# microsoft/GenerativeImage2Text

Hardware: AMD Instinct MI355X
Metric: captions/sec whole-node (GIT_BASE 224px bs=64/GPU greedy len=20) (higher is better)
Workload: dtype f16; 1 GPU; GIT_BASE 224px bs=64/GPU greedy max_len=20 frames=1; global_batch=64, parallelism=dp1, decode_steps_per_caption=19, seq_len_returned=20, hip_graph=True, contexts_in_flight=4, layernorm_folded=True, library=libgitmi_f16.so, encoder_chains=2, schedule=mixed

## Files before the change

generativeimage2text_amd/csrc/abi_ops.hip:

```cpp
#include "../../include/gitmi.h"
#include "abi_common.h"
#include "gitmi_common.h"
#include "launchers.h"

#include <hip/hip_runtime.h>

using namespace gitmi;

#ifdef GITMI_EXPERIMENT
#include "../../include/gitmi_experiment.h"
#define GITMI_EXP_EXPORT extern "C"
#else
#define GITMI_EXP_EXPORT [[maybe_unused]] static
#endif

static inline int round_up(int x, int m) { return (x + m - 1) / m * m; }

extern "C" int gitmi_operand_dtype(void);
static const char* dtype_name(int dtype) {
    return dtype == GITMI_DTYPE_F32 ? "fp32" : dtype == GITMI_DTYPE_BF16 ? "bf16" : dtype == GITMI_DTYPE_F16 ? "fp16" : "unknown";
}
static int check_dtype(const char* op, const char* arg, int dtype) {
    if (dtype == GITMI_DTYPE_F32 || dtype == gitmi_operand_dtype()) return 0;
    return fail("%s: %s is %s (%d), but this library's 16-bit operands are %s (libgitmi%s.so)", op, arg, dtype_name(dtype), dtype,
// ... 164 lines not shown
                                                  const float* stats, int strips, float eps, int M, int V, int K, int cols_per_wg,
                                                  int mtop, const int* ids, int ld_ids, int cur_len, const int* plen, int beams,
                                                  int suppress_kind, float rep_penalty, float* part_val, int* part_idx,
                                                  float* part_lse, float* logits_out, int max_wgs, void* stream) {
    if (!A || !W || !bias || !part_val || !part_idx || !part_lse) return fail("debug_vocab_topm_rules: null argument");
    if (cols_per_wg != 128) return fail("debug_vocab_topm_rules: cols_per_wg must be 128");
    VocabArgs v = vocab_op_args(A, W, bias, colsum, stats, strips, eps, M, V, K, cols_per_wg, part_val, part_idx, part_lse, logits_out, max_wgs);
    if (ids) {
        if (!plen) return fail("debug_vocab_topm_rules: ids without plen");
        if (beams < 1 || M % beams) return fail("debug_vocab_topm_rules: M=%d is not a multiple of beams=%d", M, beams);
        if (cur_len < 1 || cur_len > ld_ids) return fail("debug_vocab_topm_rules: cur_len=%d outside [1, ld_ids=%d]", cur_len, ld_ids);
        if (rep_penalty != 0.f && rep_penalty != 1.f && cur_len > HIST_SLOTS / 2)
            return fail("debug_vocab_topm_rules: the repetition penalty supports histories up to %d tokens (cur_len=%d)", HIST_SLOTS / 2, cur_len);
        v.ids = ids; v.ld_ids = ld_ids; v.cur_len = cur_len; v.plen = plen; v.beams = beams; v.suppress_kind = suppress_kind;
        v.rep_penalty = rep_penalty;
    }
    HIPCK(launch_vocab_topm(v, mtop, (hipStream_t)stream));
    return 0;
}

extern "C" int gitmi_op_sample_rows(const float* logits, int R, int V, float temperature, int top_k, float top_p, int ndraw,
                                    uint64_t seed, int step, float* draw_logprob, int* draw_token, float* filtered_out,
                                    void* stream) {
    float2* lse = nullptr;
    HIPCK(hipMalloc((void**)&lse, (size_t)R * sizeof(float2)));
    hipError_t err = launch_sample_rows(logits, V, V, R, temperature, top_k, top_p, ndraw, seed, step, draw_logprob, draw_token,
                                        lse, filtered_out, nullptr, 0, 0, 0.f, ndraw, (hipStream_t)stream);
    if (err == hipSuccess) err = hipStreamSynchronize((hipStream_t)stream);
    hipFree(lse);
    HIPCK(err);
    return 0;
}

GITMI_EXP_EXPORT int gitmi_debug_set_gemm_impl(int impl) {
    if (!set_gemm_impl(impl)) return fail("debug_set_gemm_impl: unknown selector %d (low byte: -1, 0 or 9)", impl);
    return 0;
}

GITMI_EXP_EXPORT int gitmi_debug_gemm_form(const void* A, int lda, const void* W, const float* bias, const void* res, int ldr, void* C,
                                           int ldc, int M, int N, int K, int act, int in_dtype, int out_dtype, int shared,
                                           const float* ln_part, const float* colsum, float ln_eps, float* part_out,
                                           const float* res_part, const float* res_gamma, const float* res_beta, float res_eps,
                                           void* stream) {
    if (!A || !W || !C) return fail("debug_gemm_form: null argument (A, W, C)");
    if (M < 0 || N < 1 || K < 1) return fail("debug_gemm_form: M=%d N=%d K=%d", M, N, K);
    if (lda < K) return fail("debug_gemm_form: lda=%d < K=%d", lda, K);
    if (ldc < N) return fail("debug_gemm_form: ldc=%d < N=%d", ldc, N);
    if (res && ldr < N) return fail("debug_gemm_form: ldr=%d < N=%d", ldr, N);
    if (act < GITMI_ACT_NONE || act > GITMI_ACT_GELU_ERF) return fail("debug_gemm_form: act=%d", act);
    RCK(check_dtype("debug_gemm_form", "in_dtype", in_dtype));
    const bool in_f32 = in_dtype == GITMI_DTYPE_F32;
    if ((in_f32 && K % 16) || (!in_f32 && K % 64)) return fail("debug_gemm_form: K must be a multiple of %d (K=%d)", in_f32 ? 16 : 64, K);
    GemmArgs g{};
    g.A = A; g.W = W; g.bias = bias; g.res = (const float*)res; g.C = C;
    g.M = M; g.N = N; g.K = K; g.lda = lda; g.ldc = ldc; g.ldr = res ? ldr : 0; g.act = act;
    g.shared = shared ? 1 : 0;
    if (out_dtype == GITMI_DTYPE_F16_STREAM) {
        if (in_f32) return fail("debug_gemm_form: fp16 stream rows need 16-bit operands");
        g.out_f16 = 1;
    } else {
        RCK(check_dtype("debug_gemm_form", "out_dtype", out_dtype));
    }
    const bool out_f32 = out_dtype == GITMI_DTYPE_F32;
    const bool consumer = ln_part != nullptr, producer = part_out != nullptr || res_part != nullptr;
    if (colsum && !consumer) return fail("debug_gemm_form: colsum without ln_part");
    if ((res_gamma || res_beta) && !res_part) return fail("debug_gemm_form: res_gamma / res_beta without res_part");
    if (consumer || producer) {
#ifndef GITMI_OPS_F16
        return fail("debug_gemm_form: the folded-LayerNorm forms are built into the fp16-operand library only");
#endif
        if (consumer && producer) return fail("debug_gemm_form: consumer (ln_part) and producer (part_out / res_part) arguments in one launch");
        if (consumer) {
            if (!colsum) return fail("debug_gemm_form: ln_part without colsum");
            if (res || in_f32 || out_f32 || g.out_f16) return fail("debug_gemm_form: the consumer writes operand-type rows and takes no residual");
            if (K > 1024) return fail("debug_gemm_form: row partials cover K <= 1024 (K=%d)", K);
            g.ln_part = (const float2*)ln_part; g.ln_nparts = (K + 255) / 256; g.ln_colsum = colsum; g.ln_inv_d = 1.0f / (float)K; g.ln_eps = ln_eps;
        } else {
            if (!g.out_f16 || act != GITMI_ACT_NONE) return fail("debug_gemm_form: the producer writes fp16 stream rows and has no activation");
            if (N > 1024) return fail("debug_gemm_form: row partials cover N <= 1024 (N=%d)", N);
            g.part_out = (float2*)part_out;
            if (res_part) {
                if (!res || !res_gamma || !res_beta) return fail("debug_gemm_form: res_part without res / res_gamma / res_beta");
                g.res_part = (const float2*)res_part; g.res_nparts = (N + 255) / 256; g.res_gamma = res_gamma; g.res_beta = res_beta;
                g.res_inv_d = 1.0f / (float)N; g.res_eps = res_eps;
            }
        }
        if (!gemm_uses_p8(g, false, false))
            return fail("debug_gemm_form: the folded forms exist in gemm_p8_kernel only (more than 512 rows, N %% 256 == 0, K >= 128, 16-byte aligned rows)");
    }
    HIPCK(launch_gemm(g, in_f32, out_f32, (hipStream_t)stream));
    return 0;
}

extern "C" int gitmi_op_attn_decode(const void* qkv, const void* img_k, const void* img_v, void* txt_k, void* txt_v,
                                    const int* kv_src, void* out, int B, int H, int N_img, int T_max, int pos, int beams,
                                    int dtype, int dbg, void* stream) {
    RCK(check_dtype("op_attn_decode", "dtype", dtype));
    AttnDecodeArgs a{};
    a.qkv = qkv; a.img_k = img_k; a.img_v = img_v; a.txt_k = txt_k; a.txt_v = txt_v; a.out = out;
    a.kv_src = kv_src; a.ld_src = T_max; a.d = H * 64; a.N_img = N_img; a.T_max = T_max; a.pos = pos; a.beams = beams;
    a.scale = 0.125f; a.dbg = dbg & 0xffff; a.waves_per_pair = (dbg >> 16) & 3; a.stream_wgs = dbg >> 18;
    if (dtype == GITMI_DTYPE_F32) {
        HIPCK(launch_attn_decode(a, B, H, (hipStream_t)stream));
        return 0;
    }
    a.N_pad = round_up(N_img, 32);
    HIPCK(launch_attn_decode_mfma(a, B, H, (hipStream_t)stream));
    return 0;
}
extern "C" int gitmi_op_kv_repack(const void* qkv_rows, void* kf, void* vt, int B, int N, int H, void* stream) {
    HIPCK(launch_kv_repack_frag(qkv_rows, kf, vt, B, N, round_up(N, 32), H, H * 64, (hipStream_t)stream));
    return 0;
}

GITMI_EXP_EXPORT int gitmi_debug_attention_ragged(const void* qkv, void* out, const int* ntok, int B, int N, int H, int dtype, int impl,
                                                  void* stream) {
    if (!ntok) return fail("debug_attention_ragged: ntok is required");
    const size_t esz = dtype == GITMI_DTYPE_F32 ? 4 : 2;
    const int D = H * 64;
    AttnFullArgs a{};
    a.q = qkv;
    a.k = (const char*)qkv + (size_t)D * esz;
    a.v = (const char*)qkv + (size_t)2 * D * esz;
    a.out = out;
    a.ldq = a.ldk = a.ldv = 3 * D;
    a.ldo = D;
    a.N = N; a.H = H; a.scale = 0.125f; a.ntok = ntok;
    HIPCK(launch_attn_full(a, B, dtype == GITMI_DTYPE_F32, impl, (hipStream_t)stream));
    return 0;
}
GITMI_EXP_EXPORT int gitmi_debug_attn_decode_form(const void* qkv, const void* img_k, const void* img_v, void* txt_k, void* txt_v,
                                                  const int* kv_src, void* out, const int* ntok, const int* img_of, int n_images,
                                                  int B, int H, int N_img, int T_max, int pos, int beams, int dtype, int out_frag,
                                                  int pairs_per_wg, int waves_per_pair, int stream_wgs, void* stream) {
    RCK(check_dtype("debug_attn_decode_form", "dtype", dtype));
    if (!qkv || !img_k || !img_v || !txt_k || !txt_v || !kv_src || !out) return fail("debug_attn_decode_form: null argument");
    if (beams < 1 || beams > 8) return fail("debug_attn_decode_form: beams=%d outside [1, 8]", beams);
    if (n_images < 1) return fail("debug_attn_decode_form: n_images=%d", n_images);
    if (B < 1 || H < 1 || N_img < 1 || pos < 0 || pos >= T_max)
        return fail("debug_attn_decode_form: B=%d H=%d N_img=%d pos=%d T_max=%d", B, H, N_img, pos, T_max);
    if (out_frag && dtype == GITMI_DTYPE_F32) return fail("debug_attn_decode_form: out_frag needs 16-bit rows");
    if (ntok && stream_wgs > 0) return fail("debug_attn_decode_form: the streaming kernel does not serve ragged batches (ntok)");
    AttnDecodeArgs a{};
    a.qkv = qkv; a.img_k = img_k; a.img_v = img_v; a.txt_k = txt_k; a.txt_v = txt_v; a.out = out;
    a.kv_src = kv_src; a.ld_src = T_max; a.d = H * 64; a.N_img = N_img; a.T_max = T_max; a.pos = pos; a.beams = beams;
    a.scale = 0.125f; a.ntok = ntok; a.img_of = img_of; a.out_frag = out_frag;
    a.pairs_per_wg = pairs_per_wg; a.waves_per_pair = waves_per_pair; a.stream_wgs = stream_wgs;
    if (dtype == GITMI_DTYPE_F32) {
        HIPCK(launch_attn_decode(a, B, H, (hipStream_t)stream));
        return 0;
    }
    a.N_pad = round_up(N_img, 32);
    HIPCK(launch_attn_decode_mfma(a, B, H, (hipStream_t)stream));
    return 0;
}
GITMI_EXP_EXPORT int gitmi_debug_attn_decode_ragged(const void* qkv, const void* img_k, const void* img_v, void* txt_k, void* txt_v,
                                                    const int* kv_src, void* out, const int* ntok, int B, int H, int N_img, int T_max,
                                                    int pos, int beams, int dtype, void* stream) {
    if (!ntok) return fail("debug_attn_decode_ragged: ntok is required");
    return gitmi_debug_attn_decode_form(qkv, img_k, img_v, txt_k, txt_v, kv_src, out, ntok, nullptr, B, B, H, N_img, T_max, pos, beams,
                                        dtype, 0, 0, 0, 0, stream);
}

extern "C" int gitmi_preprocess_image(const uint8_t* rgb_hwc, int H, int W, int crop, uint8_t* tmp, size_t tmp_bytes,
                                      float* out_chw, void* stream) {
    if (!rgb_hwc || !out_chw || H < 1 || W < 1 || crop < 1) return fail("preprocess: bad argument");
    const int nw = W <= H ? crop : (int)((double)crop * W / H);
    if (nw != W && (!tmp || tmp_bytes < (size_t)H * nw * 3)) return fail("preprocess: workspace must hold H * %d * 3 bytes", nw);
    HIPCK(launch_preprocess(rgb_hwc, H, W, crop, tmp, out_chw, (hipStream_t)stream));
    return 0;
}

extern "C" int gitmi_preprocess_batch(const uint8_t* rgb, size_t rgb_bytes, const int64_t* desc_host, int n, int crop, uint8_t* tmp,
                                      size_t tmp_bytes, float* out, void* stream) {
    if (!rgb || !desc_host || !out || n < 1 || crop < 1 || crop > 4096) return fail("preprocess_batch: bad argument");
    for (int i = 0; i < n; ++i) {
        const int64_t off = desc_host[3 * i], H = desc_host[3 * i + 1], W = desc_host[3 * i + 2];
        if (H < 1 || W < 1 || H > 65535 || W > 65535 || off < 0 || (uint64_t)off + (uint64_t)H * W * 3 > rgb_bytes ||
            (uint64_t)off + (uint64_t)H * W * 3 > 0xffffffffull)
            return fail("preprocess_batch: image %d (offset %lld, %lld x %lld) does not fit the staging buffer of %zu bytes", i,
                        (long long)off, (long long)H, (long long)W, rgb_bytes);
        const double r = W <= H ? (double)H / W : (double)W / H;
        if (r * crop > 65535.0) return fail("preprocess_batch: image %d: aspect ratio too extreme", i);
    }
    const size_t need = preprocess_batch_workspace((const long long*)desc_host, n, crop);
    if (need > 0 && (!tmp || tmp_bytes < need)) return fail("preprocess_batch: workspace must hold %zu bytes", need);
    if (need > 0xffffffffull) return fail("preprocess_batch: batch too large for one call");
    HIPCK(launch_preprocess_batch(rgb, (const long long*)desc_host, n, crop, tmp, out, (hipStream_t)stream));
    return 0;
}

extern "C" int gitmi_preprocess_image_to(const uint8_t* rgb_hwc, int H, int W, int out_h, int out_w, uint8_t* tmp,
                                         size_t tmp_bytes, float* out_chw, void* stream) {
    if (!rgb_hwc || !out_chw || H < 1 || W < 1 || out_h < 1 || out_w < 1) return fail("preprocess: bad argument");
    if (out_w != W && (!tmp || tmp_bytes < (size_t)H * out_w * 3))
        return fail("preprocess: workspace must hold H * %d * 3 bytes", out_w);
    HIPCK(launch_resize_crop_norm(rgb_hwc, H, W, out_h, out_w, 0, 0, out_h, out_w, tmp, out_chw, (hipStream_t)stream));
    return 0;
}

GITMI_EXP_EXPORT int gitmi_debug_score_attn(const void* qkv, const void* img_kv, const int* image_of, void* out, int Q, int H,
                                            int N_img, int Lp, int dtype, void* stream) {
    if (!qkv || !img_kv || !image_of || !out) return fail("debug_score_attn: null argument");
    if (dtype != GITMI_DTYPE_F32 && dtype != gitmi_operand_dtype()) return fail("debug_score_attn: dtype %d not served by this build", dtype);
    HIPCK(launch_score_attn(qkv, img_kv, image_of, out, Q, H, H * 64, N_img, Lp, 0.125f, dtype == GITMI_DTYPE_F32,
                            (hipStream_t)stream));
    return 0;
}
GITMI_EXP_EXPORT int gitmi_debug_score_attn_map(const void* qkv, const void* img_kv, const int* image_of, const int* ntok, float* out,
                                                int Q, int H, int N_img, int Lp, int dtype, void* stream) {
    if (!qkv || !img_kv || !image_of || !out || Q < 1 || H < 1 || N_img < 1 || Lp < 1) return fail("debug_score_attn_map: bad argument");
    if (dtype != GITMI_DTYPE_F32 && dtype != gitmi_operand_dtype()) return fail("debug_score_attn_map: dtype %d not served by this build", dtype);
    hipStream_t s = (hipStream_t)stream;
    const bool f32 = dtype == GITMI_DTYPE_F32;
    const int d = H * 64, Kc = N_img + Lp;
    void* ctx = nullptr; float2* stats = nullptr;
    auto body = [&]() -> int {
        HIPCK(hipMalloc(&ctx, (size_t)Q * Lp * d * (f32 ? 4 : 2)));
        HIPCK(hipMalloc(&stats, (size_t)Q * H * Lp * sizeof(float2)));
        HIPCK(launch_score_attn(qkv, img_kv, image_of, ctx, Q, H, d, N_img, Lp, 0.125f, f32, s, ntok, stats));
        HIPCK(launch_score_attn_map(qkv, img_kv, image_of, ntok, stats, nullptr, out, (size_t)Lp * Kc, (size_t)Kc, Lp, Q, H, N_img, Lp,
                                    0.125f, f32, nullptr, s));
        HIPCK(hipStreamSynchronize(s));
        return 0;
    };
    const int rc = body();
    hipFree(ctx); hipFree(stats);
    return rc;
}
GITMI_EXP_EXPORT int gitmi_debug_score_head(const void* A, const void* W, const float* bias, const int* tgt, int M, int V, int K,
                                            int dtype, float* out, void* stream) {
    if (!A || !W || !bias || !tgt || !out || M < 1 || V < 2 || K < 32 || K % 32) return fail("debug_score_head: bad argument");
    if (dtype != GITMI_DTYPE_F32 && dtype != gitmi_operand_dtype()) return fail("debug_score_head: dtype %d not served by this build", dtype);
    hipStream_t s = (hipStream_t)stream;
    const bool f32 = dtype == GITMI_DTYPE_F32;
    const int ntiles = f32 ? 1 : score_head_tiles(V);
    const int ldl = round_up(V, 8);
    float4* part = nullptr; float* zt = nullptr; float2* o2 = nullptr; int* bad = nullptr; float* logits = nullptr;
    int rc = 0;
    auto body = [&]() -> int {
        HIPCK(hipMalloc(&part, (size_t)M * ntiles * sizeof(float4)));
        HIPCK(hipMalloc(&zt, (size_t)M * sizeof(float)));
        HIPCK(hipMalloc(&o2, (size_t)(M + 1) * sizeof(float2)));
        HIPCK(hipMalloc(&bad, (size_t)M * sizeof(int)));
        if (f32) {
            HIPCK(hipMalloc(&logits, (size_t)M * ldl * sizeof(float)));
            GemmArgs g{};
            g.A = A; g.W = W; g.bias = bias; g.C = logits; g.M = M; g.N = V; g.K = K; g.lda = K; g.ldc = ldl;
            HIPCK(launch_gemm(g, true, true, s));
            HIPCK(launch_score_rowstats(logits, ldl, V, tgt, 0, M, part, zt, s));
        } else {
            HIPCK(launch_score_head(A, K, W, bias, tgt, M, V, K, part, zt, s));
        }
        HIPCK(hipMemsetAsync(o2, 0, (size_t)(M + 1) * sizeof(float2), s));
        HIPCK(launch_score_combine(part, ntiles, zt, tgt, M, 1, 1, V, o2, bad, s));
        HIPCK(hipMemcpyAsync(out, o2 + 1, (size_t)M * sizeof(float2), hipMemcpyDefault, s));
        HIPCK(hipStreamSynchronize(s));
        return 0;
    };
    rc = body();
    hipFree(part); hipFree(zt); hipFree(o2); hipFree(bad); hipFree(logits);
    return rc;
}

#ifdef GITMI_EXPERIMENT
GITMI_EXP_EXPORT int gitmi_debug_im2col(const float* img, void* out, int out_dtype, int B, int H, int W, int p, int K, int Kpad,
                                        void* stream) {
    if (!img || !out) return fail("debug_im2col: null argument");
    RCK(check_dtype("debug_im2col", "out_dtype", out_dtype));
    if (B < 1 || p < 1 || H < p || W < p || K != 3 * p * p || Kpad < K) return fail("debug_im2col: bad shape");
    HIPCK(launch_im2col(img, out, out_dtype == GITMI_DTYPE_F32, B, H, W, p, K, Kpad, (hipStream_t)stream));
    return 0;
}
GITMI_EXP_EXPORT int gitmi_debug_pos_resize(const float* pos, float* out, int g, int gh, int gw, int D, void* stream) {
    if (!pos || !out || g < 1 || gh < 1 || gw < 1 || D < 1) return fail("debug_pos_resize: bad argument");
    HIPCK(launch_pos_bicubic(pos, out, g, gh, gw, D, (hipStream_t)stream));
    return 0;
}
GITMI_EXP_EXPORT int gitmi_debug_vit_assemble(const float* patch_out, const float* cls, const float* pos, const float* gamma,
                                              const float* beta, float eps, void* X, int x_f16, int B, int N, int D, float* part,
                                              void* stream) {
    if (!patch_out || !cls || !pos || !gamma || !beta || !X || B < 1 || N < 1 || D < 1) return fail("debug_vit_assemble: bad argument");
    HIPCK(launch_vit_assemble_ln(patch_out, cls, pos, gamma, beta, eps, X, x_f16 != 0, B, N, D, (float2*)part, (D + 255) / 256,
                                 (hipStream_t)stream));
    return 0;
}
GITMI_EXP_EXPORT int gitmi_debug_ragged_front(int stage, const float* src, float* slots, int* meta, int* ntok, void* patches,
                                              int patches_dtype, const float* patch_out, const float* cls, const float* pos, int g,
                                              const float* gamma, const float* beta, float eps, void* X, int x_f16, float* part,
                                              int B, int p, long long max_pixels, int Nmax, int K, int Kpad, int D, void* stream) {
    hipStream_t s = (hipStream_t)stream;
    if (B < 1 || p < 1 || max_pixels < 1 || Nmax < 2 || !meta) return fail("debug_ragged_front: bad argument");
    const size_t slot = (size_t)3 * (size_t)max_pixels;
    if (stage == 0) {
        if (!src || !slots || !ntok) return fail("debug_ragged_front: staging takes src, slots, meta and ntok");
        HIPCK(launch_ragged_stage(src, slots, slot, (int4*)meta, ntok, B, p, (size_t)max_pixels, Nmax, s));
    } else if (stage == 1) {
        if (!slots || !patches || K != 3 * p * p || Kpad < K) return fail("debug_ragged_front: im2col takes slots, meta and patches");
        RCK(check_dtype("debug_ragged_front", "patches_dtype", patches_dtype));
        HIPCK(launch_im2col_ragged(slots, slot, (const int4*)meta, patches, patches_dtype == GITMI_DTYPE_F32, B, Nmax, p, K, Kpad, s));
    } else if (stage == 2) {
        if (!patch_out || !cls || !pos || !gamma || !beta || !X || g < 1 || D < 1) return fail("debug_ragged_front: assembly argument missing");
        HIPCK(launch_vit_assemble_ragged(patch_out, cls, pos, g, (const int4*)meta, gamma, beta, eps, X, x_f16 != 0, B, Nmax, p, D,
                                         (float2*)part, s));
    } else {
        return fail("debug_ragged_front: stage %d (0 staging, 1 im2col, 2 assembly)", stage);
// ... 51 lines not shown
```

generativeimage2text_amd/csrc/engine.hip:

```cpp
#include "../../include/gitmi.h"
#include "engine_state.h"

#include <algorithm>
#include <cmath>
#include <cstdarg>
#include <cstdio>
#include <cstring>

using namespace gitmi;

#ifdef GITMI_EXPERIMENT
#include "../../include/gitmi_experiment.h"
#define GITMI_EXP_EXPORT extern "C"
#else
#define GITMI_EXP_EXPORT [[maybe_unused]] static
#endif

static thread_local char g_err[1024] = "";
int gitmi::fail(const char* fmt, ...) {
    va_list ap;
    va_start(ap, fmt);
    vsnprintf(g_err, sizeof(g_err), fmt, ap);
    va_end(ap);
    return 1;
// ... 276 lines not shown
    return 0;
}

static Stream vit_stream(gitmi_engine* e, int M) {
    const int D = e->cfg.vit_width;
    const VitLayerW& L = e->w.vit[0];
    Stream st;
    st.x = e->v_x; st.M = M; st.D = D; st.tag = TAG_GEMM_VIT; st.t = e->v_h;
    st.fold = e->pol.ln_fold && on_p8(e->v_x, D, L.qkv_f.w, e->v_qkv, 3 * D, M, 3 * D, D, false) &&
              on_p8(e->v_x, D, L.ffn1_f.w, e->v_u, 4 * D, M, 4 * D, D, false) && on_p8(e->v_ctx, D, L.wo, e->v_x, D, M, D, D, true) &&
              on_p8(e->v_u, 4 * D, L.w2, e->v_x, D, M, D, 4 * D, true);
    if (st.fold) st.parts[0] = st.parts[1] = e->v_part;
    return st;
}
static Stream prefill_stream(gitmi_engine* e, int M) {
    const int d = e->cfg.dec_hidden, ffn = e->cfg.dec_ffn, D = e->cfg.vit_width;
    const DecLayerW& L = e->w.dec[0];
    Stream st;
    st.x = e->p_y; st.M = M; st.D = d; st.tag = TAG_GEMM_OTHER; st.t = e->p_ht; st.xn = e->p_hf;
    st.fold = e->pol.ln_fold && on_p8(e->feats, D, e->w.vp_w, e->p_y, d, M, d, D, true) &&
              on_p8(e->p_y, d, L.qkv_pf.w, e->img_kv[0], 3 * d, M, 3 * d, d, false) &&
              on_p8(e->p_y, d, L.qkv_pf.w, e->img_kv[0], 3 * d, M, 2 * d, d, false) &&
              (e->cfg.dec_layers < 2 || (on_p8(e->p_y, d, L.ffn1_pf.w, e->p_u, ffn, M, ffn, d, false) &&
                                         on_p8(e->p_ctx, d, L.wo, e->p_y, d, M, d, d, true) && on_p8(e->p_u, ffn, L.w2, e->p_y, d, M, d, ffn, true)));
    if (st.fold) { st.parts[0] = e->p_part[0]; st.parts[1] = e->p_part[1]; }
    return st;
}

static int encode_frames_impl(gitmi_engine* e, const float* const* frames, int F, int B, float* feats_out,
                              hipStream_t s, int stride = 0) {
    const gitmi_config& c = e->cfg;
    const int D = c.vit_width, N = e->N;
    const int F_eff = c.num_frames > 0 ? std::min(F, c.num_frames) : F;
    const int Nimg = stride > 0 ? stride : F_eff * N;
    drop_resident(e);
    SpanGuard phase(e, s, TAG_VIT, 0);
    const int BI = F_eff * B;
    const int M = BI * N;
    const int g2 = N - 1;
    const size_t slot = (size_t)3 * e->max_pixels;
    if (e->ragged)
        HIPCK(launch_im2col_ragged(e->frame_stage[0], slot, e->rg_meta, e->patches, e->pol.f32, B, N, c.patch, e->Kp, e->Kp_pad, s));
    else
    for (int fr = 0; fr < F_eff; ++fr)
        HIPCK(launch_im2col(frames[fr], (char*)e->patches + (size_t)fr * B * g2 * e->Kp_pad * e->pol.esz, e->pol.f32, B,
                            e->H, e->W, c.patch, e->Kp, e->Kp_pad, s));
    RCK(gemm(e, s, e->patches, e->Kp_pad, e->w.conv_w, nullptr, nullptr, 0, e->patch_out, D, true, BI * g2, D, e->Kp_pad, 0,
             TAG_GEMM_VIT));
    Stream x = vit_stream(e, M);
    float2* part = stream_part_out(x);
    if (e->ragged)
        HIPCK(launch_vit_assemble_ragged(e->patch_out, e->w.cls, e->w.pos, e->g_nat, e->rg_meta, e->w.lnpre_g, e->w.lnpre_b, 1e-5f, e->v_x,
                                         e->pol.stream_f16, BI, N, c.patch, D, part, s));
    else
    HIPCK(launch_vit_assemble_ln(e->patch_out, e->w.cls, e->pos_cur, e->w.lnpre_g, e->w.lnpre_b, 1e-5f, e->v_x, e->pol.stream_f16, BI, N, D,
                                 part, D / 256, s));
    stream_written(x, part, e->w.vit[0].ln1g, e->w.vit[0].ln1b, 1e-5f);
    for (int l = 0; l < c.vit_layers; ++l) {
        const VitLayerW& L = e->w.vit[l];
        const VitLayerW* Ln = l + 1 < c.vit_layers ? &e->w.vit[l + 1] : nullptr;
        RCK(ln_gemm(e, s, x, L.qkv_f, L.wqkv, L.bqkv, e->v_qkv, 3 * D, 0, 3 * D, 0));
        RCK(attn_full_packed(e, e->v_qkv, e->v_ctx, D, c.vit_heads, N, BI, e->ragged ? e->rg_ntok : nullptr, s));
        RCK(gemm_to_stream(e, s, x, e->v_ctx, D, L.wo, L.bo, D, true, L.ln2g, L.ln2b, 1e-5f));
        RCK(ln_gemm(e, s, x, L.ffn1_f, L.w1, L.b1, e->v_u, 4 * D, 0, 4 * D, 1));
        RCK(gemm_to_stream(e, s, x, e->v_u, 4 * D, L.w2, L.b2, 4 * D, true, Ln ? Ln->ln1g : nullptr, Ln ? Ln->ln1b : nullptr, 1e-5f));
    }
    for (int fr = 0; fr < F_eff; ++fr) {
        const float* te = (c.num_frames > 0 && e->pol.use_temb) ? e->w.temb[fr] : nullptr;
        if (e->pol.stream_f16) {
            const char* xs = (const char*)e->v_x + (size_t)fr * B * N * D * 2;
            HIPCK(launch_layernorm_s16(xs, D, e->w.lnpost_g, e->w.lnpost_b, 1e-5f, te, e->feats, D, false, nullptr, 0, B * N, D, N,
                                       Nimg, fr * N, s));
            if (feats_out)
                HIPCK(launch_layernorm_s16(xs, D, e->w.lnpost_g, e->w.lnpost_b, 1e-5f, te, feats_out, D, true, nullptr, 0, B * N, D,
                                           N, Nimg, fr * N, s));
        } else {
            HIPCK(launch_layernorm(e->v_x + (size_t)fr * B * N * D, D, e->w.lnpost_g, e->w.lnpost_b, 1e-5f, te, e->feats, D, e->pol.f32,
                                   feats_out, D, B * N, D, N, Nimg, fr * N, s));
        }
    }
    if (e->ragged) {
        HIPCK(launch_zero_pad_rows(e->feats, e->pol.f32, D, e->rg_ntok, B, N, s));
        if (feats_out) HIPCK(launch_zero_pad_rows(feats_out, true, D, e->rg_ntok, B, N, s));
    }

    set_resident(e, B, F_eff, stride);
    return 0;
}

static int kv_repack(gitmi_engine* e, int l, int B, int Nimg, hipStream_t s) {
    const gitmi_config& c = e->cfg;
    void* kh = e->img_kh[l];
    void* vh = e->img_vh[l];
    if (e->pol.f32) HIPCK(launch_kv_repack(e->img_kv[l], kh, vh, B, Nimg, c.dec_heads, c.dec_hidden, s));
    else HIPCK(launch_kv_repack_frag(e->img_kv[l], kh, vh, B, Nimg, round_up(Nimg, 32), c.dec_heads, c.dec_hidden, s));
    return 0;
}

static int prefill_impl(gitmi_engine* e, hipStream_t s) {
    const gitmi_config& c = e->cfg;
    const int d = c.dec_hidden, ffn = c.dec_ffn, D = c.vit_width;
    const int B = e->cur_B, Nimg = e->cur_Nimg, M = B * Nimg;
    e->have_prefill = false;
    SpanGuard phase(e, s, TAG_PREFILL, 0);
    Stream y = prefill_stream(e, M);
    RCK(gemm_to_stream(e, s, y, e->feats, D, e->w.vp_w, e->w.vp_b, D, false, e->w.vp_lng, e->w.vp_lnb, 1e-5f));
    for (int l = 0; l < c.dec_layers; ++l) {
        const DecLayerW& L = e->w.dec[l];
        const bool last = l + 1 == c.dec_layers;
        const int col0 = last ? d : 0;
        RCK(ln_gemm(e, s, y, L.qkv_pf, L.wqkv, L.bqkv, e->img_kv[l], 3 * d, col0, 3 * d - col0, 0));
        RCK(kv_repack(e, l, B, Nimg, s));
        if (last) break;
        RCK(attn_full_packed(e, e->img_kv[l], e->p_ctx, d, c.dec_heads, Nimg, B, key_counts(e), s));
        RCK(gemm_to_stream(e, s, y, e->p_ctx, d, L.wo, L.bo, d, true, L.lnag, L.lnab, 1e-12f));
        RCK(ln_gemm(e, s, y, L.ffn1_pf, L.w1, L.b1, e->p_u, ffn, 0, ffn, 2));
        RCK(gemm_to_stream(e, s, y, e->p_u, ffn, L.w2, L.b2, ffn, true, L.lnog, L.lnob, 1e-12f));
    }
    set_prefilled(e);
    return 0;
}

#ifdef GITMI_EXPERIMENT
#define GITMI_SKIPPED(e, bit) (((e)->pol.decode_skip & (bit)) != 0)
#else
#define GITMI_SKIPPED(e, bit) false
#endif
static int dgemm(gitmi_engine* e, hipStream_t s, const DGemmArgs& g_in) {
    DGemmArgs g = g_in;
    g.dbg = e->pol.dgemm_dbg;
    g.no_row_walk = e->pol.dgemm_no_row_walk >= 0 ? e->pol.dgemm_no_row_walk : e->pol.shared_device ? 0 : 1;
    g.strips_per_wg = e->pol.dgemm_strips >= 0 ? e->pol.dgemm_strips : e->pol.shared_device ? 2 : 1;
    g.rows_per_wg = e->pol.dgemm_rows > 0 ? e->pol.dgemm_rows : g.M > 64 ? 64 : e->pol.shared_device ? 32 : 16;
    SpanGuard sp(e, s, TAG_GEMM_OTHER, gemm_flops(g.M, g.N, g.K));
    HIPCK(launch_dgemm(g, s));
    return 0;
}

static DGemmArgs dgemm_ln(const void* A, const Folded& f, const DLn* ln, void* C, int c_frag, int act, int M, int N, int K) {
    return dgemm_ln(A, f.w, f.bias, f.colsum, ln, C, c_frag, act, M, N, K);
}

static int decode_layers_impl(gitmi_engine* e, const int* kv_src, int ld_ids, int pos, int R, int beams, hipStream_t s) {
    const gitmi_config& c = e->cfg;
    const int d = c.dec_hidden, ffn = c.dec_ffn;
    const int B = R / beams;
    const bool chain = e->pol.skinny && !e->pol.f32;
    for (int l = 0; l < c.dec_layers; ++l) {
        const DecLayerW& L = e->w.dec[l];
        const DecLayerW* Lp = l > 0 ? &e->w.dec[l - 1] : nullptr;
        const DLn ln_prev{e->stats_o, d / 16, 1.0f / (float)d, 1e-12f, Lp ? Lp->lnog : nullptr, Lp ? Lp->lnob : nullptr};
        const DLn ln_a{e->stats_a, d / 16, 1.0f / (float)d, 1e-12f, L.lnag, L.lnab};
        const DLn* ln_o = Lp ? &ln_prev : nullptr;
        if (chain) {
            if (!GITMI_SKIPPED(e, 2)) RCK(dgemm(e, s, dgemm_ln(l == 0 ? e->d_ht : e->xo_b, L.qkv_f, ln_o, e->d_qkv, 0, 0, R, 3 * d, d)));
        } else {
            RCK(gemm(e, s, e->d_ht, d, L.wqkv, L.bqkv, nullptr, 0, e->d_qkv, 3 * d, e->pol.f32, R, 3 * d, d, 0, TAG_GEMM_OTHER));
        }
        AttnDecodeArgs a{};
        a.qkv = e->d_qkv; a.img_k = e->img_kh[l]; a.img_v = e->img_vh[l]; a.txt_k = e->txt_k[l]; a.txt_v = e->txt_v[l]; a.out = e->d_ctx;
        a.kv_src = kv_src; a.ld_src = ld_ids; a.d = d; a.N_img = e->cur_Nimg; a.T_max = c.max_text_len;
        a.img_of = e->img_identity ? nullptr : e->img_of_dev;
        a.pos = pos; a.beams = beams; a.scale = 0.125f;
        a.out_frag = chain ? 1 : 0;
        a.N_pad = round_up(e->cur_Nimg, 32);
        a.dbg = e->pol.attn_dbg;
        a.waves_per_pair = e->pol.attn_nh;
        a.pairs_per_wg = e->pol.attn_pw > 0 ? e->pol.attn_pw : e->pol.shared_device ? 8 : 4;
        const bool stream_ok = !e->pol.shared_device && a.N_pad <= 8 * 32 && B * c.dec_heads >= 384 && e->pol.attn_nh != 2;
        a.stream_wgs = e->pol.attn_stream >= 0 ? e->pol.attn_stream : stream_ok ? 192 : 0;
        if (e->keyed) { a.ntok = e->rg_ntok; a.stream_wgs = 0; }
        if (e->pol.f32) HIPCK(launch_attn_decode(a, B, c.dec_heads, s));
        else if (!GITMI_SKIPPED(e, 1)) HIPCK(launch_attn_decode_mfma(a, B, c.dec_heads, s));
        if (chain) {
            if (!GITMI_SKIPPED(e, 4))
                RCK(dgemm(e, s, dgemm_to_stream(e->d_ctx, L.wo_p, L.bo, l == 0 ? e->d_hf : e->xo_f, ln_o, e->xa_f, e->xa_b, e->stats_a, R, d, d)));
            if (!GITMI_SKIPPED(e, 2)) RCK(dgemm(e, s, dgemm_ln(e->xa_b, L.ffn1_f, &ln_a, e->d_u, 1, 2, R, ffn, d)));
            if (!GITMI_SKIPPED(e, 4))
                RCK(dgemm(e, s, dgemm_to_stream(e->d_u, L.w2_p, L.b2, e->xa_f, &ln_a, e->xo_f, e->xo_b, e->stats_o, R, d, ffn)));
        } else {
            RCK(dec_layer_tail(e, s, L, e->d_ctx, e->d_hf, e->d_ht, e->d_y, e->d_u, R));
        }
    }
    return 0;
}

static int sample_candidates(gitmi_engine* e, const float* logits, int ldl, int R, int step, hipStream_t s, StepCands* cands);
static int trie_candidates(gitmi_engine* e, const float* logits, int ldl, int cur_len, hipStream_t s, StepCands* cands);
static float rep_penalty_of(const gitmi_engine* e) {
    const double rp = e->sample.repetition_penalty;
    return (e->ss.kind == GITMI_SEARCH_GENERATOR && rp > 0 && rp != 1.0) ? (float)rp : 0.f;
}

static int decode_head_impl(gitmi_engine* e, const int* ids, int ld_ids, int cur_len, int R, int beams, int suppress_kind,
                            int M, float* logits_out, int ldl, hipStream_t s, StepCands* cands) {
    const gitmi_config& c = e->cfg;
    const int d = c.dec_hidden;
    const bool chain = e->pol.skinny && !e->pol.f32;
    cands->part_val = e->part_val; cands->part_idx = e->part_idx; cands->part_lse = e->part_lse;
    const bool sampling = ids != nullptr && e->ss.sampled;
    const bool trie = ids != nullptr && e->trie_search;
    if ((sampling || trie) && !logits_out) { logits_out = e->logits; ldl = e->ldl; }
    if (chain) {
        VocabArgs v{};
        v.A = (const unsigned short*)e->xo_b; v.lda = d; v.W = (const unsigned short*)e->w.out_f.w; v.bias = e->w.out_f.bias; v.colsum = e->w.out_f.colsum;
        v.stats_in = e->stats_o; v.strips_in = d / 16; v.inv_d = 1.0f / (float)d; v.eps_in = 1e-12f;
        v.M = R; v.N = c.vocab; v.K = d; v.cols_per_wg = e->vocab_cols;
        v.max_wgs = e->pol.vocab_wgs >= 0 ? e->pol.vocab_wgs : (e->pol.shared_device && R <= 64) ? 60 : 0;
        v.ids = ids; v.ld_ids = ld_ids; v.cur_len = cur_len; v.plen = e->plen_dev; v.beams = beams; v.suppress_kind = suppress_kind;
        v.rep_penalty = ids ? rep_penalty_of(e) : 0.f;
        v.part_val = e->part_val; v.part_idx = e->part_idx; v.part_lse = e->part_lse;
        v.logits_out = logits_out; v.ld_logits = ldl;
        {
            SpanGuard sp(e, s, TAG_GEMM_OTHER, gemm_flops(R, c.vocab, d));
            if (!GITMI_SKIPPED(e, 8)) HIPCK(launch_vocab_topm(v, M, s));
        }
        cands->nparts = e->vocab_nparts; cands->slots = vocab_mtop_slots(M);
        if (sampling) RCK(sample_candidates(e, logits_out, ldl, R, cur_len, s, cands));
        if (trie) RCK(trie_candidates(e, logits_out, ldl, cur_len, s, cands));
    } else {
        RCK(gemm(e, s, e->d_ht, d, e->w.out_w, e->w.out_b, nullptr, 0, e->logits, e->ldl, true, R, c.vocab, d, 0, TAG_GEMM_OTHER));
        cands->nparts = 1; cands->slots = row_topm_slots(M);
        if (sampling) RCK(sample_candidates(e, e->logits, e->ldl, R, cur_len, s, cands));
        else if (trie) RCK(trie_candidates(e, e->logits, e->ldl, cur_len, s, cands));
        else if (ids)
            HIPCK(launch_row_topm(e->logits, e->ldl, c.vocab, ids, ld_ids, cur_len, e->plen_dev, beams, suppress_kind,
                                  rep_penalty_of(e), M, R,
                                  e->part_val, e->part_idx, e->part_lse, s));
        if (logits_out && logits_out != e->logits) HIPCK(launch_copy_f32(e->logits, e->ldl, logits_out, ldl, R, c.vocab, s));
    }
    return 0;
}

static int check_ready(gitmi_engine* e) {
    if (!e) return fail("null engine");
    if (!e->finalized) return fail("weights not finalized (call gitmi_finalize_weights)");
    HIPCK(hipSetDevice(e->device));
    return 0;
}

static int ragged_prepare(gitmi_engine* e, const float* const* frames, int F, int B, hipStream_t s) {
    if (!e->ragged) return 0;
    if (F != 1 || !frames[0]) return fail("ragged input (gitmi_set_image_shape(e, 0, 0)): F must be 1, frames[0] the descriptor buffer");
    drop_resident(e);
    HIPCK(launch_ragged_stage(frames[0], e->frame_stage[0], (size_t)3 * e->max_pixels, e->rg_meta, e->rg_ntok, B, e->cfg.patch,
                              e->max_pixels, e->Nmax, s));
    return 0;
}

static int check_frames(const gitmi_engine* e, const char* who, const float* const* frames, int F, int B) {
    if (!frames || F < 1 || F > e->cfg.max_frames) return fail("%s: F=%d outside [1,%d]", who, F, e->cfg.max_frames);
    if (B < 1 || B > e->cfg.max_batch) return fail("%s: B=%d outside [1,%d]", who, B, e->cfg.max_batch);
    return 0;
}

static int check_resident(const gitmi_engine* e, const char* who, int B) {
    if (!e->have_feats)
        return fail("%s: frames == NULL is a follow-up call, but the engine holds no resident images (encode some with a call "
                    "that takes frames; a change of the image shape or mode, of the temporal embedding or of the LayerNorm "
                    "folding, and a failed call, drop them)", who);
    if (B != e->cur_B) return fail("%s: follow-up call with B=%d, but %d images are resident (B must equal that count)", who, B, e->cur_B);
    return 0;
}

extern "C" int gitmi_encode_frames(gitmi_engine* e, const float* const* frames, int F, int B, float* feats_out,
                                   void* stream) {
    RCK(check_ready(e));
    RCK(check_frames(e, "encode_frames", frames, F, B));
    RCK(ragged_prepare(e, frames, F, B, (hipStream_t)stream));
    return encode_frames_impl(e, frames, F, B, feats_out, (hipStream_t)stream);
}

static EmbedArgs embed_args(gitmi_engine* e, bool on) {
    EmbedArgs em{};
    if (!on) return em;
    em.words = e->w.words_f; em.positions = e->w.positions_f; em.gamma = e->w.emb_lng; em.beta = e->w.emb_lnb; em.eps = 1e-8f;
    em.h_f = e->d_hf; em.h_t = e->d_ht; em.D = e->cfg.dec_hidden; em.vocab = e->cfg.vocab;
    em.frag = (e->pol.skinny && !e->pol.f32) ? 1 : 0;
    return em;
}
static int embed_position(gitmi_engine* e, const int* ids, int ld_ids, int pos, int R, hipStream_t s) {
    const EmbedArgs em = embed_args(e, true);
    HIPCK(launch_embed_ln(ids, ld_ids, pos, em.words, em.positions, em.gamma, em.beta, em.eps, em.h_f, em.h_t, e->pol.f32, R, em.D,
                          em.vocab, em.frag != 0, s));
    return 0;
}

extern "C" int gitmi_prefill(gitmi_engine* e, void* stream) {
    RCK(check_ready(e));
    if (!e->have_feats) return fail("prefill: no encoded frames");
    return prefill_impl(e, (hipStream_t)stream);
}

extern "C" int gitmi_step_logits(gitmi_engine* e, const int64_t* tokens, int R, int t, float* logits_out, void* stream) {
    RCK(check_ready(e));
    if (!e->have_feats) return fail("step_logits: no encoded frames");
    hipStream_t s = (hipStream_t)stream;
    if (!e->have_prefill) RCK(prefill_impl(e, s));
    const int B = e->cur_B;
    if (R < B || R % B) return fail("step_logits: R=%d is not a multiple of the encoded batch %d", R, B);
    const int beams = R / B;
    if (beams > e->cfg.max_beams) return fail("step_logits: %d beams exceed max_beams", beams);
    if (t < 1 || t > e->cfg.max_text_len) return fail("step_logits: t=%d outside [1,%d]", t, e->cfg.max_text_len);
    const gitmi_config& c = e->cfg;
    const int T = c.max_text_len;
    e->img_identity = true;
    HIPCK(launch_load_ids((const long long*)tokens, R, t, e->ss.ids[0], e->ss.kv_src[0], T, s));
    StepCands cands{};
    for (int pos = 0; pos < t; ++pos) {
        SpanGuard step(e, s, TAG_STEP, 0);
        RCK(embed_position(e, e->ss.ids[0], T, pos, R, s));
        RCK(decode_layers_impl(e, e->ss.kv_src[0], T, pos, R, beams, s));
        if (pos == t - 1) RCK(decode_head_impl(e, nullptr, T, t, R, beams, 0, 1, logits_out, c.vocab, s, &cands));
    }
    return 0;
}

static int search_begin_impl(gitmi_engine* e, const Request& rq, int V, hipStream_t s) {
    const gitmi_config& c = e->cfg;
    const gitmi_search* sp = rq.sp;
    const int B = rq.Q, minP = rq.minP, maxP = rq.maxP;
    if (!sp) return fail("search: null config");
    if (sp->kind != GITMI_SEARCH_AUTOREGRESSIVE && sp->kind != GITMI_SEARCH_GENERATOR && sp->kind != GITMI_SEARCH_TRIE)
        return fail("search: bad kind");
    if (sp->kind == GITMI_SEARCH_TRIE) {
// ... 784 lines not shown
```

generativeimage2text_amd/csrc/kernels_attn_decode.hip:

```cpp
#include "gitmi_common.h"
#include "launchers.h"
#include <algorithm>
#include <type_traits>

#pragma clang fp contract(off)

namespace gitmi {

static constexpr int HD = 64;

__global__ __launch_bounds__(256) void kv_repack_frag_kernel(const bf16_t* __restrict__ qkv, bf16_t* __restrict__ kf,
                                                             bf16_t* __restrict__ vt, int N, int Np, int H, int d) {
    __shared__ bf16_t vs[32][HD + 8];
    const int s = blockIdx.x, h = blockIdx.y, b = blockIdx.z, tid = threadIdx.x;
    const int nsteps = Np >> 5;
    bf16_t* kdst = kf + ((size_t)b * H + h) * Np * HD;
    bf16_t* vdst = vt + ((size_t)b * H + h) * Np * HD;
    const int key = tid >> 3, ch = tid & 7;
    const int n = s * 32 + key;
    u32x4_t kv = {0u, 0u, 0u, 0u}, vv = kv;
    if (n < N) {
        const bf16_t* src = qkv + ((size_t)b * N + n) * 3 * d + d + h * HD + ch * 8;
        kv = *reinterpret_cast<const u32x4_t*>(src);
        vv = *reinterpret_cast<const u32x4_t*>(src + d);
    }
    *reinterpret_cast<u32x4_t*>(kdst + frag_tile(n >> 4, ch >> 2, 2, (ch & 3) * 16 + (n & 15))) = kv;
    *reinterpret_cast<u32x4_t*>(&vs[key][ch * 8]) = vv;
    __syncthreads();
    const int dt = tid >> 6, lane = tid & 63, lg = lane >> 4, dim = dt * 16 + (lane & 15);
    bf16_t o[8];
#pragma unroll
    for (int e = 0; e < 8; ++e) o[e] = vs[(e >> 2) * 16 + lg * 4 + (e & 3)][dim];
    u32x4_t ov;
#pragma unroll
    for (int e = 0; e < 4; ++e) ov[e] = (uint32_t)o[2 * e] | ((uint32_t)o[2 * e + 1] << 16);
    *reinterpret_cast<u32x4_t*>(vdst + (((size_t)s * 4 + dt) * 64 + lane) * 8) = ov;
}

__device__ __forceinline__ void unpack8(const u32x4_t& r, float (&v)[8]) {
#pragma unroll
    for (int i = 0; i < 4; ++i) {
        unpack2op(r[i], v[2 * i], v[2 * i + 1]);
    }
}
__device__ __forceinline__ void ld8bf(const bf16_t* p, float (&v)[8]) { unpack8(*reinterpret_cast<const u32x4_t*>(p), v); }

constexpr int ACS = 4;

struct Pair {
    int h, row0;
    bool on;
};

template <int KB>
__device__ __forceinline__ void load_text_kv(const AttnDecodeArgs& a, const Pair& p, int j, int s, int sub, u32x4_t& kr, u32x4_t& vr) {
    if (s == a.pos) {
        const bf16_t* src = reinterpret_cast<const bf16_t*>(a.qkv) + (size_t)(p.row0 + j) * (3 * a.d) + a.d + p.h * HD + sub * 8;
        kr = *reinterpret_cast<const u32x4_t*>(src);
        vr = *reinterpret_cast<const u32x4_t*>(src + a.d);
    } else {
        const int srow = KB == 1 ? p.row0 : a.kv_src[(size_t)(p.row0 + j) * a.ld_src + s];
        const size_t off = ((size_t)srow * a.T_max + s) * a.d + p.h * HD + sub * 8;
        kr = *reinterpret_cast<const u32x4_t*>(reinterpret_cast<const bf16_t*>(a.txt_k) + off);
        vr = *reinterpret_cast<const u32x4_t*>(reinterpret_cast<const bf16_t*>(a.txt_v) + off);
    }
}

template <int KB, int TI>
struct TextItems {
    int j[TI];
    u32x4_t kr[TI], vr[TI];
    __device__ __forceinline__ void load(const AttnDecodeArgs& a, const Pair& p, int grp, int ngrp, int sub) {
        const int nt = a.pos + 1;
#pragma unroll
        for (int u = 0; u < TI; ++u) {
            const int it = grp + ngrp * u;
            j[u] = (p.on && it < a.beams * nt) ? it / nt : -1;
            const int s = it < a.beams * nt ? it % nt : 0;
            kr[u] = u32x4_t{0u, 0u, 0u, 0u};
            vr[u] = kr[u];
            if (j[u] >= 0) load_text_kv<KB>(a, p, j[u], s, sub, kr[u], vr[u]);
        }
    }
};

__device__ __forceinline__ void append_text_cache(const AttnDecodeArgs& a, const Pair& p, int t, int sub) {
    if (p.on && t < a.beams * 8) {
        const int j = t >> 3;
        const bf16_t* src = reinterpret_cast<const bf16_t*>(a.qkv) + (size_t)(p.row0 + j) * (3 * a.d) + a.d + p.h * HD + sub * 8;
        const size_t dst = ((size_t)(p.row0 + j) * a.T_max + a.pos) * a.d + p.h * HD + sub * 8;
        *reinterpret_cast<u32x4_t*>(reinterpret_cast<bf16_t*>(a.txt_k) + dst) = *reinterpret_cast<const u32x4_t*>(src);
        *reinterpret_cast<u32x4_t*>(reinterpret_cast<bf16_t*>(a.txt_v) + dst) = *reinterpret_cast<const u32x4_t*>(src + a.d);
    }
}

__device__ __forceinline__ void load_q_frag(const AttnDecodeArgs& a, const Pair& p, int l15, int lg, bf16x8_t (&qf)[2]) {
#pragma unroll
    for (int ds = 0; ds < 2; ++ds) {
        float qv[8] = {0.f, 0.f, 0.f, 0.f, 0.f, 0.f, 0.f, 0.f};
        if (p.on && l15 < a.beams)
            ld8bf(reinterpret_cast<const bf16_t*>(a.qkv) + (size_t)(p.row0 + l15) * (3 * a.d) + p.h * HD + ds * 32 + lg * 8, qv);
        u32x4_t t;
#pragma unroll
        for (int e = 0; e < 4; ++e) t[e] = pack2bf(qv[2 * e] * a.scale, qv[2 * e + 1] * a.scale);
        qf[ds] = __builtin_bit_cast(bf16x8_t, t);
    }
}

struct ImagePartial {
    float m, l;
    f32x4_t o[4];
    __device__ __forceinline__ void init() {
        m = -INFINITY;
        l = 0.f;
#pragma unroll
        for (int dt = 0; dt < 4; ++dt) o[dt] = f32x4_t{0.f, 0.f, 0.f, 0.f};
    }
    __device__ __forceinline__ static void mask_max(f32x4_t (&sc)[2], int s, int nimg_steps, int n_img, int lg, float& cm) {
#pragma unroll
        for (int t = 0; t < 2; ++t)
#pragma unroll
            for (int r = 0; r < 4; ++r) {
                if (s * 32 + t * 16 + lg * 4 + r >= n_img || s >= nimg_steps) sc[t][r] = -INFINITY;
                cm = fmaxf(cm, sc[t][r]);
            }
    }
    __device__ __forceinline__ float new_max(float cm, bool rescale) {
        cm = fmaxf(cm, __shfl_xor(cm, 16, 64));
        cm = fmaxf(cm, __shfl_xor(cm, 32, 64));
        const float mn = fmaxf(m, cm);
        if (rescale) {
            const float al = fast_exp(m - mn);
            l *= al;
#pragma unroll
            for (int dt = 0; dt < 4; ++dt) { o[dt][0] *= al; o[dt][1] *= al; o[dt][2] *= al; o[dt][3] *= al; }
        }
        m = mn;
        return mn;
    }
    __device__ __forceinline__ bf16x8_t p_frag(const f32x4_t (&sc)[2], float mn) {
        float p[8];
#pragma unroll
        for (int t = 0; t < 2; ++t)
#pragma unroll
            for (int r = 0; r < 4; ++r) {
                p[t * 4 + r] = fast_exp(sc[t][r] - mn);
                l += p[t * 4 + r];
            }
        u32x4_t pp;
#pragma unroll
        for (int e = 0; e < 4; ++e) pp[e] = pack2bf(p[2 * e], p[2 * e + 1]);
        return __builtin_bit_cast(bf16x8_t, pp);
    }
    __device__ __forceinline__ void finish() {
        l += __shfl_xor(l, 16, 64);
        l += __shfl_xor(l, 32, 64);
    }
    template <int KB>
    __device__ __forceinline__ void publish(float (&slot)[KB][HD + 2], int k, int l15, int lg) const {
        if (l15 < k) {
#pragma unroll
            for (int dt = 0; dt < 4; ++dt)
#pragma unroll
                for (int r = 0; r < 4; ++r) slot[l15][dt * 16 + lg * 4 + r] = o[dt][r];
            if (lg == 0) { slot[l15][HD] = m; slot[l15][HD + 1] = l; }
        }
    }
};

template <int KB>
struct TextPartial {
    float q[KB][8], m[KB], l[KB], o[KB][8];
    __device__ __forceinline__ void init(const AttnDecodeArgs& a, const Pair& p, int sub) {
#pragma unroll
        for (int j = 0; j < KB; ++j) {
            m[j] = -INFINITY;
            l[j] = 0.f;
#pragma unroll
            for (int e = 0; e < 8; ++e) { q[j][e] = 0.f; o[j][e] = 0.f; }
            if (p.on && j < a.beams) {
                ld8bf(reinterpret_cast<const bf16_t*>(a.qkv) + (size_t)(p.row0 + j) * (3 * a.d) + p.h * HD + sub * 8, q[j]);
#pragma unroll
                for (int e = 0; e < 8; ++e) q[j][e] *= a.scale;
            }
        }
    }
    __device__ __forceinline__ void item(int jj, const u32x4_t& kr, const u32x4_t& vr) {
        float kv[8], vv[8];
        unpack8(kr, kv);
        unpack8(vr, vv);
#pragma unroll
        for (int j = 0; j < KB; ++j) {
            if (j == jj) {
                float sv = 0.f;
#pragma unroll
                for (int e = 0; e < 8; ++e) sv = fmaf(q[j][e], kv[e], sv);
                sv += __shfl_xor(sv, 1, 64);
                sv += __shfl_xor(sv, 2, 64);
                sv += __shfl_xor(sv, 4, 64);
                const float mn = fmaxf(m[j], sv);
                const float al = fast_exp(m[j] - mn);
                const float pe = fast_exp(sv - mn);
                l[j] = fmaf(l[j], al, pe);
#pragma unroll
                for (int e = 0; e < 8; ++e) o[j][e] = fmaf(o[j][e], al, pe * vv[e]);
                m[j] = mn;
            }
        }
    }
    template <int TI>
    __device__ __forceinline__ void items(const TextItems<KB, TI>& ti, bool enabled) {
#pragma unroll
        for (int u = 0; u < TI; ++u) {
            if (ti.j[u] >= 0 && enabled) item(ti.j[u], ti.kr[u], ti.vr[u]);
        }
    }
    template <int TI>
    __device__ __forceinline__ void tail(const AttnDecodeArgs& a, const Pair& p, int grp, int ngrp, int sub) {
        if (!p.on) return;
        const int nt = a.pos + 1;
        for (int it = grp + ngrp * TI; it < a.beams * nt; it += ngrp) {
            u32x4_t kr, vr;
            load_text_kv<KB>(a, p, it / nt, it % nt, sub, kr, vr);
            item(it / nt, kr, vr);
        }
    }
    __device__ __forceinline__ void merge_groups() {
#pragma unroll
        for (int j = 0; j < KB; ++j) {
#pragma unroll
            for (int off = 8; off < 64; off <<= 1) {
                const float m2 = __shfl_xor(m[j], off, 64);
                const float l2 = __shfl_xor(l[j], off, 64);
                const float mn = fmaxf(m[j], m2);
                const float a1 = m[j] == -INFINITY ? 0.f : fast_exp(m[j] - mn);
                const float a2 = m2 == -INFINITY ? 0.f : fast_exp(m2 - mn);
                l[j] = fmaf(l[j], a1, l2 * a2);
#pragma unroll
                for (int e = 0; e < 8; ++e) {
                    const float o2 = __shfl_xor(o[j][e], off, 64);
                    o[j][e] = fmaf(o[j][e], a1, o2 * a2);
                }
                m[j] = mn;
            }
        }
    }
    __device__ __forceinline__ void fold_into(float (&slot)[KB][HD + 2], int k, int lane, int sub) const {
#pragma unroll
        for (int j = 0; j < KB; ++j) {
            if (lane < 8 && j < k) {
                const float mi = slot[j][HD], li = slot[j][HD + 1];
                const float mn = fmaxf(mi, m[j]);
                const float a1 = mi == -INFINITY ? 0.f : fast_exp(mi - mn);
                const float a2 = m[j] == -INFINITY ? 0.f : fast_exp(m[j] - mn);
#pragma unroll
                for (int e = 0; e < 8; ++e) slot[j][sub * 8 + e] = fmaf(slot[j][sub * 8 + e], a1, o[j][e] * a2);
                if (sub == 0) { slot[j][HD] = mn; slot[j][HD + 1] = fmaf(li, a1, l[j] * a2); }
            }
        }
    }
};

__device__ __forceinline__ void store_out(const AttnDecodeArgs& a, int row, int col, float r) {
    bf16_t* O = reinterpret_cast<bf16_t*>(a.out);
    if (a.out_frag) O[frag_offset(row, col, a.d >> 5)] = f2bf(r);
    else O[(size_t)row * a.d + col] = f2bf(r);
}
template <int KB>
__device__ __forceinline__ void write_rows(const AttnDecodeArgs& a, const Pair& p, const float (&s0)[KB][HD + 2], int t, int nthr) {
    if (!p.on) return;
    for (int i = t; i < a.beams * HD; i += nthr) {
        const int j = i / HD, dd = i % HD;
        const float r1 = s0[j][dd] / s0[j][HD + 1];
        store_out(a, p.row0 + j, p.h * HD + dd, r1);
    }
}
template <int KB>
__device__ __forceinline__ void write_rows(const AttnDecodeArgs& a, const Pair& p, const float (&s0)[KB][HD + 2],
                                           const float (&s1)[KB][HD + 2], int t, int nthr) {
    if (!p.on) return;
    for (int i = t; i < a.beams * HD; i += nthr) {
        const int j = i / HD, dd = i % HD;
        const float m0 = s0[j][HD], m1 = s1[j][HD];
        const float mm = fmaxf(m0, m1);
        const float a0 = m0 == -INFINITY ? 0.f : fast_exp(m0 - mm);
        const float a1 = m1 == -INFINITY ? 0.f : fast_exp(m1 - mm);
        const float num = fmaf(a0, s0[j][dd], a1 * s1[j][dd]);
        const float den = fmaf(a0, s0[j][HD + 1], a1 * s1[j][HD + 1]);
        const float r = num / den;
        store_out(a, p.row0 + j, p.h * HD + dd, r);
    }
}

template <int KB, int TI = 3, int PW = 1, int NH = 2, bool RAGGED = false>
__global__ __launch_bounds__(64 * NH * PW) void attn_decode_mfma_kernel(AttnDecodeArgs a) {
    __shared__ float part[PW][NH][KB][HD + 2];
    constexpr int PT = 64 * NH;

    const int tid = threadIdx.x, lane = tid & 63, wave = tid >> 6;
    const int l15 = lane & 15, lg = lane >> 4;
    const int hp = wave / NH, half = wave % NH;
    const int H = a.d / HD;
    const int k = a.beams;
    const int Np = a.N_pad, nsteps = Np >> 5;
    const int pair = NH == 2 ? (int)(blockIdx.y * H + blockIdx.x) : (int)blockIdx.x * PW + hp;
    Pair p;
    p.on = PW == 1 || pair < a.n_pairs;
    p.h = p.on ? pair % H : 0;
    const int b = p.on ? pair / H : 0;
    p.row0 = b * k;
    const int bi = a.img_of ? a.img_of[b] : b;
    const bf16_t* Kf = reinterpret_cast<const bf16_t*>(a.img_k) + ((size_t)bi * H + p.h) * Np * HD;
    const bf16_t* Vt = reinterpret_cast<const bf16_t*>(a.img_v) + ((size_t)bi * H + p.h) * Np * HD;
    const int n_img = RAGGED ? a.ntok[bi] : a.N_img;
    const int nimg_steps = (!p.on || (a.dbg & 1)) ? 0 : RAGGED ? (n_img + 31) >> 5 : nsteps;

    bf16x8_t kq[ACS][2][2], vq[ACS][4];
    auto load_chunk = [&](int s0) {
#pragma unroll
        for (int c = 0; c < ACS; ++c) {
            const int s = s0 + NH * c;
            const bool on = s < nimg_steps && !(a.dbg & 8);
            const bf16_t* kp = Kf + frag_tile(2 * s, 0, 2, lane);
            const bf16_t* vp = Vt + ((size_t)s * 4 * 64 + lane) * 8;
#pragma unroll
            for (int t = 0; t < 2; ++t)
#pragma unroll
                for (int ds = 0; ds < 2; ++ds) {
                    const bf16x8_t* q = reinterpret_cast<const bf16x8_t*>(kp + (t * 2 + ds) * 512);
                    kq[c][t][ds] = !on ? bf16x8_t{0, 0, 0, 0, 0, 0, 0, 0} : (a.dbg & 16) ? *q : __builtin_nontemporal_load(q);
                }
#pragma unroll
            for (int dt = 0; dt < 4; ++dt) {
                const bf16x8_t* q = reinterpret_cast<const bf16x8_t*>(vp + dt * 512);
                vq[c][dt] = !on ? bf16x8_t{0, 0, 0, 0, 0, 0, 0, 0} : (a.dbg & 16) ? *q : __builtin_nontemporal_load(q);
            }
        }
    };
    load_chunk(half);

    const int t = tid % PT, grp = t >> 3, sub = tid & 7;
    TextItems<KB, TI> ti;
    ti.load(a, p, grp, 8 * NH, sub);
    append_text_cache(a, p, t, sub);
    bf16x8_t qf[2];
    load_q_frag(a, p, l15, lg, qf);

    ImagePartial ip;
    ip.init();
    for (int s0 = half; s0 < nimg_steps; s0 += NH * ACS) {
        if (s0 != half) load_chunk(s0);
        f32x4_t sc[ACS][2];
        float cm = -INFINITY;
#pragma unroll
        for (int c = 0; c < ACS; ++c) {
#pragma unroll
            for (int u = 0; u < 2; ++u) {
                sc[c][u] = mfma16(kq[c][u][0], qf[0], f32x4_t{0.f, 0.f, 0.f, 0.f});
                sc[c][u] = mfma16(kq[c][u][1], qf[1], sc[c][u]);
            }
            ip.mask_max(sc[c], s0 + NH * c, nimg_steps, RAGGED ? n_img : a.N_img, lg, cm);
        }
        const float mn = ip.new_max(cm, s0 != half);
#pragma unroll
        for (int c = 0; c < ACS; ++c) {
            const bf16x8_t pf = ip.p_frag(sc[c], mn);
            if (a.dbg & 4) {
#pragma unroll
                for (int dt = 0; dt < 4; ++dt) asm volatile("" ::"v"(vq[c][dt]));
                asm volatile("" ::"v"(pf));
                continue;
            }
#pragma unroll
            for (int dt = 0; dt < 4; ++dt) ip.o[dt] = mfma16(vq[c][dt], pf, ip.o[dt]);
        }
    }
    ip.finish();
    TextPartial<KB> tp;
    tp.init(a, p, sub);
    tp.items(ti, !(a.dbg & 2));
    tp.template tail<TI>(a, p, grp, 8 * NH, sub);
    tp.merge_groups();
    ip.publish(part[hp][half], k, l15, lg);
    if constexpr (NH > 1) __syncthreads(); else __builtin_amdgcn_wave_barrier();
    tp.fold_into(part[hp][half], k, lane, sub);
    if constexpr (NH > 1) __syncthreads(); else __builtin_amdgcn_wave_barrier();
    if constexpr (NH == 1) write_rows(a, p, part[hp][0], t, PT);
    else write_rows(a, p, part[hp][0], part[hp][NH - 1], t, PT);
}

typedef __attribute__((address_space(3))) void attn_lds_void_t;

template <int N> __device__ __forceinline__ void attn_wait_vm() { asm volatile("s_waitcnt vmcnt(%0)" ::"n"(N) : "memory"); }
__device__ __forceinline__ void attn_wait_slots_ahead(int ahead) {
    switch (ahead) {
        case 0: attn_wait_vm<0>(); break;
        case 1: attn_wait_vm<4>(); break;
        case 2: attn_wait_vm<8>(); break;
        case 3: attn_wait_vm<12>(); break;
        case 4: attn_wait_vm<16>(); break;
        case 5: attn_wait_vm<20>(); break;
        case 6: attn_wait_vm<24>(); break;
        case 7: attn_wait_vm<28>(); break;
        case 8: attn_wait_vm<32>(); break;
        case 9: attn_wait_vm<36>(); break;
        case 10: attn_wait_vm<40>(); break;
        default: attn_wait_vm<44>(); break;
    }
}

constexpr int AS_WAVES = 4;
constexpr int AS_SLOT = 4096;

template <int KB, int TI, int RING>
__global__ __launch_bounds__(64 * AS_WAVES) void attn_decode_stream_kernel(AttnDecodeArgs a) {
    static_assert(RING >= 2 && RING <= 12, "ring depth");
    __shared__ __attribute__((aligned(16))) unsigned char ring_mem[AS_WAVES][RING * AS_SLOT];
    __shared__ float part[AS_WAVES][KB][HD + 2];

    const int tid = threadIdx.x, lane = tid & 63;
    const int wave = __builtin_amdgcn_readfirstlane(tid >> 6);
    const int l15 = lane & 15, lg = lane >> 4;
    const int H = a.d / HD;
    const int k = a.beams;
    const int Np = a.N_pad, nsteps = Np >> 5;
    unsigned char* ring = ring_mem[wave];

    const int W = (int)gridDim.x * AS_WAVES, w0 = (int)blockIdx.x * AS_WAVES + wave;
    const int npw = w0 < a.n_pairs ? (a.n_pairs - 1 - w0) / W + 1 : 0;
    const int slots_per_pair = 2 * nsteps;
    const int total_slots = npw * slots_per_pair;

    int issued = 0;
    int p_ord = 0, p_s0 = 0, p_v = 0, p_c = 0;
    const bf16_t* p_K = nullptr; const bf16_t* p_V = nullptr;
    auto producer_pair = [&]() {
        const int pair = w0 + p_ord * W;
        const int h = pair % H, b = pair / H;
        const int bi = a.img_of ? a.img_of[b] : b;
        p_K = reinterpret_cast<const bf16_t*>(a.img_k) + ((size_t)bi * H + h) * Np * HD;
        p_V = reinterpret_cast<const bf16_t*>(a.img_v) + ((size_t)bi * H + h) * Np * HD;
    };
    if (npw > 0) producer_pair();
    auto issue_slot = [&]() {
        if (issued >= total_slots) return;
        const bf16_t* src = (p_v ? p_V : p_K) + (size_t)(p_s0 + p_c) * (AS_SLOT / 2) + lane * 8;
        unsigned char* dst = ring + (issued % RING) * AS_SLOT;
#pragma unroll
        for (int f = 0; f < 4; ++f)
            __builtin_amdgcn_global_load_lds((const void*)(src + f * 512), (attn_lds_void_t*)(dst + f * 1024), 16, 0, 2);
        ++issued;
        const int nsc = min(ACS, nsteps - p_s0);
        if (++p_c == nsc) {
            p_c = 0;
            if (p_v == 0) p_v = 1;
            else {
                p_v = 0; p_s0 += ACS;
                if (p_s0 >= nsteps) { p_s0 = 0; ++p_ord; if (p_ord < npw) producer_pair(); }
            }
        }
    };
    for (int i = 0; i < RING; ++i) issue_slot();

    int consumed = 0;
    auto slot_ready = [&]() -> const unsigned char* {
        const int ahead = issued - consumed - 1;
        if (ahead == RING - 1) attn_wait_vm<4 * (RING - 1)>();
        else attn_wait_slots_ahead(ahead);
        return ring + (consumed % RING) * AS_SLOT;
    };
    auto slot_done = [&]() {
        asm volatile("s_waitcnt lgkmcnt(0)" ::: "memory");
        ++consumed;
        issue_slot();
    };


    for (int ord = 0; ord < npw; ++ord) {
        const int pair = w0 + ord * W;
        const Pair p{pair % H, (pair / H) * k, true};

        const int grp = lane >> 3, sub = lane & 7;
        TextItems<KB, TI> ti;
        ti.load(a, p, grp, 8, sub);
        append_text_cache(a, p, lane, sub);
        bf16x8_t qf[2];
        load_q_frag(a, p, l15, lg, qf);

        ImagePartial ip;
        ip.init();
        for (int s0 = 0; s0 < nsteps; s0 += ACS) {
            f32x4_t sc[ACS][2];
            float cm = -INFINITY;
#pragma unroll
            for (int c = 0; c < ACS; ++c) {
                if (s0 + c < nsteps) {
                    const unsigned char* sl = slot_ready();
                    bf16x8_t kq[2][2];
#pragma unroll
                    for (int t = 0; t < 2; ++t)
#pragma unroll
                        for (int ds = 0; ds < 2; ++ds)
                            kq[t][ds] = *reinterpret_cast<const bf16x8_t*>(sl + (t * 2 + ds) * 1024 + lane * 16);
                    __builtin_amdgcn_sched_barrier(0);
#pragma unroll
                    for (int t = 0; t < 2; ++t) {
                        sc[c][t] = mfma16(kq[t][0], qf[0], f32x4_t{0.f, 0.f, 0.f, 0.f});
                        sc[c][t] = mfma16(kq[t][1], qf[1], sc[c][t]);
                    }
                    slot_done();
                } else {
                    sc[c][0] = f32x4_t{0.f, 0.f, 0.f, 0.f};
                    sc[c][1] = sc[c][0];
                }
                ip.mask_max(sc[c], s0 + c, nsteps, a.N_img, lg, cm);
            }
            const float mn = ip.new_max(cm, s0 != 0);
#pragma unroll
            for (int c = 0; c < ACS; ++c) {
                const bf16x8_t pf = ip.p_frag(sc[c], mn);
                if (s0 + c < nsteps) {
                    const unsigned char* sl = slot_ready();
                    bf16x8_t vq[4];
#pragma unroll
                    for (int dt = 0; dt < 4; ++dt) vq[dt] = *reinterpret_cast<const bf16x8_t*>(sl + dt * 1024 + lane * 16);
                    __builtin_amdgcn_sched_barrier(0);
#pragma unroll
                    for (int dt = 0; dt < 4; ++dt) ip.o[dt] = mfma16(vq[dt], pf, ip.o[dt]);
                    slot_done();
                } else {
#pragma unroll
                    for (int dt = 0; dt < 4; ++dt) ip.o[dt] = mfma16(bf16x8_t{0, 0, 0, 0, 0, 0, 0, 0}, pf, ip.o[dt]);
                }
            }
        }
        ip.finish();
        TextPartial<KB> tp;
        tp.init(a, p, sub);
        tp.items(ti, true);
        tp.template tail<TI>(a, p, grp, 8, sub);
        tp.merge_groups();
        ip.publish(part[wave], k, l15, lg);
        __builtin_amdgcn_wave_barrier();
        tp.fold_into(part[wave], k, lane, sub);
        __builtin_amdgcn_wave_barrier();
        write_rows(a, p, part[wave], lane, 64);
        __builtin_amdgcn_wave_barrier();
    }
}

hipError_t launch_kv_repack_frag(const void* qkv, void* kf, void* vt, int B, int N, int N_pad, int H, int d, hipStream_t s) {
    if (B <= 0 || N <= 0) return hipSuccess;
    if (N_pad % 32 || N_pad < N) return hipErrorInvalidValue;
    hipLaunchKernelGGL(kv_repack_frag_kernel, dim3(N_pad / 32, H, B), dim3(256), 0, s, (const bf16_t*)qkv, (bf16_t*)kf,
                       (bf16_t*)vt, N, N_pad, H, d);
    return hipGetLastError();
}

template <typename F>
static void with_beam_rows(int beams, F&& f) {
    if (beams <= 1) f(std::integral_constant<int, 1>{});
    else if (beams <= 2) f(std::integral_constant<int, 2>{});
    else if (beams <= 4) f(std::integral_constant<int, 4>{});
    else f(std::integral_constant<int, 8>{});
}

hipError_t launch_attn_decode_mfma(const AttnDecodeArgs& a, int B, int H, hipStream_t s) {
    if (B <= 0) return hipSuccess;
    if (a.beams > 8 || a.N_pad % 32 || a.N_pad < a.N_img || a.N_img < 1) return hipErrorInvalidValue;
    if (a.ntok && a.stream_wgs > 0) return hipErrorInvalidValue;
    AttnDecodeArgs p = a;
    p.n_pairs = B * H;
    if (a.stream_wgs > 0) {
        const int nwg = std::max(1, std::min(a.stream_wgs, (p.n_pairs + AS_WAVES - 1) / AS_WAVES));
        with_beam_rows(a.beams, [&](auto kb) {
            constexpr int KB = decltype(kb)::value;
            hipLaunchKernelGGL((attn_decode_stream_kernel<KB, 3, KB == 8 ? 8 : 9>), dim3(nwg), dim3(64 * AS_WAVES), 0, s, p);
        });
        return hipGetLastError();
    }
    const bool one_wave = a.waves_per_pair == 1 || (a.waves_per_pair != 2 && a.N_pad <= 8 * 32);
    if (a.ntok || !one_wave) {
        with_beam_rows(a.beams, [&](auto kb) {
            constexpr int KB = decltype(kb)::value;
            if (a.ntok) hipLaunchKernelGGL((attn_decode_mfma_kernel<KB, 3, 1, 2, true>), dim3(H, B), dim3(128), 0, s, p);
            else hipLaunchKernelGGL((attn_decode_mfma_kernel<KB>), dim3(H, B), dim3(128), 0, s, p);
        });
        return hipGetLastError();
    }
    int pw = a.pairs_per_wg >= 8 ? 8 : a.pairs_per_wg >= 4 || a.pairs_per_wg <= 0 ? 4 : a.pairs_per_wg >= 2 ? 2 : 1;
    while (pw > 1 && p.n_pairs / pw < 96) pw >>= 1;
    if (a.beams > 4 && pw == 8) pw = 4;
    with_beam_rows(a.beams, [&](auto kb) {
        constexpr int KB = decltype(kb)::value;
        auto packed = [&](auto pwc) {
            constexpr int PW = decltype(pwc)::value;
            hipLaunchKernelGGL((attn_decode_mfma_kernel<KB, 3, PW, 1>), dim3((p.n_pairs + PW - 1) / PW), dim3(64 * PW), 0, s, p);
        };
        if (pw == 8) { if constexpr (KB < 8) packed(std::integral_constant<int, 8>{}); }
        else if (pw == 4) packed(std::integral_constant<int, 4>{});
        else if (pw == 2) packed(std::integral_constant<int, 2>{});
        else packed(std::integral_constant<int, 1>{});
    });
    return hipGetLastError();
}

}
```

generativeimage2text_amd/csrc/kernels_dgemm.hip:

```cpp
#include "gitmi_common.h"
#include "launchers.h"
#include <type_traits>
#include <utility>

namespace gitmi {

constexpr int STRIP_SLOTS = 16;

struct RowStatLoads {
    float2 v[STRIP_SLOTS];
};
__device__ __forceinline__ void stats_issue(RowStatLoads& L, const float2* __restrict__ stats, int strips, int M,
                                            int row, int lg) {
#pragma unroll
    for (int u = 0; u < STRIP_SLOTS; ++u) {
        const int sidx = lg + 4 * u;
        L.v[u] = sidx < strips ? stats[(size_t)sidx * M + row] : float2{0.f, 0.f};
    }
}
__device__ __forceinline__ void stats_issue_nb(RowStatLoads& L, const float2* __restrict__ stats, int strips, int M,
                                               int row, int lg) {
#pragma unroll
    for (int u = 0; u < STRIP_SLOTS; ++u) {
        const int sidx = lg + 4 * u;
        const float2 v = stats[(size_t)min(sidx, strips - 1) * M + row];
        L.v[u] = sidx < strips ? v : float2{0.f, 0.f};
    }
}
__device__ __forceinline__ void stats_finish(const RowStatLoads& L, float inv_d, float eps, float& mean, float& rstd) {
    float s = 0.f, q = 0.f;
#pragma unroll
    for (int u = 0; u < STRIP_SLOTS; ++u) { s += L.v[u].x; q += L.v[u].y; }
    s += __shfl_xor(s, 16, 64); q += __shfl_xor(q, 16, 64);
    s += __shfl_xor(s, 32, 64); q += __shfl_xor(q, 32, 64);
    mean = s * inv_d;
    const float var = fmaxf(q * inv_d - mean * mean, 0.f);
    rstd = rsqrtf(var + eps);
}


struct KSlice { int kb, ke; };
__device__ __forceinline__ KSlice k_slice(int ksteps, int nw, int wave) {
    const int per = (ksteps + nw - 1) / nw;
    const int kb = wave * per;
    return KSlice{kb, min(kb + per, ksteps)};
}

__device__ __forceinline__ float4 load_cols4(const float* p, int n, int N) {
    float4 r;
    r.x = p[n < N ? n : N - 1];
    r.y = p[n + 1 < N ? n + 1 : N - 1];
    r.z = p[n + 2 < N ? n + 2 : N - 1];
    r.w = p[n + 3 < N ? n + 3 : N - 1];
    return r;
}

constexpr int DW_KS = 6;
struct WSlice { bf16x8_t f[DW_KS]; };
__device__ __forceinline__ WSlice load_w_slice(const bf16_t* W, int strip, KSlice ks, int ksteps, int lane) {
    WSlice w;
    const bf16_t* wp = W + frag_tile(strip, 0, ksteps, lane);
#pragma unroll
    for (int u = 0; u < DW_KS; ++u)
        w.f[u] = ks.kb + u < ks.ke ? __builtin_nontemporal_load(reinterpret_cast<const bf16x8_t*>(wp + (size_t)(ks.kb + u) * 512))
                                   : bf16x8_t{0, 0, 0, 0, 0, 0, 0, 0};
    return w;
}
__device__ __forceinline__ void load_x_slice(bf16x8_t (&xf)[DW_KS][4], const bf16_t* X, int rt0, KSlice ks, int ksteps, int lane) {
#pragma unroll
    for (int u = 0; u < DW_KS; ++u)
#pragma unroll
        for (int i = 0; i < 4; ++i)
            xf[u][i] = ks.kb + u < ks.ke ? *reinterpret_cast<const bf16x8_t*>(X + frag_tile(rt0 + i, ks.kb + u, ksteps, lane))
                                         : bf16x8_t{0, 0, 0, 0, 0, 0, 0, 0};
}
__device__ __forceinline__ void mfma_slice(f32x4_t (&acc)[4], const WSlice& w, const bf16x8_t (&xf)[DW_KS][4], KSlice ks) {
#pragma unroll
    for (int u = 0; u < DW_KS; ++u) {
        if (ks.kb + u < ks.ke) {
#pragma unroll
            for (int i = 0; i < 4; ++i) acc[i] = mfma16(w.f[u], xf[u][i], acc[i]);
        }
    }
}

template <int NW, int MT>
__device__ __forceinline__ f32x4_t sum_waves(f32x4_t (*red)[MT][64], int tile, int lane) {
    f32x4_t tot = {0.f, 0.f, 0.f, 0.f};
#pragma unroll
    for (int w = 0; w < NW; ++w) {
        const f32x4_t t = red[w][tile][lane];
        tot[0] += t[0]; tot[1] += t[1]; tot[2] += t[2]; tot[3] += t[3];
    }
    return tot;
}

#define DGEMM_CONSUMER_FINISH(v, tot, bias4, cs4, have_stats, mean, rstd, act)              \
    float v[4] = {(tot)[0], (tot)[1], (tot)[2], (tot)[3]};                                  \
    {                                                                                       \
        const float biasv[4] = {(bias4).x, (bias4).y, (bias4).z, (bias4).w};                \
        if (have_stats) {                                                                   \
            const float cs[4] = {(cs4).x, (cs4).y, (cs4).z, (cs4).w};                       \
            _Pragma("unroll") for (int r = 0; r < 4; ++r) v[r] = (rstd) * (v[r] - (mean) * cs[r]) + biasv[r]; \
        } else {                                                                            \
            _Pragma("unroll") for (int r = 0; r < 4; ++r) v[r] += biasv[r];                 \
        }                                                                                   \
        if ((act) != GITMI_ACT_NONE) {                                                      \
            _Pragma("unroll") for (int r = 0; r < 4; ++r) v[r] = apply_act(v[r], (act));    \
        }                                                                                   \
    }
__device__ __forceinline__ void consumer_store(const DGemmArgs& g, const float (&v)[4], int fm_raw, int fm, int fn) {
    if (fm_raw >= g.M || fn >= g.N) return;
    if (g.c_frag) {
        uint2 t;
        t.x = pack2bf(v[0], v[1]);
        t.y = pack2bf(v[2], v[3]);
        *reinterpret_cast<uint2*>(reinterpret_cast<bf16_t*>(g.C) + frag_offset(fm, fn, g.N >> 5)) = t;
        return;
    }
    bf16_t* cp = reinterpret_cast<bf16_t*>(g.C) + (size_t)fm * g.ldc + fn;
    if (fn + 3 < g.N && (g.ldc & 3) == 0) {
        uint2 t;
        t.x = pack2bf(v[0], v[1]);
        t.y = pack2bf(v[2], v[3]);
        *reinterpret_cast<uint2*>(cp) = t;
    } else {
        for (int r = 0; r < 4; ++r)
            if (fn + r < g.N) cp[r] = f2bf(v[r]);
    }
}

enum { DEPI_BF16 = 0, DEPI_RES = 1 };

template <int MT, int NW, int EPI>
__global__ __launch_bounds__(64 * NW) void dgemm_kernel(DGemmArgs g) {
    static_assert(NW >= MT, "wave i finishes row tile i: a workgroup needs at least MT waves");
    __shared__ __attribute__((aligned(16))) f32x4_t red[NW][MT][64];

    const int tid = threadIdx.x, lane = tid & 63, wave = tid >> 6;
    const int l15 = lane & 15, lg = lane >> 4;
    const int n0 = blockIdx.x * 16, m0 = blockIdx.y * (16 * MT);

    const bf16_t* __restrict__ X = g.A;
    const bf16_t* __restrict__ W = g.W;

    const bool finisher = wave < MT;
    const int fi = wave;
    const int fm_raw = m0 + fi * 16 + l15;
    const int fm = fm_raw < g.M ? fm_raw : g.M - 1;
    const int fn = n0 + lg * 4;

    RowStatLoads sl;
    bool have_stats = false;
    float4 ep_a = {0.f, 0.f, 0.f, 0.f}, ep_b = ep_a, ep_c = ep_a, ep_d = ep_a;
    if (finisher && !(g.dbg & 8)) {
        ep_a = load_cols4(g.bias, fn, g.N);
        if constexpr (EPI == DEPI_BF16) {
            if (g.stats_in) {
                stats_issue(sl, g.stats_in, g.strips_in, g.M, fm, lg);
                have_stats = true;
                ep_b = load_cols4(g.colsum, fn, g.N);
            }
        } else {
            ep_b = *reinterpret_cast<const float4*>(g.res_x + (size_t)fm * g.N + fn);
            if (g.res_stats) {
                stats_issue(sl, g.res_stats, g.res_strips, g.M, fm, lg);
                have_stats = true;
                ep_c = *reinterpret_cast<const float4*>(g.res_gamma + fn);
                ep_d = *reinterpret_cast<const float4*>(g.res_beta + fn);
            }
        }
    }

    const int ksteps = g.K >> 5;
    const KSlice ks = k_slice(ksteps, NW, wave);

    const bf16_t* wp = W + frag_tile(blockIdx.x, 0, ksteps, lane);
    const bf16_t* xp[MT];
#pragma unroll
    for (int i = 0; i < MT; ++i) xp[i] = X + frag_tile(blockIdx.y * MT + i, 0, ksteps, lane);
    f32x4_t acc[MT];
#pragma unroll
    for (int i = 0; i < MT; ++i) acc[i] = f32x4_t{0.f, 0.f, 0.f, 0.f};

    auto chunk = [&](auto UC, int k0) {
        constexpr int U = decltype(UC)::value;
        bf16x8_t wf[U], xf[U][MT];
#pragma unroll
        for (int u = 0; u < U; ++u) {
            if (g.dbg & 16) wf[u] = *reinterpret_cast<const bf16x8_t*>(wp + (size_t)(k0 + u) * 512);
            else if (!(g.dbg & 2)) wf[u] = __builtin_nontemporal_load(reinterpret_cast<const bf16x8_t*>(wp + (size_t)(k0 + u) * 512));
            else wf[u] = bf16x8_t{1, 1, 1, 1, 1, 1, 1, 1};
#pragma unroll
            for (int i = 0; i < MT; ++i) {
                if (!(g.dbg & 1)) xf[u][i] = *reinterpret_cast<const bf16x8_t*>(xp[i] + (size_t)(k0 + u) * 512);
                else xf[u][i] = bf16x8_t{1, 1, 1, 1, 1, 1, 1, 1};
            }
        }
        if (g.dbg & 4) {
#pragma unroll
            for (int u = 0; u < U; ++u) {
                asm volatile("" ::"v"(wf[u]));
#pragma unroll
                for (int i = 0; i < MT; ++i) asm volatile("" ::"v"(xf[u][i]));
            }
            return;
        }
#pragma unroll
        for (int u = 0; u < U; ++u)
#pragma unroll
            for (int i = 0; i < MT; ++i)
                acc[i] = mfma16(wf[u], xf[u][i], acc[i]);
    };
    constexpr int UBIG = MT >= 4 ? 6 : 12;
    int k = ks.kb;
    for (; k + UBIG <= ks.ke; k += UBIG) chunk(std::integral_constant<int, UBIG>{}, k);
    for (; k + 2 <= ks.ke; k += 2) chunk(std::integral_constant<int, 2>{}, k);
    for (; k < ks.ke; ++k) chunk(std::integral_constant<int, 1>{}, k);

#pragma unroll
    for (int i = 0; i < MT; ++i) red[wave][i][lane] = acc[i];
    __syncthreads();
    if (!finisher) return;
    const f32x4_t tot = sum_waves<NW>(red, fi, lane);

    if constexpr (EPI == DEPI_BF16) {
        float mean = 0.f, rstd = 1.f;
        if (have_stats) stats_finish(sl, g.inv_d, g.eps_in, mean, rstd);
        DGEMM_CONSUMER_FINISH(v, tot, ep_a, ep_b, have_stats, mean, rstd, g.act);
        consumer_store(g, v, fm_raw, fm, fn);
    } else {
        float v[4] = {tot[0], tot[1], tot[2], tot[3]};
        const float biasv[4] = {ep_a.x, ep_a.y, ep_a.z, ep_a.w};
        float res[4] = {ep_b.x, ep_b.y, ep_b.z, ep_b.w};
        if (have_stats) {
            float mean, rstd;
            stats_finish(sl, g.res_inv_d, g.res_eps, mean, rstd);
            const float gm[4] = {ep_c.x, ep_c.y, ep_c.z, ep_c.w}, bt[4] = {ep_d.x, ep_d.y, ep_d.z, ep_d.w};
#pragma unroll
            for (int r = 0; r < 4; ++r) res[r] = (res[r] - mean) * rstd * gm[r] + bt[r];
        }
        float s = 0.f, q = 0.f;
#pragma unroll
        for (int r = 0; r < 4; ++r) {
            v[r] += biasv[r] + res[r];
            s += v[r];
            q += v[r] * v[r];
        }
        s += __shfl_xor(s, 16, 64); q += __shfl_xor(q, 16, 64);
        s += __shfl_xor(s, 32, 64); q += __shfl_xor(q, 32, 64);
        if (fm_raw >= g.M) return;
        *reinterpret_cast<f32x4_t*>(g.x_out + (size_t)fm * g.N + fn) = f32x4_t{v[0], v[1], v[2], v[3]};
        uint2 t;
        t.x = pack2bf(v[0], v[1]);
        t.y = pack2bf(v[2], v[3]);
        *reinterpret_cast<uint2*>(g.xb_out + frag_offset(fm, fn, (g.N + 31) >> 5)) = t;
        if (lg == 0) g.stats_out[(size_t)blockIdx.x * g.M + fm] = float2{s, q};
    }
}

__global__ __launch_bounds__(256) void dgemm_wide_rows_kernel(DGemmArgs g) {
    __shared__ __attribute__((aligned(16))) f32x4_t red[2][4][4][64];

// ... 448 lines not shown
```

generativeimage2text_amd/csrc/launchers.h:

```cpp
#pragma once
#include <hip/hip_runtime.h>
#include <stddef.h>

namespace gitmi {

struct GemmArgs {
    const void* A; const void* W; const float* bias; const float* res; void* C;
    int M, N, K;
    int lda, ldc, ldr;
    int act;
    int tiles_n, nwg;
    int ng;
    int dbg;
    int out_f16;
    int shared;
    const float2* ln_part; int ln_nparts; const float* ln_colsum; float ln_inv_d, ln_eps;
    float2* part_out;
    const float2* res_part; int res_nparts; const float* res_gamma; const float* res_beta; float res_inv_d, res_eps;
};
bool gemm_uses_p8(const GemmArgs& g, bool in_f32, bool out_f32);
hipError_t launch_gemm(const GemmArgs& g, bool in_f32, bool out_f32, hipStream_t s);
hipError_t launch_gemm_p8(GemmArgs g, bool out_f32, hipStream_t s);
bool gemm_p8_supports(const GemmArgs& g);
int gemm_p8_cost(const GemmArgs& g, int bm);
bool set_gemm_impl(int impl);

struct DGemmArgs {
    const unsigned short* A; const unsigned short* W;
    const float* bias;
    const float* colsum;
    const float2* stats_in;
    int strips_in; float inv_d, eps_in;
    void* C;
    int c_frag;
    const float* res_x;
    const float2* res_stats; int res_strips; const float* res_gamma; const float* res_beta; float res_inv_d, res_eps;
    float* x_out; unsigned short* xb_out; float2* stats_out;
    int M, N, K, lda, ldc, act;
    int dbg;
    int rows_per_wg;
    int strips_per_wg;
    int no_row_walk;
};
hipError_t launch_dgemm(const DGemmArgs& g, hipStream_t s);
struct DLn { const float2* stats; int strips; float inv_d, eps; const float* gamma; const float* beta; };
inline DGemmArgs dgemm_ln(const void* A, const void* W, const float* bias, const float* colsum, const DLn* ln, void* C, int c_frag,
                          int act, int M, int N, int K) {
    DGemmArgs g{};
    g.A = (const unsigned short*)A; g.lda = K; g.W = (const unsigned short*)W; g.bias = bias;
    if (ln) { g.colsum = colsum; g.stats_in = ln->stats; g.strips_in = ln->strips; g.inv_d = ln->inv_d; g.eps_in = ln->eps; }
    g.C = C; g.ldc = N; g.c_frag = c_frag; g.act = act; g.M = M; g.N = N; g.K = K;
    return g;
}
inline DGemmArgs dgemm_to_stream(const void* A, const void* W, const float* bias, const float* res_x, const DLn* res_ln, float* x_out,
                                 void* xb_out, float2* stats_out, int M, int N, int K) {
    DGemmArgs g{};
    g.A = (const unsigned short*)A; g.lda = K; g.W = (const unsigned short*)W; g.bias = bias; g.res_x = res_x;
    if (res_ln) {
        g.res_stats = res_ln->stats; g.res_strips = res_ln->strips; g.res_gamma = res_ln->gamma; g.res_beta = res_ln->beta;
        g.res_inv_d = res_ln->inv_d; g.res_eps = res_ln->eps;
    }
    g.x_out = x_out; g.xb_out = (unsigned short*)xb_out; g.stats_out = stats_out; g.M = M; g.N = N; g.K = K;
    return g;
}

struct VocabArgs {
    const unsigned short* A; int lda; const unsigned short* W; const float* bias; const float* colsum;
    const float2* stats_in; int strips_in; float inv_d, eps_in;
    int M, N, K, cols_per_wg;
    const int* ids; int ld_ids, cur_len; const int* plen; int beams, suppress_kind;
    float rep_penalty;
    float* part_val; int* part_idx; float2* part_lse;
    float* logits_out; int ld_logits;
    int max_wgs;
    int nblk;
};
hipError_t launch_vocab_topm(const VocabArgs& g, int mtop, hipStream_t s);
int vocab_parts(int V, int cols_per_wg);
int vocab_mtop_slots(int mtop);

hipError_t launch_layernorm(const float* x, int ldx, const float* gamma, const float* beta, float eps,
                            const float* add_after, void* y_t, int ld_t, bool t_is_f32, float* y_f, int ld_f,
                            int rows, int D, int map_n_in, int map_n_out, int map_off, hipStream_t s);
hipError_t launch_im2col(const float* img, void* out, bool out_f32, int B, int H, int W, int p, int K, int Kpad,
                         hipStream_t s);
hipError_t launch_pos_bicubic(const float* pos, float* out, int g, int gh, int gw, int D, hipStream_t s);
hipError_t launch_ragged_stage(const float* src, float* dst, size_t slot, int4* meta, int* ntok, int B, int p, size_t max_pixels,
                               int Nmax, hipStream_t s);
hipError_t launch_im2col_ragged(const float* stage, size_t slot, const int4* meta, void* out, bool out_f32, int B, int Nmax,
                                int p, int K, int Kpad, hipStream_t s);
hipError_t launch_vit_assemble_ragged(const float* patch_out, const float* cls, const float* pos, int g, const int4* meta,
                                      const float* gamma, const float* beta, float eps, void* X, bool x_f16, int B, int Nmax,
                                      int p, int D, float2* part, hipStream_t s);
hipError_t launch_zero_pad_rows(void* x, bool is_f32, int ld, const int* ntok, int B, int Nmax, hipStream_t s);
hipError_t launch_ragged_report(const int4* meta, const int* image_of, int Q, int nout_per, float* logprob, int* info,
                                int* bad, hipStream_t s);
hipError_t launch_vit_assemble_ln(const float* patch_out, const float* cls, const float* pos, const float* gamma,
                                  const float* beta, float eps, void* X, bool x_f16, int B, int N, int D, float2* part,
                                  int nparts, hipStream_t s);
hipError_t launch_layernorm_s16(const void* x, int ldx, const float* gamma, const float* beta, float eps,
                                const float* add_after, void* y_t, int ld_t, bool t_is_f32, void* y_s, int ld_s,
                                int rows, int D, int map_n_in, int map_n_out, int map_off, hipStream_t s);
hipError_t launch_embed_ln(const int* ids, int ld_ids, int pos, const float* words, const float* positions,
                           const float* gamma, const float* beta, float eps, float* h_f, void* h_t, bool t_is_f32,
                           int R, int D, int vocab, bool frag, hipStream_t s);
hipError_t launch_context_embed(const long long* tokens, int ld, const int4* seg, int Q, const int* cnt, const float* words,
                                const float* positions, const float* gamma, const float* beta, float eps, void* feats, bool t_is_f32,
                                float* feats_f, int* ntok, int B, int n_img, int stride, int D, int vocab, int max_pos, hipStream_t s);
hipError_t launch_frag_pack(const void* src_bf16, void* dst_bf16, int rows, int rows_out, int K, hipStream_t s);
hipError_t launch_convert_pad(const float* src, void* dst, bool dst_f32, size_t rows, int K, int Kpad,
                              hipStream_t s);
hipError_t launch_convert(const void* src, bool src_f32, void* dst, bool dst_f32, size_t n, hipStream_t s);
hipError_t launch_chain_input(const float* x, void* xb_frag, float2* stats, int R, int d, hipStream_t s);
hipError_t launch_copy_f32(const float* src, int lds, float* dst, int ldd, int rows, int cols, hipStream_t s);
hipError_t launch_fill_i32(int* dst, int value, int n, hipStream_t s);

struct AttnFullArgs {
    const void* q; const void* k; const void* v; void* out;
    int ldq, ldk, ldv, ldo;
    int N, H;
    float scale;
    const int* ntok;
};
hipError_t launch_attn_full(const AttnFullArgs& a, int B, bool is_f32, int impl, hipStream_t s);

struct AttnDecodeArgs {
    const void* qkv; const void* img_k; const void* img_v; void* txt_k; void* txt_v; void* out;
    const int* kv_src;
    const int* img_of;
    int ld_src;
    int d;
    int N_img, T_max, pos, beams;
    int N_pad;
    int out_frag;
    float scale;
    int dbg;
    int pairs_per_wg;
    int stream_wgs;
    int waves_per_pair;
    int n_pairs;
    const int* ntok;
};
hipError_t launch_kv_repack(const void* qkv, void* kh, void* vh, int B, int N, int H, int d, hipStream_t s);
hipError_t launch_attn_decode(const AttnDecodeArgs& a, int B, int H, hipStream_t s);
hipError_t launch_kv_repack_frag(const void* qkv, void* kf, void* vt, int B, int N, int N_pad, int H, int d, hipStream_t s);
hipError_t launch_attn_decode_mfma(const AttnDecodeArgs& a, int B, int H, hipStream_t s);

constexpr int SS_NHMAX = 8;
struct SearchState {
    int B, k, pn, T, V, eos, kind;
    int prefixed;
    int sampled;
    double length_penalty;
    double* len_norm;
    const long long* start;
    int ld_start;
    const int* plen;
    int* ids[2];
    int* kv_src[2];
    float* score[2];
    int* done;
    int nh;
    int* hyp_n;
    int* hyp_cnt;
    double* hyp_worst;
    double* hyp_score;
    int* hyp_len;
    int* hyp_seq;
    int* hyp_tok;
    int* stop;
    int* early;
    int* info;
};
struct StepCands {
    const float* part_val; const int* part_idx; const float2* part_lse;
    int nparts, slots;
};
struct EmbedArgs {
    const float* words; const float* positions; const float* gamma; const float* beta; float eps;
    float* h_f; void* h_t; int D, vocab;
    int frag;
};
int row_topm_slots(int M);
hipError_t launch_sample_rows(const float* logits, int ldl, int V, int R, float temperature, int top_k, float top_p,
                              int ndraw, unsigned long long seed, int step, float* part_val, int* part_idx,
                              float2* part_lse, float* filtered_out, const int* ids, int ld_ids, int cur_len,
                              float rep_penalty, int stride, hipStream_t s);
struct TrieArgs {
    const int* child_off; const int* child_tok; const int* child_node;
    int* cursor;
};
hipError_t launch_trie_select(const float* logits, int ldl, int V, const int* ids, int ld_ids, int cur_len, const int* plen,
                              int eos, const TrieArgs& tr, int B, float* part_val, int* part_idx, float2* part_lse,
                              hipStream_t s);
hipError_t launch_row_topm(const float* logits, int ldl, int V, const int* ids, int ld_ids, int cur_len,
                           const int* plen, int beams, int suppress_kind, float rep_penalty, int M, int R,
                           float* part_val, int* part_idx, float2* part_lse, hipStream_t s);
hipError_t launch_search_step(const SearchState& st, int src, int cur_len, const StepCands& in, const EmbedArgs& em,
                              bool t_is_f32, hipStream_t s);
hipError_t launch_search_init(const SearchState& st, hipStream_t s);
hipError_t launch_search_finish(const SearchState& st, int cur, int cur_len, long long* tokens_out,
                                float* logprob_out, int* info_out, int* sent_out, hipStream_t s);
hipError_t launch_search_rows(const SearchState& st, int cur, int cur_len, long long* out, hipStream_t s);
hipError_t launch_fill_start(long long* start, int ld, const long long* prefix, int ldp, int shared, int sos, int B, int P,
                             hipStream_t s);
hipError_t launch_load_ids(const long long* tokens, int R, int t, int* ids, int* kv_src, int ld, hipStream_t s);

hipError_t launch_score_embed_ln(const long long* tokens, int ld, int Q, int Lp, const float* words, const float* positions,
                                 const float* gamma, const float* beta, float eps, float* h_f, void* h_t, bool t_is_f32,
                                 int D, int vocab, int max_pos, hipStream_t s);
hipError_t launch_score_attn(const void* qkv, const void* img_kv, const int* image_of, void* out, int Q, int H, int d,
                             int N_img, int Lp, float scale, bool is_f32, hipStream_t s, const int* ntok = nullptr,
                             float2* stats = nullptr);
hipError_t launch_score_attn_map(const void* qkv, const void* img_kv, const int* image_of, const int* ntok, const float2* stats,
                                 const int* lens, float* out, size_t out_sq, size_t out_sj, int Tc, int Q, int H, int N_img,
                                 int Lp, float scale, bool is_f32, int* bad, hipStream_t s);
int score_head_tiles(int V);
hipError_t launch_score_head(const void* A, int lda, const void* W, const float* bias, const int* tgt, int M, int V, int K,
                             float4* part, float* zt, hipStream_t s);
hipError_t launch_score_rowstats(const float* logits, int ldl, int V, const int* tgt, int row_off, int rows, float4* part,
                                 float* zt, hipStream_t s);
hipError_t launch_score_targets(const long long* tokens, int ld, int Lp, const int* lens, int V, int M, int* tgt,
                                hipStream_t s);
hipError_t launch_score_combine(const float4* part, int ntiles, const float* zt, const int* tgt, int M, int Lp, int ld, int V,
                                float2* out, int* bad, hipStream_t s);
hipError_t launch_score_info(const int* bad, int Q, int ld, int* info, hipStream_t s, int i1 = 0, int i2 = 0);

hipError_t launch_preprocess(const unsigned char* rgb, int H, int W, int crop, unsigned char* tmp, float* out, hipStream_t s);
hipError_t launch_preprocess_batch(const unsigned char* rgb, const long long* desc, int n, int crop, unsigned char* tmp, float* out,
                                   hipStream_t s);
size_t preprocess_batch_workspace(const long long* desc, int n, int crop);
hipError_t launch_resize_crop_norm(const uint8_t* rgb, int H, int W, int nh, int nw, int top, int left, int ch, int cw,
                                   uint8_t* tmp, float* out, hipStream_t s);

}
```

generativeimage2text_amd/engine.py:

```python
from __future__ import annotations

import ctypes as C
import os
from typing import Dict, List, Mapping, Optional, Sequence, Tuple

import torch

_HERE = os.path.dirname(os.path.abspath(__file__))
LIB_PATH = os.path.join(_HERE, "libgitmi.so")
LIB_PATH_F16 = os.path.join(_HERE, "libgitmi_f16.so")
LIB_PATH_EXP = os.path.join(_HERE, "libgitmi_exp.so")
LIB_PATH_F16_EXP = os.path.join(_HERE, "libgitmi_f16_exp.so")

PREC_BF16, PREC_F32 = 0, 1
DTYPE_F32, DTYPE_BF16, DTYPE_F16 = 0, 1, 2
DTYPE_F16_STREAM = 3
SEARCH_AUTOREGRESSIVE, SEARCH_GENERATOR, SEARCH_TRIE = 0, 1, 2
SEARCH_SCORE = 3
SEARCH_ATTEND = 4
SEARCH_CONTEXT = 5
ACT_NONE, ACT_QUICKGELU, ACT_GELU_ERF = 0, 1, 2

EXPORTED_SYMBOLS = [
    "gitmi_abi_version", "gitmi_last_error", "gitmi_create", "gitmi_destroy", "gitmi_load_tensor",
    "gitmi_finalize_weights", "gitmi_encode_frames", "gitmi_prefill", "gitmi_step_logits",
    "gitmi_generate", "gitmi_search_begin", "gitmi_search_rows", "gitmi_search_advance",
    "gitmi_search_finish", "gitmi_profile_enable", "gitmi_profile_read", "gitmi_set_graph",
    "gitmi_op_gemm", "gitmi_op_layernorm", "gitmi_op_attention", "gitmi_op_dgemm", "gitmi_op_dgemm_res",
    "gitmi_op_vocab_topm", "gitmi_clone", "gitmi_op_attn_decode", "gitmi_preprocess_image",
    "gitmi_set_image_shape", "gitmi_preprocess_image_to", "gitmi_generate_prefixed", "gitmi_set_temporal_embedding", "gitmi_op_kv_repack", "gitmi_set_encode_after", "gitmi_op_sample_rows",
    "gitmi_search_done_count", "gitmi_set_trie", "gitmi_operand_dtype", "gitmi_set_shared_device", "gitmi_preprocess_batch",
    "gitmi_set_ln_fold", "gitmi_op_gemm_ln",
]
EXPERIMENT_SYMBOLS = [
    "gitmi_debug_import_stage", "gitmi_debug_head_from", "gitmi_debug_set_gemm_impl", "gitmi_debug_set_dgemm",
    "gitmi_debug_score_attn", "gitmi_debug_score_head", "gitmi_debug_attention_ragged", "gitmi_debug_attn_decode_ragged",
    "gitmi_debug_vocab_topm_rules", "gitmi_debug_search_begin_prefixed", "gitmi_debug_search_advance_lists", "gitmi_debug_read_hidden",
    "gitmi_debug_im2col", "gitmi_debug_pos_resize", "gitmi_debug_vit_assemble", "gitmi_debug_ragged_front", "gitmi_debug_zero_pad_rows",
    "gitmi_debug_layernorm_map", "gitmi_debug_score_attn_map", "gitmi_debug_attn_decode_form", "gitmi_debug_dgemm_form",
    "gitmi_debug_gemm_form", "gitmi_debug_context_embed",
]


class GitmiConfig(C.Structure):
    _fields_ = [(n, C.c_int32) for n in (
        "image_size", "patch", "vit_width", "vit_layers", "vit_heads", "dec_hidden", "dec_layers",
        "dec_heads", "dec_ffn", "vocab", "max_pos", "num_frames", "sos", "eos", "precision",
        "max_batch", "max_beams", "max_frames", "max_text_len", "max_image_pixels", "max_image_tokens")]


class GitmiSearch(C.Structure):
    _fields_ = [("kind", C.c_int32), ("beam_size", C.c_int32), ("per_node_beam_size", C.c_int32),
                ("max_steps", C.c_int32), ("length_penalty", C.c_double),
                ("do_sample", C.c_int32), ("top_k", C.c_int32), ("top_p", C.c_double), ("temperature", C.c_double),
                ("seed", C.c_uint64), ("repetition_penalty", C.c_double),
                ("num_keep_best", C.c_int32), ("reserved_", C.c_int32)]


class GitmiProfile(C.Structure):
    _fields_ = [("vit_ms", C.c_float), ("prefill_ms", C.c_float), ("decode_ms", C.c_float),
                ("total_ms", C.c_float), ("gemm_ms", C.c_float), ("gemm_launches", C.c_int32),
                ("gemm_flops", C.c_double), ("vit_gemm_ms", C.c_float), ("vit_gemm_launches", C.c_int32),
                ("vit_gemm_flops", C.c_double), ("decode_step_ms", C.c_float), ("decode_steps", C.c_int32),
                ("decode_step_bytes", C.c_double)]

    def as_dict(self) -> Dict[str, float]:
        return {n: getattr(self, n) for n, _ in self._fields_}


class GitmiError(RuntimeError):
    pass


_libs: Dict[str, C.CDLL] = {}
_experiment = False
_MEASUREMENT_LIBS = ("exp", "f16_exp")
_gemm_impl = -1


def use_experiment_build(on: bool = True) -> None:
    global _experiment
    _experiment = bool(on)


def load_library(operands: str = "bf16") -> C.CDLL:
    if operands == "bf16" and _experiment:
        operands = "exp"
    if operands in _libs:
        return _libs[operands]
    path = {"bf16": LIB_PATH, "f16": LIB_PATH_F16, "exp": LIB_PATH_EXP, "f16_exp": LIB_PATH_F16_EXP}[operands]
    if not os.path.exists(path):
        raise GitmiError(
            f"{path} not found: build it with `python -c 'import __graft_entry__ as g; g.build()'` "
            f"or `make -C generativeimage2text_amd/csrc`.  There is no CPU fallback.")
    lib = C.CDLL(path)
    vp, i32, i64p, fp = C.c_void_p, C.c_int, C.POINTER(C.c_int64), C.c_void_p
    lib.gitmi_abi_version.restype = C.c_int
    lib.gitmi_last_error.restype = C.c_char_p
    lib.gitmi_create.argtypes = [C.POINTER(GitmiConfig), i32, C.POINTER(vp)]
    lib.gitmi_destroy.argtypes = [vp]
    lib.gitmi_destroy.restype = None
    lib.gitmi_load_tensor.argtypes = [vp, C.c_char_p, vp, i64p, i32, i32]
    lib.gitmi_finalize_weights.argtypes = [vp]
    lib.gitmi_encode_frames.argtypes = [vp, C.POINTER(vp), i32, i32, vp, vp]
    lib.gitmi_prefill.argtypes = [vp, vp]
    lib.gitmi_step_logits.argtypes = [vp, vp, i32, i32, vp, vp]
    lib.gitmi_generate.argtypes = [vp, C.POINTER(vp), i32, i32, vp, i32, C.POINTER(GitmiSearch), vp, vp, vp, vp]
    lib.gitmi_search_begin.argtypes = [vp, C.POINTER(GitmiSearch), i32, vp, i32, i32, vp]
    lib.gitmi_search_rows.argtypes = [vp, vp, C.POINTER(C.c_int), C.POINTER(C.c_int), vp]
    lib.gitmi_search_advance.argtypes = [vp, vp, vp]
    lib.gitmi_search_finish.argtypes = [vp, vp, vp, vp, vp]
    lib.gitmi_search_done_count.argtypes = [vp, C.POINTER(C.c_int), vp]
    lib.gitmi_set_trie.argtypes = [vp, i32, vp, vp, vp]
    lib.gitmi_profile_enable.argtypes = [vp, i32]
    lib.gitmi_profile_read.argtypes = [vp, C.POINTER(GitmiProfile)]
    lib.gitmi_set_graph.argtypes = [vp, i32]
    lib.gitmi_set_temporal_embedding.argtypes = [vp, i32]
    lib.gitmi_set_encode_after.argtypes = [vp, vp]
    lib.gitmi_set_shared_device.argtypes = [vp, i32]
    lib.gitmi_set_ln_fold.argtypes = [vp, i32]
    lib.gitmi_op_gemm.argtypes = [vp, vp, vp, vp, vp, i32, i32, i32, i32, i32, i32, i32, i32, vp]
    lib.gitmi_op_gemm_ln.argtypes = [vp, vp, vp, vp, vp, C.c_float, vp, vp, vp, vp, C.c_float, vp, vp, i32, i32, i32, i32, vp]
    lib.gitmi_op_layernorm.argtypes = [vp, vp, vp, C.c_float, vp, vp, i32, i32, i32, vp]
    lib.gitmi_op_attention.argtypes = [vp, vp, i32, i32, i32, i32, i32, vp]
    lib.gitmi_op_dgemm.argtypes = [vp, vp, vp, vp, vp, i32, C.c_float, vp, i32, i32, i32, i32, i32, i32, vp]
    lib.gitmi_op_dgemm_res.argtypes = [vp, vp, vp, vp, vp, i32, vp, vp, C.c_float, vp, vp, vp, i32, i32, i32, vp]
    lib.gitmi_op_vocab_topm.argtypes = [vp, vp, vp, vp, vp, i32, C.c_float, i32, i32, i32, i32, i32, vp, vp, vp, vp, vp, i32, vp]
    lib.gitmi_generate_prefixed.argtypes = [vp, C.POINTER(vp), i32, i32, vp, i32, C.POINTER(C.c_int32), C.POINTER(C.c_int32),
                                            i32, C.POINTER(GitmiSearch), vp, vp, vp, vp, vp]
    lib.gitmi_clone.argtypes = [vp, C.POINTER(vp)]
    lib.gitmi_preprocess_image.argtypes = [vp, i32, i32, i32, vp, C.c_size_t, vp, vp]
    lib.gitmi_preprocess_image_to.argtypes = [vp, i32, i32, i32, i32, vp, C.c_size_t, vp, vp]
    lib.gitmi_preprocess_batch.argtypes = [vp, C.c_size_t, i64p, i32, i32, vp, C.c_size_t, vp, vp]
    lib.gitmi_set_image_shape.argtypes = [vp, i32, i32, vp]
    lib.gitmi_op_attn_decode.argtypes = [vp, vp, vp, vp, vp, vp, vp, i32, i32, i32, i32, i32, i32, i32, i32, vp]
    lib.gitmi_op_kv_repack.argtypes = [vp, vp, vp, i32, i32, i32, vp]
    lib.gitmi_op_sample_rows.argtypes = [vp, i32, i32, C.c_float, i32, C.c_float, i32, C.c_uint64, i32, vp, vp, vp, vp]
    if operands in _MEASUREMENT_LIBS:
        lib.gitmi_debug_import_stage.argtypes = [vp, vp, i32, vp]
        lib.gitmi_debug_head_from.argtypes = [vp, vp, i32, vp, vp]
        lib.gitmi_debug_set_gemm_impl.argtypes = [i32]
        lib.gitmi_debug_set_dgemm.argtypes = [i32]
        lib.gitmi_debug_dgemm_form.argtypes = [vp, i32, vp, vp, vp, vp, i32, C.c_float, vp, i32, i32, vp, vp, i32, vp, vp, C.c_float,
                                               vp, vp, vp, i32, i32, i32, i32, i32, i32, vp]
        lib.gitmi_debug_gemm_form.argtypes = [vp, i32, vp, vp, vp, i32, vp, i32, i32, i32, i32, i32, i32, i32, i32, vp, vp, C.c_float,
                                              vp, vp, vp, vp, C.c_float, vp]
        lib.gitmi_debug_score_attn.argtypes = [vp, vp, vp, vp, i32, i32, i32, i32, i32, vp]
        lib.gitmi_debug_score_head.argtypes = [vp, vp, vp, vp, i32, i32, i32, i32, vp, vp]
        lib.gitmi_debug_score_attn_map.argtypes = [vp, vp, vp, vp, vp, i32, i32, i32, i32, i32, vp]
        lib.gitmi_debug_attention_ragged.argtypes = [vp, vp, vp, i32, i32, i32, i32, i32, vp]
        lib.gitmi_debug_attn_decode_ragged.argtypes = [vp, vp, vp, vp, vp, vp, vp, vp, i32, i32, i32, i32, i32, i32, i32, vp]
        lib.gitmi_debug_attn_decode_form.argtypes = [vp, vp, vp, vp, vp, vp, vp, vp, vp, i32, i32, i32, i32, i32, i32, i32, i32, i32,
                                                     i32, i32, i32, vp]
        lib.gitmi_debug_vocab_topm_rules.argtypes = [vp, vp, vp, vp, vp, i32, C.c_float, i32, i32, i32, i32, i32, vp, i32, i32, vp, i32,
                                                     i32, C.c_float, vp, vp, vp, vp, i32, vp]
        lib.gitmi_debug_search_begin_prefixed.argtypes = [vp, C.POINTER(GitmiSearch), i32, vp, i32, vp, i32, vp]
        lib.gitmi_debug_search_advance_lists.argtypes = [vp, vp, vp, vp, i32, i32, i32, vp]
        lib.gitmi_debug_read_hidden.argtypes = [vp, i32, vp, vp, C.POINTER(C.c_int), C.POINTER(C.c_int), vp]
        lib.gitmi_debug_im2col.argtypes = [vp, vp, i32, i32, i32, i32, i32, i32, i32, vp]
        lib.gitmi_debug_pos_resize.argtypes = [vp, vp, i32, i32, i32, i32, vp]
        lib.gitmi_debug_vit_assemble.argtypes = [vp, vp, vp, vp, vp, C.c_float, vp, i32, i32, i32, i32, vp, vp]
        lib.gitmi_debug_ragged_front.argtypes = [i32, vp, vp, vp, vp, vp, i32, vp, vp, vp, i32, vp, vp, C.c_float, vp, i32, vp, i32, i32,
                                                 C.c_longlong, i32, i32, i32, i32, vp]
        lib.gitmi_debug_zero_pad_rows.argtypes = [vp, i32, i32, vp, i32, i32, vp]
        lib.gitmi_debug_layernorm_map.argtypes = [vp, i32, vp, vp, C.c_float, vp, vp, i32, vp, i32, i32, i32, i32, i32, vp]
        lib.gitmi_debug_context_embed.argtypes = [vp, i32, vp, vp, i32, vp, i32, vp, i32, vp, vp, C.c_float, vp, i32, vp, vp, i32, i32,
                                                  i32, i32, vp]
    for name in EXPORTED_SYMBOLS + (EXPERIMENT_SYMBOLS if operands in _MEASUREMENT_LIBS else []):
        if name not in ("gitmi_last_error", "gitmi_destroy"):
            getattr(lib, name).restype = C.c_int
    if lib.gitmi_abi_version() != 10:
        raise GitmiError("libgitmi.so ABI version mismatch")
    lib.gitmi_operand_dtype.restype = C.c_int
    if lib.gitmi_operand_dtype() != {"bf16": DTYPE_BF16, "f16": DTYPE_F16, "exp": DTYPE_BF16, "f16_exp": DTYPE_F16}[operands]:
        raise GitmiError(f"{path} was not built for {operands} operands")
    if operands in _MEASUREMENT_LIBS and _gemm_impl != -1:
        _ck(lib.gitmi_debug_set_gemm_impl(_gemm_impl), lib)
    _libs[operands] = lib
    return lib


def _experiment_only(lib, name: str):
    try:
        return getattr(lib, name)
    except AttributeError:
        raise GitmiError(f"{name} is exported by the measurement build only (libgitmi_exp.so, libgitmi_f16_exp.so): call "
                         f"generativeimage2text_amd.engine.use_experiment_build() before creating the engine") from None


def _ck(rc: int, lib=None) -> None:
    if rc != 0:
        libs = [lib] if lib is not None else list(_libs.values())
        msgs = [m for m in ((l.gitmi_last_error() or b"").decode("utf-8", "replace") for l in libs) if m]
        raise GitmiError(" | ".join(msgs) or "gitmi call failed")


def _stream() -> int:
    return int(torch.cuda.current_stream().cuda_stream)


def _ptr(t: Optional[torch.Tensor]) -> Optional[int]:
    return None if t is None else int(t.data_ptr())


def _torch_dtype_code(t: torch.Tensor) -> int:
    return {torch.float32: DTYPE_F32, torch.bfloat16: DTYPE_BF16, torch.float16: DTYPE_F16}[t.dtype]


_OPERAND_LIBS = {torch.bfloat16: "bf16", torch.float16: "f16"}


def _op_library(*dtypes: torch.dtype, fp32_ok: bool = False) -> C.CDLL:
    dts = set(dtypes) - {torch.float32}
    if not dts and fp32_ok:
        return load_library()
    if len(dts) != 1 or next(iter(dts)) not in _OPERAND_LIBS:
        raise GitmiError(f"operands must all be bf16 or all fp16, got {sorted(str(d) for d in dts) or ['float32']}")
    return load_library(_OPERAND_LIBS[dts.pop()])


def _exp_library(*dtypes: torch.dtype, operands: Optional[str] = None) -> C.CDLL:
    if operands is None:
        dts = set(dtypes) - {torch.float32}
        if len(dts) > 1 or not dts <= set(_OPERAND_LIBS):
            raise GitmiError(f"operands must all be bf16 or all fp16, got {sorted(str(d) for d in dts)}")
        operands = _OPERAND_LIBS[dts.pop()] if dts else "bf16"
    if operands not in ("bf16", "f16"):
        raise GitmiError(f"operands={operands!r}: bf16 or f16")
    return load_library("f16_exp" if operands == "f16" and _experiment else operands)


RAGGED_DESC_BYTES = 256


def id_table(rows: Sequence[Sequence[int]]) -> torch.Tensor:
    table = torch.zeros(len(rows), max(len(r) for r in rows), dtype=torch.int64)
    for q, r in enumerate(rows):
        table[q, :len(r)] = torch.as_tensor(list(r), dtype=torch.int64)
    return table


def _sentence_tables(lens: Sequence[int], image_of: Optional[Sequence[int]]):
    Q = len(lens)
    return (C.c_int32 * Q)(*lens), None if image_of is None else (C.c_int32 * Q)(*[int(i) for i in image_of])


class Geometry(tuple):

    def __new__(cls, Nk: int, F: int, grids, image_rows: Optional[int] = None, context: Optional[Sequence[int]] = None):
        self = super().__new__(cls, (int(Nk), int(F), list(grids)))
        self.image_rows = int(Nk if image_rows is None else image_rows)
        self.context = [0] * len(self[2]) if context is None else [int(v) for v in context]
        return self

    @property
    def stride(self) -> int:
        return self[0]


def context_segments(context, B: int, vocab: int, max_pos: int):
    segments, image_of = [], []
    for i, seg in enumerate(context or []):
        tokens = torch.as_tensor(seg["tokens"]).detach().to("cpu", torch.int64)
        length = torch.as_tensor(seg["length"]).detach().to("cpu", torch.int64).reshape(-1)
        if tokens.dim() != 2 or int(tokens.shape[0]) != B or int(length.numel()) != B:
            raise ValueError(f"context[{i}]: 'tokens' must be [B, Lc] and 'length' [B] for the {B} images of the batch, got "
                             f"{tuple(tokens.shape)} and {tuple(length.shape)}")
        Lc = int(tokens.shape[1])
        for b in range(B):
            n = int(length[b])
            if n < 0 or n > Lc:
                raise ValueError(f"context[{i}]: length {n} of image {b} outside [0, {Lc}]")
            if n > max_pos:
                raise ValueError(f"context[{i}]: a segment of {n} tokens exceeds the {max_pos} positions of the textual embedding")
            if n == 0:
                continue
            ids = tokens[b, :n].tolist()
            if min(ids) < 0 or max(ids) >= vocab:
                raise ValueError(f"context[{i}]: token ids of image {b} outside [0, {vocab})")
            segments.append(ids)
            image_of.append(b)
    return segments, image_of


def context_capacity(image_size: int, patch: int, max_image_tokens: int, max_frames: int, max_context: int) -> int:
    if max_context <= 0:
        return int(max_image_tokens)
    n_nat = (int(image_size) // int(patch)) ** 2 + 1
    return max(n_nat, int(max_image_tokens)) + -(-int(max_context) // max(1, int(max_frames)))


class RaggedImages:

    def __init__(self, buffer: torch.Tensor, shapes: Sequence[Tuple[int, int]]):
        self.buffer, self.shapes = buffer, [tuple(int(v) for v in hw) for hw in shapes]

    def __len__(self) -> int:
        return len(self.shapes)


def pack_ragged(images: Sequence[torch.Tensor], patch: int, max_pixels: int, max_tokens: int, max_batch: int,
                device=None) -> RaggedImages:
    images = list(images)
    B = len(images)
    if not 1 <= B <= max_batch:
        raise ValueError(f"{B} images: a ragged call takes 1 .. max_batch={max_batch}")
# ... 654 lines not shown
                  res_x=None, res_stats=None, res_gamma=None, res_beta=None, res_eps: float = 1e-12, x=None, xb=None,
                  stats_out=None, packed: bool = False, rows_per_wg: int = 0, strips_per_wg: int = 0, no_row_walk: int = 0):
    lib = _exp_library(A.dtype, W.dtype)
    own = A.dtype
    if own == torch.float32:
        raise GitmiError(f"operands must be bf16 or fp16, got {A.dtype} / {W.dtype}")
    if packed:
        if M is None:
            raise ValueError("packed operands: M is required")
        Af, Wf = A, W
    else:
        M = int(A.shape[0]) if M is None else int(M)
        Af, Wf = to_frag(A, 64), to_frag(W)
    M, N, K = int(M), int(bias.numel()), int(A.shape[1])
    Mp = (M + 15) // 16 * 16
    producer = res_x is not None
    if producer:
        x = torch.empty(M, N, device=A.device, dtype=torch.float32) if x is None else x
        xb = torch.empty(Mp, (N + 31) // 32 * 32, device=A.device, dtype=own) if xb is None else xb
        stats_out = torch.empty(N // 16, M, 2, device=A.device, dtype=torch.float32) if stats_out is None else stats_out
    elif out is None:
        out = torch.empty(Mp if frag_out else M, N, device=A.device, dtype=own)
    _ck(_experiment_only(lib, "gitmi_debug_dgemm_form")(
        Af.data_ptr(), int(Af.shape[0]), Wf.data_ptr(), _ptr(bias), _ptr(colsum), _ptr(stats),
        0 if stats is None else int(stats.shape[0]), eps, _ptr(out), int(bool(frag_out)), int(act), _ptr(res_x), _ptr(res_stats),
        0 if res_stats is None else int(res_stats.shape[0]), _ptr(res_gamma), _ptr(res_beta), res_eps, _ptr(x), _ptr(xb),
        _ptr(stats_out), M, N, K, int(rows_per_wg), int(strips_per_wg), int(no_row_walk), _stream()), lib)
    return (x, xb, stats_out) if producer else out


def _vocab_head_call(A, W, bias, mtop, cols_per_wg, colsum, stats, want_logits, packed, rows, V, measurement=False):
    lib = _exp_library(A.dtype, W.dtype) if measurement else _op_library(A.dtype, W.dtype)
    K = A.shape[1]
    V = int(bias.numel()) if V is None else int(V)
    if packed:
        Af, Wf, M, bp, cp = A, W, int(rows), bias, colsum
    else:
        M = A.shape[0]
        Vp = (V + cols_per_wg - 1) // cols_per_wg * cols_per_wg
        Af, Wf, bp, cp = to_frag(A, 64), to_frag(W, cols_per_wg), _pad_vec(bias, Vp), _pad_vec(colsum, Vp)
    nparts = (V + cols_per_wg - 1) // cols_per_wg
    slots = 1 if mtop <= 1 else 2 if mtop <= 2 else 4 if mtop <= 4 else 8 if mtop <= 8 else 16
    pv = torch.empty(M, nparts, slots, device=A.device, dtype=torch.float32)
    pi = torch.empty(M, nparts, slots, device=A.device, dtype=torch.int32)
    pl = torch.empty(M, nparts, 2, device=A.device, dtype=torch.float32)
    lg = torch.empty(M, V, device=A.device, dtype=torch.float32) if want_logits else None
    strips = 0 if stats is None else int(stats.shape[0])
    keep = (Af, Wf, bp, cp)
    return lib, M, (Af.data_ptr(), Wf.data_ptr(), bp.data_ptr(), _ptr(cp), _ptr(stats), strips), (M, V, K, cols_per_wg, mtop), \
        (pv.data_ptr(), pi.data_ptr(), pl.data_ptr(), _ptr(lg)), (pv, pi, pl, lg), keep


def op_vocab_topm(A: torch.Tensor, W: torch.Tensor, bias: torch.Tensor, mtop: int, cols_per_wg: int = 128,
                  colsum: Optional[torch.Tensor] = None, stats: Optional[torch.Tensor] = None, eps: float = 1e-12,
                  suppress_tok: Optional[torch.Tensor] = None, want_logits: bool = False, packed: bool = False,
                  rows: Optional[int] = None, V: Optional[int] = None, max_wgs: int = 0):
    lib, _, ops, shape, outs, result, keep = _vocab_head_call(A, W, bias, mtop, cols_per_wg, colsum, stats, want_logits, packed, rows, V)
    _ck(lib.gitmi_op_vocab_topm(*ops, eps, *shape, _ptr(suppress_tok), *outs, int(max_wgs), _stream()), lib)
    return result


def op_vocab_topm_rules(A: torch.Tensor, W: torch.Tensor, bias: torch.Tensor, mtop: int, ids: Optional[torch.Tensor],
                        cur_len: int, plen: Optional[torch.Tensor], beams: int = 1, suppress_kind: int = 0,
                        rep_penalty: float = 0.0, cols_per_wg: int = 128, colsum: Optional[torch.Tensor] = None,
                        stats: Optional[torch.Tensor] = None, eps: float = 1e-12, want_logits: bool = False, packed: bool = False,
                        rows: Optional[int] = None, V: Optional[int] = None, max_wgs: int = 0):
    lib, M, ops, shape, outs, result, keep = _vocab_head_call(A, W, bias, mtop, cols_per_wg, colsum, stats, want_logits, packed, rows, V,
                                                              measurement=True)
    if ids is not None:
        ids = ids.to(device=A.device, dtype=torch.int32).contiguous()
        plen = plen.to(device=A.device, dtype=torch.int32).contiguous()
        if ids.dim() != 2 or ids.shape[0] != M or plen.numel() * beams != M:
            raise ValueError(f"ids {tuple(ids.shape)} / plen {tuple(plen.shape)} do not describe {M} rows of {beams} beams")
    _ck(_experiment_only(lib, "gitmi_debug_vocab_topm_rules")(
        *ops, eps, *shape, _ptr(ids), 0 if ids is None else int(ids.shape[1]), int(cur_len), _ptr(plen), int(beams),
        int(suppress_kind), float(rep_penalty), *outs, int(max_wgs), _stream()), lib)
    return result


def set_gemm_impl(impl: int) -> None:
    global _gemm_impl
    lib = load_library()
    _ck(_experiment_only(lib, "gitmi_debug_set_gemm_impl")(int(impl)), lib)
    _gemm_impl = int(impl)
    other = _libs.get("f16_exp")
    if other is not None and other is not lib:
        _ck(other.gitmi_debug_set_gemm_impl(int(impl)), other)


def op_attn_decode(qkv, img_k, img_v, txt_k, txt_v, kv_src, B, H, N_img, T_max, pos, beams, dbg=0):
    lib = _op_library(qkv.dtype, img_k.dtype, img_v.dtype, txt_k.dtype, txt_v.dtype, fp32_ok=True)
    R, d = B * beams, H * 64
    out = torch.empty(R, d, device=qkv.device, dtype=qkv.dtype)
    if qkv.dtype != torch.float32 and img_k.dim() == 4:
        img_k, img_v = kv_repack(img_k, img_v)
    _ck(lib.gitmi_op_attn_decode(qkv.data_ptr(), img_k.data_ptr(), img_v.data_ptr(), txt_k.data_ptr(), txt_v.data_ptr(),
                                 kv_src.data_ptr(), out.data_ptr(), B, H, N_img, T_max, pos, beams, _torch_dtype_code(qkv),
                                 dbg, _stream()), lib)
    return out


def op_attention_ragged(qkv: torch.Tensor, ntok, B: int, N: int, H: int, impl: int) -> torch.Tensor:
    lib = load_library()
    nt = torch.as_tensor(ntok, dtype=torch.int32).to(qkv.device)
    out = torch.empty(B * N, H * 64, device=qkv.device, dtype=qkv.dtype)
    _ck(_experiment_only(lib, "gitmi_debug_attention_ragged")(qkv.data_ptr(), out.data_ptr(), nt.data_ptr(), B, N, H,
                                                              _torch_dtype_code(qkv), impl, _stream()), lib)
    return out


def op_attn_decode_ragged(qkv, img_k, img_v, txt_k, txt_v, kv_src, ntok, B, H, N_img, T_max, pos, beams):
    lib = load_library()
    R, d = B * beams, H * 64
    nt = torch.as_tensor(ntok, dtype=torch.int32).to(qkv.device)
    out = torch.empty(R, d, device=qkv.device, dtype=qkv.dtype)
    if qkv.dtype != torch.float32 and img_k.dim() == 4:
        img_k, img_v = kv_repack(img_k, img_v)
    _ck(_experiment_only(lib, "gitmi_debug_attn_decode_ragged")(qkv.data_ptr(), img_k.data_ptr(), img_v.data_ptr(), txt_k.data_ptr(),
                                                                txt_v.data_ptr(), kv_src.data_ptr(), out.data_ptr(), nt.data_ptr(), B,
                                                                H, N_img, T_max, pos, beams, _torch_dtype_code(qkv), _stream()), lib)
    return out


def op_attn_decode_form(qkv, img_k, img_v, txt_k, txt_v, kv_src, B, H, N_img, T_max, pos, beams, *, out=None, img_of=None,
                        ntok=None, out_frag=False, pairs_per_wg=0, waves_per_pair=0, stream_wgs=0, operands=None):
    lib = _exp_library(qkv.dtype, img_k.dtype, img_v.dtype, txt_k.dtype, txt_v.dtype,
                       operands=operands if qkv.dtype == torch.float32 else None)
    R, d = B * beams, H * 64
    n_images = img_k.shape[0] if img_k.dim() == 4 else img_k.numel() // (H * ((N_img + 31) // 32 * 32) * 64)
    if qkv.dtype != torch.float32 and img_k.dim() == 4:
        img_k, img_v = kv_repack(img_k, img_v)
    if img_of is None:
        if n_images < B:
            raise ValueError(f"{n_images} images for {B} sentences and no img_of")
    else:
        host = torch.as_tensor(img_of, dtype=torch.int64).cpu()
        if host.numel() != B or int(host.min()) < 0 or int(host.max()) >= n_images:
            raise ValueError(f"img_of {host.tolist()} does not map {B} sentences onto {n_images} images")
        img_of = host.to(device=qkv.device, dtype=torch.int32)
    if ntok is not None:
        ntok = torch.as_tensor(ntok, dtype=torch.int32).to(qkv.device)
        if ntok.numel() != n_images:
            raise ValueError(f"ntok holds {ntok.numel()} counts for {n_images} images")
    if out is None:
        rows = (R + 15) // 16 * 16 if out_frag else R
        out = torch.empty(rows, d, device=qkv.device, dtype=qkv.dtype)
    _ck(_experiment_only(lib, "gitmi_debug_attn_decode_form")(
        qkv.data_ptr(), img_k.data_ptr(), img_v.data_ptr(), txt_k.data_ptr(), txt_v.data_ptr(), kv_src.data_ptr(), out.data_ptr(),
        _ptr(ntok), _ptr(img_of), n_images, B, H, N_img, T_max, pos, beams, _torch_dtype_code(qkv), int(bool(out_frag)),
        int(pairs_per_wg), int(waves_per_pair), int(stream_wgs), _stream()), lib)
    return out


def op_score_attn(qkv: torch.Tensor, img_kv: torch.Tensor, image_of: torch.Tensor, Q: int, H: int, N_img: int,
                  Lp: int) -> torch.Tensor:
    lib = load_library()
    img = image_of.to(device=qkv.device, dtype=torch.int32).contiguous()
    out = torch.empty(Q * Lp, H * 64, device=qkv.device, dtype=qkv.dtype)
    _ck(_experiment_only(lib, "gitmi_debug_score_attn")(qkv.data_ptr(), img_kv.data_ptr(), img.data_ptr(), out.data_ptr(), Q, H,
                                                        N_img, Lp, _torch_dtype_code(qkv), _stream()), lib)
    return out


def op_score_attn_map(qkv: torch.Tensor, img_kv: torch.Tensor, image_of: torch.Tensor, Q: int, H: int, N_img: int, Lp: int,
                      ntok: Optional[torch.Tensor] = None) -> torch.Tensor:
    lib = load_library()
    img = image_of.to(device=qkv.device, dtype=torch.int32).contiguous()
    nt = None if ntok is None else ntok.to(device=qkv.device, dtype=torch.int32).contiguous()
    out = torch.empty(Q, Lp, N_img + Lp, device=qkv.device, dtype=torch.float32)
    _ck(_experiment_only(lib, "gitmi_debug_score_attn_map")(qkv.data_ptr(), img_kv.data_ptr(), img.data_ptr(), _ptr(nt),
                                                            out.data_ptr(), Q, H, N_img, Lp, _torch_dtype_code(qkv), _stream()), lib)
    return out


def op_score_head(A: torch.Tensor, W: torch.Tensor, bias: torch.Tensor, tgt: torch.Tensor) -> torch.Tensor:
    lib = load_library()
    M, K = A.shape
    V = W.shape[0]
    t = tgt.to(device=A.device, dtype=torch.int32).contiguous()
    out = torch.zeros(M, 2, device=A.device, dtype=torch.float32)
    _ck(_experiment_only(lib, "gitmi_debug_score_head")(A.data_ptr(), W.data_ptr(), bias.float().contiguous().data_ptr(),
                                                        t.data_ptr(), M, V, K, _torch_dtype_code(A), out.data_ptr(),
                                                        _stream()), lib)
    return out


def _front(name: str, *dtypes: torch.dtype, operands: Optional[str] = None):
    lib = _exp_library(*dtypes, operands=operands)
    return lib, _experiment_only(lib, name)


def op_im2col(img: torch.Tensor, out: torch.Tensor, B: int, H: int, W: int, p: int, Kpad: int, operands: Optional[str] = None) -> None:
    lib, fn = _front("gitmi_debug_im2col", out.dtype, operands=operands)
    _ck(fn(img.data_ptr(), out.data_ptr(), _torch_dtype_code(out), B, H, W, p, 3 * p * p, Kpad, _stream()), lib)


def op_pos_resize(pos: torch.Tensor, out: torch.Tensor, g: int, gh: int, gw: int, operands: Optional[str] = None) -> None:
    lib, fn = _front("gitmi_debug_pos_resize", operands=operands)
    _ck(fn(pos.data_ptr(), out.data_ptr(), g, gh, gw, int(pos.shape[1]), _stream()), lib)


def op_vit_assemble(patch_out: torch.Tensor, cls: torch.Tensor, pos: torch.Tensor, gamma: torch.Tensor, beta: torch.Tensor,
                    eps: float, X: torch.Tensor, B: int, N: int, part: Optional[torch.Tensor] = None,
                    operands: Optional[str] = None) -> None:
    lib, fn = _front("gitmi_debug_vit_assemble", operands=operands)
    _ck(fn(patch_out.data_ptr(), cls.data_ptr(), pos.data_ptr(), gamma.data_ptr(), beta.data_ptr(), eps, X.data_ptr(),
           1 if X.dtype == torch.float16 else 0, B, N, int(cls.numel()), _ptr(part), _stream()), lib)


def op_ragged_front(stage: int, B: int, p: int, max_pixels: int, Nmax: int, *, src=None, slots=None, meta=None, ntok=None,
                    patches=None, Kpad: int = 0, patch_out=None, cls=None, pos=None, g: int = 0, gamma=None, beta=None,
                    eps: float = 1e-5, X=None, part=None, operands: Optional[str] = None) -> None:
    lib, fn = _front("gitmi_debug_ragged_front", *(() if patches is None else (patches.dtype,)), operands=operands)
    _ck(fn(int(stage), _ptr(src), _ptr(slots), _ptr(meta), _ptr(ntok), _ptr(patches),
           DTYPE_F32 if patches is None else _torch_dtype_code(patches), _ptr(patch_out), _ptr(cls), _ptr(pos), int(g), _ptr(gamma),
           _ptr(beta), eps, _ptr(X), 1 if X is not None and X.dtype == torch.float16 else 0, _ptr(part), B, p, int(max_pixels), Nmax,
           3 * p * p, int(Kpad), 0 if cls is None else int(cls.numel()), _stream()), lib)


def op_zero_pad_rows(x: torch.Tensor, ntok: torch.Tensor, B: int, Nmax: int, ld: int, operands: Optional[str] = None) -> None:
    lib, fn = _front("gitmi_debug_zero_pad_rows", operands=operands)
    _ck(fn(x.data_ptr(), 1 if x.dtype == torch.float32 else 0, ld, ntok.data_ptr(), B, Nmax, _stream()), lib)


def op_layernorm_map(x: torch.Tensor, gamma: torch.Tensor, beta: torch.Tensor, eps: float, add_after: Optional[torch.Tensor],
                     y_t: Optional[torch.Tensor], y_s: Optional[torch.Tensor], rows: int, D: int, map_n_in: int = 0,
                     map_n_out: int = 0, map_off: int = 0, operands: Optional[str] = None) -> None:
    lib, fn = _front("gitmi_debug_layernorm_map", *(() if y_t is None else (y_t.dtype,)), operands=operands)
    _ck(fn(x.data_ptr(), 1 if x.dtype == torch.float16 else 0, gamma.data_ptr(), beta.data_ptr(), eps, _ptr(add_after), _ptr(y_t),
           DTYPE_F32 if y_t is None else _torch_dtype_code(y_t), _ptr(y_s), rows, D, map_n_in, map_n_out, map_off, _stream()), lib)


def op_sample_rows(logits: torch.Tensor, temperature: float = 1.0, top_k: int = 0, top_p: float = 1.0, ndraw: int = 2,
                   seed: int = 0, step: int = 1, want_filtered: bool = True):
    lib = load_library()
    logits = logits.float().contiguous()
    R, V = logits.shape
    lp = torch.empty(R, ndraw, device=logits.device, dtype=torch.float32)
    tok = torch.empty(R, ndraw, device=logits.device, dtype=torch.int32)
    filt = torch.empty(R, V, device=logits.device, dtype=torch.float32) if want_filtered else None
    _ck(lib.gitmi_op_sample_rows(logits.data_ptr(), R, V, float(temperature), int(top_k), float(top_p), int(ndraw), int(seed),
                                 int(step), lp.data_ptr(), tok.data_ptr(), _ptr(filt), _stream()), lib)
    return filt, tok, lp


def kv_repack(img_k: torch.Tensor, img_v: torch.Tensor):
    lib = _op_library(img_k.dtype, img_v.dtype)
    B, H, N, _ = img_k.shape
    d = H * 64
    rows = torch.zeros(B * N, 3 * d, device=img_k.device, dtype=img_k.dtype)
    rows[:, d:2 * d] = img_k.permute(0, 2, 1, 3).reshape(B * N, d)
    rows[:, 2 * d:] = img_v.permute(0, 2, 1, 3).reshape(B * N, d)
    Np = (N + 31) // 32 * 32
    kf = torch.empty(B * H * Np * 64, device=img_k.device, dtype=img_k.dtype)
    vt = torch.empty(B * H * Np * 64, device=img_k.device, dtype=img_k.dtype)
    _ck(lib.gitmi_op_kv_repack(rows.data_ptr(), kf.data_ptr(), vt.data_ptr(), B, N, H, _stream()), lib)
    return kf, vt


def preprocess_image(rgb_hwc: torch.Tensor, crop: int = 224) -> torch.Tensor:
    lib = load_library()
    assert rgb_hwc.is_cuda and rgb_hwc.dtype == torch.uint8 and rgb_hwc.dim() == 3 and rgb_hwc.shape[2] == 3
    rgb_hwc = rgb_hwc.contiguous()
    H, W = int(rgb_hwc.shape[0]), int(rgb_hwc.shape[1])
    nw = crop if W <= H else int(crop * W / H)
    tmp = torch.empty(H * nw * 3, dtype=torch.uint8, device=rgb_hwc.device)
    out = torch.empty(3, crop, crop, dtype=torch.float32, device=rgb_hwc.device)
    _ck(lib.gitmi_preprocess_image(rgb_hwc.data_ptr(), H, W, crop, tmp.data_ptr(), tmp.numel(), out.data_ptr(), _stream()), lib)
    return out


def preprocess_image_to(rgb_hwc: torch.Tensor, out_h: int, out_w: int) -> torch.Tensor:
    lib = load_library()
    assert rgb_hwc.is_cuda and rgb_hwc.dtype == torch.uint8 and rgb_hwc.dim() == 3 and rgb_hwc.shape[2] == 3
    rgb_hwc = rgb_hwc.contiguous()
    H, W = int(rgb_hwc.shape[0]), int(rgb_hwc.shape[1])
    tmp = torch.empty(H * out_w * 3, dtype=torch.uint8, device=rgb_hwc.device)
    out = torch.empty(3, out_h, out_w, dtype=torch.float32, device=rgb_hwc.device)
    _ck(lib.gitmi_preprocess_image_to(rgb_hwc.data_ptr(), H, W, int(out_h), int(out_w), tmp.data_ptr(), tmp.numel(),
                                      out.data_ptr(), _stream()), lib)
    return out


def preprocess_batch(staging: torch.Tensor, desc: Sequence[Tuple[int, int, int]], crop: int = 224) -> torch.Tensor:
    lib = load_library()
    assert staging.is_cuda and staging.dtype == torch.uint8 and staging.is_contiguous()
    n = len(desc)
    table = (C.c_int64 * (3 * n))(*[int(v) for d in desc for v in d])
    need = 0
    for _, H, W in desc:
        nw = crop if W <= H else int(crop * W / H)
        if nw != W:
            need += (H * nw * 3 + 63) // 64 * 64
    tmp = torch.empty(max(need, 64), dtype=torch.uint8, device=staging.device)
    out = torch.empty(n, 3, crop, crop, dtype=torch.float32, device=staging.device)
    _ck(lib.gitmi_preprocess_batch(staging.data_ptr(), staging.numel(), table, n, int(crop), tmp.data_ptr(), tmp.numel(),
                                   out.data_ptr(), _stream()), lib)
    return out
```

include/gitmi_experiment.h:

```cpp
#ifndef GITMI_EXPERIMENT_H_
#define GITMI_EXPERIMENT_H_
#include "gitmi.h"
#ifdef __cplusplus
extern "C" {
#endif

int  gitmi_debug_import_stage(gitmi_engine* dst, gitmi_engine* src, int stage, void* stream);
int  gitmi_debug_head_from(gitmi_engine* dst, gitmi_engine* src, int R, float* logits_out, void* stream);

int  gitmi_debug_set_gemm_impl(int impl);

int  gitmi_debug_set_dgemm(int dbg);

int  gitmi_debug_dgemm_form(const void* A, int a_rows, const void* W, const float* bias, const float* colsum, const float* stats,
                            int strips, float eps, void* C, int c_frag, int act, const float* res_x, const float* res_stats,
                            int res_strips, const float* res_gamma, const float* res_beta, float res_eps, float* x_out,
                            void* xb_out, float* stats_out, int M, int N, int K, int rows_per_wg, int strips_per_wg,
                            int no_row_walk, void* stream);

int  gitmi_debug_gemm_form(const void* A, int lda, const void* W, const float* bias, const void* res, int ldr, void* C, int ldc,
                           int M, int N, int K, int act, int in_dtype, int out_dtype, int shared, const float* ln_part,
                           const float* colsum, float ln_eps, float* part_out, const float* res_part, const float* res_gamma,
                           const float* res_beta, float res_eps, void* stream);

int  gitmi_debug_score_attn(const void* qkv, const void* img_kv, const int* image_of, void* out, int Q, int H, int N_img, int Lp,
                            int dtype, void* stream);
int  gitmi_debug_score_attn_map(const void* qkv, const void* img_kv, const int* image_of, const int* ntok, float* out, int Q, int H,
                                int N_img, int Lp, int dtype, void* stream);
int  gitmi_debug_score_head(const void* A, const void* W, const float* bias, const int* tgt, int M, int V, int K, int dtype,
                            float* out, void* stream);

int  gitmi_debug_attention_ragged(const void* qkv, void* out, const int* ntok, int B, int N, int H, int dtype, int impl, void* stream);
int  gitmi_debug_attn_decode_ragged(const void* qkv, const void* img_k, const void* img_v, void* txt_k, void* txt_v,
                                    const int* kv_src, void* out, const int* ntok, int B, int H, int N_img, int T_max, int pos,
                                    int beams, int dtype, void* stream);
int  gitmi_debug_attn_decode_form(const void* qkv, const void* img_k, const void* img_v, void* txt_k, void* txt_v,
                                  const int* kv_src, void* out, const int* ntok, const int* img_of, int n_images, int B, int H,
                                  int N_img, int T_max, int pos, int beams, int dtype, int out_frag, int pairs_per_wg,
                                  int waves_per_pair, int stream_wgs, void* stream);

int  gitmi_debug_vocab_topm_rules(const void* A, const void* W, const float* bias, const float* colsum, const float* stats,
                                  int strips, float eps, int M, int V, int K, int cols_per_wg, int mtop, const int* ids, int ld_ids,
                                  int cur_len, const int* plen, int beams, int suppress_kind, float rep_penalty, float* part_val,
                                  int* part_idx, float* part_lse, float* logits_out, int max_wgs, void* stream);
int  gitmi_debug_search_begin_prefixed(gitmi_engine* e, const gitmi_search* sp, int B, const int64_t* start_host, int ld,
                                       const int32_t* plen_host, int vocab, void* stream);
int  gitmi_debug_search_advance_lists(gitmi_engine* e, const float* part_val, const int* part_idx, const float* part_lse,
                                      int nparts, int slots, int embed, void* stream);
int  gitmi_debug_read_hidden(gitmi_engine* e, int R, float* hf_out, void* ht_out, int* ht_frag, int* ht_dtype, void* stream);

int  gitmi_debug_im2col(const float* img, void* out, int out_dtype, int B, int H, int W, int p, int K, int Kpad, void* stream);
int  gitmi_debug_pos_resize(const float* pos, float* out, int g, int gh, int gw, int D, void* stream);
int  gitmi_debug_vit_assemble(const float* patch_out, const float* cls, const float* pos, const float* gamma, const float* beta,
                              float eps, void* X, int x_f16, int B, int N, int D, float* part, void* stream);
int  gitmi_debug_ragged_front(int stage, const float* src, float* slots, int* meta, int* ntok, void* patches, int patches_dtype,
                              const float* patch_out, const float* cls, const float* pos, int g, const float* gamma,
                              const float* beta, float eps, void* X, int x_f16, float* part, int B, int p, long long max_pixels,
                              int Nmax, int K, int Kpad, int D, void* stream);
int  gitmi_debug_zero_pad_rows(void* x, int is_f32, int ld, const int* ntok, int B, int Nmax, void* stream);
int  gitmi_debug_layernorm_map(const void* x, int src_f16, const float* gamma, const float* beta, float eps, const float* add_after,
                               void* y_t, int out_dtype, void* y_s, int rows, int D, int map_n_in, int map_n_out, int map_off,
                               void* stream);

int  gitmi_debug_context_embed(const int64_t* tokens, int ld, const int32_t* len_host, const int32_t* image_of_host, int Q,
                               const float* words, int vocab, const float* positions, int max_pos, const float* gamma,
                               const float* beta, float eps, void* feats, int dtype, float* feats_f32, int* ntok, int B, int n_img,
                               int stride, int D, void* stream);

#ifdef __cplusplus
}
#endif
#endif
```

Baseline: 11380 captions/s.

## Fuse decoder QKV projection into the attention decode kernel

Adds an attention-decode kernel form that computes the LayerNorm-folded QKV projection for its own pairs inside the kernel, replacing the separate QKV dgemm launch in the chained fp16 decode path. It is meant to remove one kernel launch per decoder layer per step and the round-trip of the QKV activations through global memory. The fused form is used only for greedy, non-ragged, non-streaming batches with 8 pairs per workgroup, so heads may redundantly recompute or load weight slices and occupancy may differ. Shared dgemm helpers are moved into a common header so both kernels can use them.

```diff
diff --git a/generativeimage2text_amd/csrc/abi_ops.hip b/generativeimage2text_amd/csrc/abi_ops.hip
--- a/generativeimage2text_amd/csrc/abi_ops.hip
+++ b/generativeimage2text_amd/csrc/abi_ops.hip
@@ -340,6 +340,42 @@
     }
     a.N_pad = round_up(N_img, 32);
     HIPCK(launch_attn_decode_mfma(a, B, H, (hipStream_t)stream));
+    return 0;
+}
+GITMI_EXP_EXPORT int gitmi_debug_attn_decode_qkv(const void* x, int x_rows, const void* w, const float* bias, const float* colsum,
+                                                 const float* stats, int strips, float eps, const void* img_k, const void* img_v,
+                                                 void* txt_k, void* txt_v, const int* kv_src, void* out, const int* ntok,
+                                                 const int* img_of, int n_images, int B, int H, int N_img, int T_max, int pos,
+                                                 int beams, int dtype, int out_frag, int pairs_per_wg, int waves_per_pair,
+                                                 int stream_wgs, void* stream) {
+    RCK(check_dtype("debug_attn_decode_qkv", "dtype", dtype));
+    if (dtype == GITMI_DTYPE_F32) return fail("debug_attn_decode_qkv: 16-bit operands only (the f32 mode keeps its QKV launch)");
+    if (!x || !w || !bias || !img_k || !img_v || !txt_k || !txt_v || !kv_src || !out) return fail("debug_attn_decode_qkv: null argument");
+    if (n_images < 1) return fail("debug_attn_decode_qkv: n_images=%d", n_images);
+    if (B < 1 || H < 1 || N_img < 1 || pos < 0 || pos >= T_max)
+        return fail("debug_attn_decode_qkv: B=%d H=%d N_img=%d pos=%d T_max=%d", B, H, N_img, pos, T_max);
+    if (beams != 1) return fail("debug_attn_decode_qkv: beams=%d (beam batches keep the QKV launch)", beams);
+    if (ntok) return fail("debug_attn_decode_qkv: ntok (ragged batches keep the QKV launch)");
+    if (waves_per_pair == 2) return fail("debug_attn_decode_qkv: waves_per_pair=2 (two-wave pairs keep the QKV launch)");
+    if (stream_wgs != 0) return fail("debug_attn_decode_qkv: stream_wgs=%d (the streaming form keeps the QKV launch)", stream_wgs);
+    if (pairs_per_wg != 8) return fail("debug_attn_decode_qkv: pairs_per_wg=%d (the form packs 8 pairs)", pairs_per_wg);
+    if (round_up(N_img, 32) > 256) return fail("debug_attn_decode_qkv: N_img=%d (more than 256 padded keys: the two-wave form)", N_img);
+    if (H * 64 > 768) return fail("debug_attn_decode_qkv: hidden=%d > 768", H * 64);
+    if (x_rows < round_up(B, 16)) return fail("debug_attn_decode_qkv: x_rows=%d, but B=%d rows are loaded as %d", x_rows, B, round_up(B, 16));
+    if (stats) {
+        if (!colsum) return fail("debug_attn_decode_qkv: stats without colsum");
+        if (strips < 1 || strips > 64) return fail("debug_attn_decode_qkv: strips=%d outside [1, 64]", strips);
+    }
+    AttnDecodeArgs a{};
+    a.img_k = img_k; a.img_v = img_v; a.txt_k = txt_k; a.txt_v = txt_v; a.out = out;
+    a.kv_src = kv_src; a.ld_src = T_max; a.d = H * 64; a.N_img = N_img; a.T_max = T_max; a.pos = pos; a.beams = beams;
+    a.scale = 0.125f; a.img_of = img_of; a.out_frag = out_frag; a.pairs_per_wg = pairs_per_wg; a.waves_per_pair = waves_per_pair;
+    a.N_pad = round_up(N_img, 32);
+    const DLn ln{(const float2*)stats, strips, 1.0f / (float)a.d, eps, nullptr, nullptr};
+    const DGemmArgs g = dgemm_ln(x, w, bias, colsum, stats ? &ln : nullptr, nullptr, 0, 0, B, 3 * a.d, a.d);
+    attn_decode_set_qkv(a, g);
+    if (!attn_decode_qkv_form(a, B, H)) return fail("debug_attn_decode_qkv: not a launch of the form");
+    HIPCK(launch_attn_decode_qkv(a, B, H, (hipStream_t)stream));
     return 0;
 }
 GITMI_EXP_EXPORT int gitmi_debug_attn_decode_ragged(const void* qkv, const void* img_k, const void* img_v, void* txt_k, void* txt_v,
diff --git a/generativeimage2text_amd/csrc/dgemm_shared.h b/generativeimage2text_amd/csrc/dgemm_shared.h
--- /dev/null
+++ b/generativeimage2text_amd/csrc/dgemm_shared.h
@@ -0,0 +1,115 @@
+#pragma once
+#include "gitmi_common.h"
+
+namespace gitmi {
+
+constexpr int STRIP_SLOTS = 16;
+
+struct RowStatLoads {
+    float2 v[STRIP_SLOTS];
+};
+__device__ __forceinline__ void stats_issue(RowStatLoads& L, const float2* __restrict__ stats, int strips, int M,
+                                            int row, int lg) {
+#pragma unroll
+    for (int u = 0; u < STRIP_SLOTS; ++u) {
+        const int sidx = lg + 4 * u;
+        L.v[u] = sidx < strips ? stats[(size_t)sidx * M + row] : float2{0.f, 0.f};
+    }
+}
+__device__ __forceinline__ void stats_issue_nb(RowStatLoads& L, const float2* __restrict__ stats, int strips, int M,
+                                               int row, int lg) {
+#pragma unroll
+    for (int u = 0; u < STRIP_SLOTS; ++u) {
+        const int sidx = lg + 4 * u;
+        const float2 v = stats[(size_t)min(sidx, strips - 1) * M + row];
+        L.v[u] = sidx < strips ? v : float2{0.f, 0.f};
+    }
+}
+__device__ __forceinline__ void stats_finish(const RowStatLoads& L, float inv_d, float eps, float& mean, float& rstd) {
+    float s = 0.f, q = 0.f;
+#pragma unroll
+    for (int u = 0; u < STRIP_SLOTS; ++u) { s += L.v[u].x; q += L.v[u].y; }
+    s += __shfl_xor(s, 16, 64); q += __shfl_xor(q, 16, 64);
+    s += __shfl_xor(s, 32, 64); q += __shfl_xor(q, 32, 64);
+    mean = s * inv_d;
+    const float var = fmaxf(q * inv_d - mean * mean, 0.f);
+    rstd = rsqrtf(var + eps);
+}
+
+
+struct KSlice { int kb, ke; };
+__device__ __forceinline__ KSlice k_slice(int ksteps, int nw, int wave) {
+    const int per = (ksteps + nw - 1) / nw;
+    const int kb = wave * per;
+    return KSlice{kb, min(kb + per, ksteps)};
+}
+
+__device__ __forceinline__ float4 load_cols4(const float* p, int n, int N) {
+    float4 r;
+    r.x = p[n < N ? n : N - 1];
+    r.y = p[n + 1 < N ? n + 1 : N - 1];
+    r.z = p[n + 2 < N ? n + 2 : N - 1];
+    r.w = p[n + 3 < N ? n + 3 : N - 1];
+    return r;
+}
+
+constexpr int DW_KS = 6;
+struct WSlice { bf16x8_t f[DW_KS]; };
+template <bool NT = true>
+__device__ __forceinline__ WSlice load_w_slice(const bf16_t* W, int strip, KSlice ks, int ksteps, int lane) {
+    WSlice w;
+    const bf16_t* wp = W + frag_tile(strip, 0, ksteps, lane);
+#pragma unroll
+    for (int u = 0; u < DW_KS; ++u)
+        w.f[u] = ks.kb + u >= ks.ke ? bf16x8_t{0, 0, 0, 0, 0, 0, 0, 0}
+                 : NT ? __builtin_nontemporal_load(reinterpret_cast<const bf16x8_t*>(wp + (size_t)(ks.kb + u) * 512))
+                      : *reinterpret_cast<const bf16x8_t*>(wp + (size_t)(ks.kb + u) * 512);
+    return w;
+}
+template <int MT>
+__device__ __forceinline__ void load_x_slice(bf16x8_t (&xf)[DW_KS][MT], const bf16_t* X, int rt0, KSlice ks, int ksteps, int lane) {
+#pragma unroll
+    for (int u = 0; u < DW_KS; ++u)
+#pragma unroll
+        for (int i = 0; i < MT; ++i)
+            xf[u][i] = ks.kb + u < ks.ke ? *reinterpret_cast<const bf16x8_t*>(X + frag_tile(rt0 + i, ks.kb + u, ksteps, lane))
+                                         : bf16x8_t{0, 0, 0, 0, 0, 0, 0, 0};
+}
+template <int MT>
+__device__ __forceinline__ void mfma_slice(f32x4_t (&acc)[MT], const WSlice& w, const bf16x8_t (&xf)[DW_KS][MT], KSlice ks) {
+#pragma unroll
+    for (int u = 0; u < DW_KS; ++u) {
+        if (ks.kb + u < ks.ke) {
+#pragma unroll
+            for (int i = 0; i < MT; ++i) acc[i] = mfma16(w.f[u], xf[u][i], acc[i]);
+        }
+    }
+}
+
+template <int NW, int MT>
+__device__ __forceinline__ f32x4_t sum_waves(f32x4_t (*red)[MT][64], int tile, int lane) {
+    f32x4_t tot = {0.f, 0.f, 0.f, 0.f};
+#pragma unroll
+    for (int w = 0; w < NW; ++w) {
+        const f32x4_t t = red[w][tile][lane];
+        tot[0] += t[0]; tot[1] += t[1]; tot[2] += t[2]; tot[3] += t[3];
+    }
+    return tot;
+}
+
+#define DGEMM_CONSUMER_FINISH(v, tot, bias4, cs4, have_stats, mean, rstd, act)              \
+    float v[4] = {(tot)[0], (tot)[1], (tot)[2], (tot)[3]};                                  \
+    {                                                                                       \
+        const float biasv[4] = {(bias4).x, (bias4).y, (bias4).z, (bias4).w};                \
+        if (have_stats) {                                                                   \
+            const float cs[4] = {(cs4).x, (cs4).y, (cs4).z, (cs4).w};                       \
+            _Pragma("unroll") for (int r = 0; r < 4; ++r) v[r] = (rstd) * (v[r] - (mean) * cs[r]) + biasv[r]; \
+        } else {                                                                            \
+            _Pragma("unroll") for (int r = 0; r < 4; ++r) v[r] += biasv[r];                 \
+        }                                                                                   \
+        if ((act) != GITMI_ACT_NONE) {                                                      \
+            _Pragma("unroll") for (int r = 0; r < 4; ++r) v[r] = apply_act(v[r], (act));    \
+        }                                                                                   \
+    }
+
+}
diff --git a/generativeimage2text_amd/csrc/engine.hip b/generativeimage2text_amd/csrc/engine.hip
--- a/generativeimage2text_amd/csrc/engine.hip
+++ b/generativeimage2text_amd/csrc/engine.hip
@@ -452,11 +452,6 @@
         const DLn ln_prev{e->stats_o, d / 16, 1.0f / (float)d, 1e-12f, Lp ? Lp->lnog : nullptr, Lp ? Lp->lnob : nullptr};
         const DLn ln_a{e->stats_a, d / 16, 1.0f / (float)d, 1e-12f, L.lnag, L.lnab};
         const DLn* ln_o = Lp ? &ln_prev : nullptr;
-        if (chain) {
-            if (!GITMI_SKIPPED(e, 2)) RCK(dgemm(e, s, dgemm_ln(l == 0 ? e->d_ht : e->xo_b, L.qkv_f, ln_o, e->d_qkv, 0, 0, R, 3 * d, d)));
-        } else {
-            RCK(gemm(e, s, e->d_ht, d, L.wqkv, L.bqkv, nullptr, 0, e->d_qkv, 3 * d, e->pol.f32, R, 3 * d, d, 0, TAG_GEMM_OTHER));
-        }
         AttnDecodeArgs a{};
         a.qkv = e->d_qkv; a.img_k = e->img_kh[l]; a.img_v = e->img_vh[l]; a.txt_k = e->txt_k[l]; a.txt_v = e->txt_v[l]; a.out = e->d_ctx;
         a.kv_src = kv_src; a.ld_src = ld_ids; a.d = d; a.N_img = e->cur_Nimg; a.T_max = c.max_text_len;
@@ -470,7 +465,17 @@
         const bool stream_ok = !e->pol.shared_device && a.N_pad <= 8 * 32 && B * c.dec_heads >= 384 && e->pol.attn_nh != 2;
         a.stream_wgs = e->pol.attn_stream >= 0 ? e->pol.attn_stream : stream_ok ? 192 : 0;
         if (e->keyed) { a.ntok = e->rg_ntok; a.stream_wgs = 0; }
+        bool qkv_inside = false;
+        if (chain) {
+            const DGemmArgs g = dgemm_ln(l == 0 ? e->d_ht : e->xo_b, L.qkv_f, ln_o, e->d_qkv, 0, 0, R, 3 * d, d);
+            attn_decode_set_qkv(a, g);
+            qkv_inside = !GITMI_SKIPPED(e, ~0) && !e->pol.dgemm_dbg && attn_decode_qkv_form(a, B, c.dec_heads) && attn_decode_pairs_per_wg(a, B, c.dec_heads) == 8;
+            if (!qkv_inside && !GITMI_SKIPPED(e, 2) && !GITMI_SKIPPED(e, 16)) RCK(dgemm(e, s, g));
+        } else {
+            RCK(gemm(e, s, e->d_ht, d, L.wqkv, L.bqkv, nullptr, 0, e->d_qkv, 3 * d, e->pol.f32, R, 3 * d, d, 0, TAG_GEMM_OTHER));
+        }
         if (e->pol.f32) HIPCK(launch_attn_decode(a, B, c.dec_heads, s));
+        else if (qkv_inside) HIPCK(launch_attn_decode_qkv(a, B, c.dec_heads, s));
         else if (!GITMI_SKIPPED(e, 1)) HIPCK(launch_attn_decode_mfma(a, B, c.dec_heads, s));
         if (chain) {
             if (!GITMI_SKIPPED(e, 4))
diff --git a/generativeimage2text_amd/csrc/kernels_attn_decode.hip b/generativeimage2text_amd/csrc/kernels_attn_decode.hip
--- a/generativeimage2text_amd/csrc/kernels_attn_decode.hip
+++ b/generativeimage2text_amd/csrc/kernels_attn_decode.hip
@@ -1,5 +1,6 @@
 #include "gitmi_common.h"
 #include "launchers.h"
+#include "dgemm_shared.h"
 #include <algorithm>
 #include <type_traits>
 
@@ -52,12 +53,22 @@
     bool on;
 };
 
+struct QkvSrc {
+    const bf16_t* q0;
+    int row_stride, part;
+    __device__ __forceinline__ const bf16_t* q(int j) const { return q0 + (size_t)j * row_stride; }
+    __device__ __forceinline__ const bf16_t* k(int j) const { return q(j) + part; }
+    __device__ __forceinline__ const bf16_t* v(int j) const { return q(j) + 2 * part; }
+};
+__device__ __forceinline__ QkvSrc qkv_rows(const AttnDecodeArgs& a, const Pair& p) {
+    return QkvSrc{reinterpret_cast<const bf16_t*>(a.qkv) + (size_t)p.row0 * (3 * a.d) + p.h * HD, 3 * a.d, a.d};
+}
+
 template <int KB>
-__device__ __forceinline__ void load_text_kv(const AttnDecodeArgs& a, const Pair& p, int j, int s, int sub, u32x4_t& kr, u32x4_t& vr) {
+__device__ __forceinline__ void load_text_kv(const AttnDecodeArgs& a, const Pair& p, const QkvSrc& qs, int j, int s, int sub, u32x4_t& kr, u32x4_t& vr) {
     if (s == a.pos) {
-        const bf16_t* src = reinterpret_cast<const bf16_t*>(a.qkv) + (size_t)(p.row0 + j) * (3 * a.d) + a.d + p.h * HD + sub * 8;
-        kr = *reinterpret_cast<const u32x4_t*>(src);
-        vr = *reinterpret_cast<const u32x4_t*>(src + a.d);
+        kr = *reinterpret_cast<const u32x4_t*>(qs.k(j) + sub * 8);
+        vr = *reinterpret_cast<const u32x4_t*>(qs.v(j) + sub * 8);
     } else {
         const int srow = KB == 1 ? p.row0 : a.kv_src[(size_t)(p.row0 + j) * a.ld_src + s];
         const size_t off = ((size_t)srow * a.T_max + s) * a.d + p.h * HD + sub * 8;
@@ -70,7 +81,7 @@
 struct TextItems {
     int j[TI];
     u32x4_t kr[TI], vr[TI];
-    __device__ __forceinline__ void load(const AttnDecodeArgs& a, const Pair& p, int grp, int ngrp, int sub) {
+    __device__ __forceinline__ void load(const AttnDecodeArgs& a, const Pair& p, const QkvSrc& qs, int grp, int ngrp, int sub) {
         const int nt = a.pos + 1;
 #pragma unroll
         for (int u = 0; u < TI; ++u) {
@@ -79,27 +90,26 @@
             const int s = it < a.beams * nt ? it % nt : 0;
             kr[u] = u32x4_t{0u, 0u, 0u, 0u};
             vr[u] = kr[u];
-            if (j[u] >= 0) load_text_kv<KB>(a, p, j[u], s, sub, kr[u], vr[u]);
+            if (j[u] >= 0) load_text_kv<KB>(a, p, qs, j[u], s, sub, kr[u], vr[u]);
         }
     }
 };
 
-__device__ __forceinline__ void append_text_cache(const AttnDecodeArgs& a, const Pair& p, int t, int sub) {
+__device__ __forceinline__ void append_text_cache(const AttnDecodeArgs& a, const Pair& p, const QkvSrc& qs, int t, int sub) {
     if (p.on && t < a.beams * 8) {
         const int j = t >> 3;
-        const bf16_t* src = reinterpret_cast<const bf16_t*>(a.qkv) + (size_t)(p.row0 + j) * (3 * a.d) + a.d + p.h * HD + sub * 8;
         const size_t dst = ((size_t)(p.row0 + j) * a.T_max + a.pos) * a.d + p.h * HD + sub * 8;
-        *reinterpret_cast<u32x4_t*>(reinterpret_cast<bf16_t*>(a.txt_k) + dst) = *reinterpret_cast<const u32x4_t*>(src);
-        *reinterpret_cast<u32x4_t*>(reinterpret_cast<bf16_t*>(a.txt_v) + dst) = *reinterpret_cast<const u32x4_t*>(src + a.d);
-    }
-}
-
-__device__ __forceinline__ void load_q_frag(const AttnDecodeArgs& a, const Pair& p, int l15, int lg, bf16x8_t (&qf)[2]) {
+        *reinterpret_cast<u32x4_t*>(reinterpret_cast<bf16_t*>(a.txt_k) + dst) = *reinterpret_cast<const u32x4_t*>(qs.k(j) + sub * 8);
+        *reinterpret_cast<u32x4_t*>(reinterpret_cast<bf16_t*>(a.txt_v) + dst) = *reinterpret_cast<const u32x4_t*>(qs.v(j) + sub * 8);
+    }
+}
+
+__device__ __forceinline__ void load_q_frag(const AttnDecodeArgs& a, const Pair& p, const QkvSrc& qs, int l15, int lg, bf16x8_t (&qf)[2]) {
 #pragma unroll
     for (int ds = 0; ds < 2; ++ds) {
         float qv[8] = {0.f, 0.f, 0.f, 0.f, 0.f, 0.f, 0.f, 0.f};
         if (p.on && l15 < a.beams)
-            ld8bf(reinterpret_cast<const bf16_t*>(a.qkv) + (size_t)(p.row0 + l15) * (3 * a.d) + p.h * HD + ds * 32 + lg * 8, qv);
+            ld8bf(qs.q(l15) + ds * 32 + lg * 8, qv);
         u32x4_t t;
 #pragma unroll
         for (int e = 0; e < 4; ++e) t[e] = pack2bf(qv[2 * e] * a.scale, qv[2 * e + 1] * a.scale);
@@ -171,7 +181,7 @@
 template <int KB>
 struct TextPartial {
     float q[KB][8], m[KB], l[KB], o[KB][8];
-    __device__ __forceinline__ void init(const AttnDecodeArgs& a, const Pair& p, int sub) {
+    __device__ __forceinline__ void init(const AttnDecodeArgs& a, const Pair& p, const QkvSrc& qs, int sub) {
 #pragma unroll
         for (int j = 0; j < KB; ++j) {
             m[j] = -INFINITY;
@@ -179,7 +189,7 @@
 #pragma unroll
             for (int e = 0; e < 8; ++e) { q[j][e] = 0.f; o[j][e] = 0.f; }
             if (p.on && j < a.beams) {
-                ld8bf(reinterpret_cast<const bf16_t*>(a.qkv) + (size_t)(p.row0 + j) * (3 * a.d) + p.h * HD + sub * 8, q[j]);
+                ld8bf(qs.q(j) + sub * 8, q[j]);
 #pragma unroll
                 for (int e = 0; e < 8; ++e) q[j][e] *= a.scale;
             }
@@ -216,12 +226,12 @@
         }
     }
     template <int TI>
-    __device__ __forceinline__ void tail(const AttnDecodeArgs& a, const Pair& p, int grp, int ngrp, int sub) {
+    __device__ __forceinline__ void tail(const AttnDecodeArgs& a, const Pair& p, const QkvSrc& qs, int grp, int ngrp, int sub) {
         if (!p.on) return;
         const int nt = a.pos + 1;
         for (int it = grp + ngrp * TI; it < a.beams * nt; it += ngrp) {
             u32x4_t kr, vr;
-            load_text_kv<KB>(a, p, it / nt, it % nt, sub, kr, vr);
+            load_text_kv<KB>(a, p, qs, it / nt, it % nt, sub, kr, vr);
             item(it / nt, kr, vr);
         }
     }
@@ -340,11 +350,12 @@
     load_chunk(half);
 
     const int t = tid % PT, grp = t >> 3, sub = tid & 7;
+    const QkvSrc qs = qkv_rows(a, p);
     TextItems<KB, TI> ti;
-    ti.load(a, p, grp, 8 * NH, sub);
-    append_text_cache(a, p, t, sub);
+    ti.load(a, p, qs, grp, 8 * NH, sub);
+    append_text_cache(a, p, qs, t, sub);
     bf16x8_t qf[2];
-    load_q_frag(a, p, l15, lg, qf);
+    load_q_frag(a, p, qs, l15, lg, qf);
 
     ImagePartial ip;
     ip.init();
@@ -377,9 +388,9 @@
     }
     ip.finish();
     TextPartial<KB> tp;
-    tp.init(a, p, sub);
+    tp.init(a, p, qs, sub);
     tp.items(ti, !(a.dbg & 2));
-    tp.template tail<TI>(a, p, grp, 8 * NH, sub);
+    tp.template tail<TI>(a, p, qs, grp, 8 * NH, sub);
     tp.merge_groups();
     ip.publish(part[hp][half], k, l15, lg);
     if constexpr (NH > 1) __syncthreads(); else __builtin_amdgcn_wave_barrier();
@@ -387,6 +398,159 @@
     if constexpr (NH > 1) __syncthreads(); else __builtin_amdgcn_wave_barrier();
     if constexpr (NH == 1) write_rows(a, p, part[hp][0], t, PT);
     else write_rows(a, p, part[hp][0], part[hp][NH - 1], t, PT);
+}
+
+constexpr int AQ_PW = 8;
+constexpr int AQ_STRIPS = 3 * HD / 16;
+
+__device__ __forceinline__ void attn_lds_barrier() {
+    asm volatile("s_waitcnt lgkmcnt(0)" ::: "memory");
+    __builtin_amdgcn_s_barrier();
+    asm volatile("" ::: "memory");
+}
+
+template <int TI>
+__global__ __launch_bounds__(64 * AQ_PW) void attn_decode_qkv_kernel(AttnDecodeArgs a) {
+    constexpr int KB = 1;
+    __shared__ __attribute__((aligned(16))) f32x4_t red[AQ_STRIPS][4][1][64];
+    __shared__ __attribute__((aligned(16))) bf16_t rows[AQ_PW][3 * HD];
+    __shared__ float part[AQ_PW][KB][HD + 2];
+
+    const int tid = threadIdx.x, lane = tid & 63;
+    const int wave = __builtin_amdgcn_readfirstlane(tid >> 6);
+    const int l15 = lane & 15, lg = lane >> 4;
+    const int H = a.d / HD, B = a.n_pairs / H;
+    const int Np = a.N_pad, nsteps = Np >> 5;
+    const int nsb = (B + AQ_PW - 1) / AQ_PW, total = H * nsb, per = (total + 7) >> 3;
+    const int blk = (int)(blockIdx.x & 7) * per + (int)(blockIdx.x >> 3);
+    if (blk >= total) return;
+    const int b0 = (blk % nsb) * AQ_PW;
+    Pair p;
+    p.h = blk / nsb;
+    p.on = b0 + wave < B;
+    const int b = p.on ? b0 + wave : 0;
+    p.row0 = b;
+    const int bi = a.img_of ? a.img_of[b] : b;
+    const bf16_t* Kf = reinterpret_cast<const bf16_t*>(a.img_k) + ((size_t)bi * H + p.h) * Np * HD;
+    const bf16_t* Vt = reinterpret_cast<const bf16_t*>(a.img_v) + ((size_t)bi * H + p.h) * Np * HD;
+    const int nimg_steps = p.on ? nsteps : 0;
+
+    bf16x8_t kq[ACS][2][2], vq[ACS][4];
+    auto load_k = [&](int s0) {
+#pragma unroll
+        for (int c = 0; c < ACS; ++c) {
+            const bool on = s0 + c < nimg_steps;
+            const bf16_t* kp = Kf + frag_tile(2 * (s0 + c), 0, 2, lane);
+#pragma unroll
+            for (int t = 0; t < 2; ++t)
+#pragma unroll
+                for (int ds = 0; ds < 2; ++ds)
+                    kq[c][t][ds] = !on ? bf16x8_t{0, 0, 0, 0, 0, 0, 0, 0}
+                                       : __builtin_nontemporal_load(reinterpret_cast<const bf16x8_t*>(kp + (t * 2 + ds) * 512));
+        }
+    };
+    auto load_v = [&](int s0) {
+#pragma unroll
+        for (int c = 0; c < ACS; ++c) {
+            const bool on = s0 + c < nimg_steps;
+            const bf16_t* vp = Vt + ((size_t)(s0 + c) * 4 * 64 + lane) * 8;
+#pragma unroll
+            for (int dt = 0; dt < 4; ++dt)
+                vq[c][dt] = !on ? bf16x8_t{0, 0, 0, 0, 0, 0, 0, 0}
+                                : __builtin_nontemporal_load(reinterpret_cast<const bf16x8_t*>(vp + dt * 512));
+        }
+    };
+    load_k(0);
+
+    const int ksteps = a.d >> 5, N = 3 * a.d;
+    const int slice = wave & 3;
+    const KSlice ks = k_slice(ksteps, 4, slice);
+    const int rt = b0 >> 4;
+    auto strip_of = [&](int ls) { return (ls >> 2) * (a.d >> 4) + p.h * 4 + (ls & 3); };
+    bf16x8_t xf[DW_KS][1];
+    load_x_slice(xf, reinterpret_cast<const bf16_t*>(a.x), rt, ks, ksteps, lane);
+#pragma unroll 2
+    for (int u = 0; u < AQ_STRIPS / 2; ++u) {
+        const int ls = (wave >> 2) * (AQ_STRIPS / 2) + u;
+        const WSlice wf = load_w_slice<false>(reinterpret_cast<const bf16_t*>(a.w), strip_of(ls), ks, ksteps, lane);
+        f32x4_t acc[1] = {f32x4_t{0.f, 0.f, 0.f, 0.f}};
+        mfma_slice(acc, wf, xf, ks);
+        red[ls][slice][0][lane] = acc[0];
+    }
+    load_v(0);
+    const int fm_raw = rt * 16 + l15;
+    const int fm = fm_raw < a.M ? fm_raw : a.M - 1;
+    const bool second = wave + AQ_PW < AQ_STRIPS;
+    const int fn0 = strip_of(wave) * 16 + lg * 4, fn1 = strip_of(second ? wave + AQ_PW : wave) * 16 + lg * 4;
+    RowStatLoads sl;
+    if (a.stats_in) stats_issue(sl, a.stats_in, a.strips_in, a.M, fm, lg);
+    const float4 bias4[2] = {load_cols4(a.bias, fn0, N), load_cols4(a.bias, fn1, N)};
+    float4 cs4[2] = {float4{0.f, 0.f, 0.f, 0.f}, float4{0.f, 0.f, 0.f, 0.f}};
+    if (a.stats_in) { cs4[0] = load_cols4(a.colsum, fn0, N); cs4[1] = load_cols4(a.colsum, fn1, N); }
+    attn_lds_barrier();
+    {
+#pragma clang fp contract(fast)
+        float mean = 0.f, rstd = 1.f;
+        if (a.stats_in) stats_finish(sl, a.inv_d, a.eps_in, mean, rstd);
+        const int i = l15 - (b0 & 15);
+#pragma unroll
+        for (int t = 0; t < 2; ++t) {
+            if (t == 1 && !second) break;
+            const int ls = wave + t * AQ_PW;
+            const f32x4_t tot = sum_waves<4>(red[ls], 0, lane);
+            DGEMM_CONSUMER_FINISH(v, tot, bias4[t], cs4[t], a.stats_in, mean, rstd, GITMI_ACT_NONE);
+            if (i >= 0 && i < AQ_PW) {
+                uint2 o;
+                o.x = pack2bf(v[0], v[1]);
+                o.y = pack2bf(v[2], v[3]);
+                *reinterpret_cast<uint2*>(&rows[i][ls * 16 + lg * 4]) = o;
+            }
+        }
+    }
+    attn_lds_barrier();
+    const QkvSrc qs{rows[wave], 0, HD};
+
+    const int grp = lane >> 3, sub = lane & 7;
+    TextItems<KB, TI> ti;
+    ti.load(a, p, qs, grp, 8, sub);
+    append_text_cache(a, p, qs, lane, sub);
+    bf16x8_t qf[2];
+    load_q_frag(a, p, qs, l15, lg, qf);
+
+    ImagePartial ip;
+    ip.init();
+    for (int s0 = 0; s0 < nimg_steps; s0 += ACS) {
+        if (s0 != 0) { load_k(s0); load_v(s0); }
+        f32x4_t sc[ACS][2];
+        float cm = -INFINITY;
+#pragma unroll
+        for (int c = 0; c < ACS; ++c) {
+#pragma unroll
+            for (int u = 0; u < 2; ++u) {
+                sc[c][u] = mfma16(kq[c][u][0], qf[0], f32x4_t{0.f, 0.f, 0.f, 0.f});
+                sc[c][u] = mfma16(kq[c][u][1], qf[1], sc[c][u]);
+            }
+            ip.mask_max(sc[c], s0 + c, nimg_steps, a.N_img, lg, cm);
+        }
+        const float mn = ip.new_max(cm, s0 != 0);
+#pragma unroll
+        for (int c = 0; c < ACS; ++c) {
+            const bf16x8_t pf = ip.p_frag(sc[c], mn);
+#pragma unroll
+            for (int dt = 0; dt < 4; ++dt) ip.o[dt] = mfma16(vq[c][dt], pf, ip.o[dt]);
+        }
+    }
+    ip.finish();
+    TextPartial<KB> tp;
+    tp.init(a, p, qs, sub);
+    tp.items(ti, true);
+    tp.template tail<TI>(a, p, qs, grp, 8, sub);
+    tp.merge_groups();
+    ip.publish(part[wave], a.beams, l15, lg);
+    __builtin_amdgcn_wave_barrier();
+    tp.fold_into(part[wave], a.beams, lane, sub);
+    __builtin_amdgcn_wave_barrier();
+    write_rows(a, p, part[wave], lane, 64);
 }
 
 typedef __attribute__((address_space(3))) void attn_lds_void_t;
@@ -481,11 +645,12 @@
         const Pair p{pair % H, (pair / H) * k, true};
 
         const int grp = lane >> 3, sub = lane & 7;
+        const QkvSrc qs = qkv_rows(a, p);
         TextItems<KB, TI> ti;
-        ti.load(a, p, grp, 8, sub);
-        append_text_cache(a, p, lane, sub);
+        ti.load(a, p, qs, grp, 8, sub);
+        append_text_cache(a, p, qs, lane, sub);
         bf16x8_t qf[2];
-        load_q_frag(a, p, l15, lg, qf);
+        load_q_frag(a, p, qs, l15, lg, qf);
 
         ImagePartial ip;
         ip.init();
@@ -536,9 +701,9 @@
         }
         ip.finish();
         TextPartial<KB> tp;
-        tp.init(a, p, sub);
+        tp.init(a, p, qs, sub);
         tp.items(ti, true);
-        tp.template tail<TI>(a, p, grp, 8, sub);
+        tp.template tail<TI>(a, p, qs, grp, 8, sub);
         tp.merge_groups();
         ip.publish(part[wave], k, l15, lg);
         __builtin_amdgcn_wave_barrier();
@@ -563,6 +728,30 @@
     else if (beams <= 2) f(std::integral_constant<int, 2>{});
     else if (beams <= 4) f(std::integral_constant<int, 4>{});
     else f(std::integral_constant<int, 8>{});
+}
+
+int attn_decode_pairs_per_wg(const AttnDecodeArgs& a, int B, int H) {
+    int pw = a.pairs_per_wg >= 8 ? 8 : a.pairs_per_wg >= 4 || a.pairs_per_wg <= 0 ? 4 : a.pairs_per_wg >= 2 ? 2 : 1;
+    while (pw > 1 && B * H / pw < 96) pw >>= 1;
+    if (a.beams > 4 && pw == 8) pw = 4;
+    return pw;
+}
+
+bool attn_decode_qkv_form(const AttnDecodeArgs& a, int B, int H) {
+    if (B <= 0 || a.beams != 1 || a.waves_per_pair == 2 || a.ntok || a.stream_wgs != 0 || a.dbg) return false;
+    if (a.N_img < 1 || a.N_pad % 32 || a.N_pad < a.N_img || a.N_pad > 8 * 32) return false;
+    if (a.d != H * HD || a.d > 4 * DW_KS * 32 || a.M < B) return false;
+    if (!a.x || !a.w || !a.bias) return false;
+    return !a.stats_in || (a.colsum && a.strips_in >= 1 && a.strips_in <= 4 * STRIP_SLOTS);
+}
+
+hipError_t launch_attn_decode_qkv(const AttnDecodeArgs& a, int B, int H, hipStream_t s) {
+    if (!attn_decode_qkv_form(a, B, H)) return hipErrorInvalidValue;
+    AttnDecodeArgs p = a;
+    p.n_pairs = B * H;
+    const int total = H * ((B + AQ_PW - 1) / AQ_PW);
+    hipLaunchKernelGGL((attn_decode_qkv_kernel<3>), dim3(8 * ((total + 7) / 8)), dim3(64 * AQ_PW), 0, s, p);
+    return hipGetLastError();
 }
 
 hipError_t launch_attn_decode_mfma(const AttnDecodeArgs& a, int B, int H, hipStream_t s) {
@@ -588,9 +777,7 @@
         });
         return hipGetLastError();
     }
-    int pw = a.pairs_per_wg >= 8 ? 8 : a.pairs_per_wg >= 4 || a.pairs_per_wg <= 0 ? 4 : a.pairs_per_wg >= 2 ? 2 : 1;
-    while (pw > 1 && p.n_pairs / pw < 96) pw >>= 1;
-    if (a.beams > 4 && pw == 8) pw = 4;
+    const int pw = attn_decode_pairs_per_wg(a, B, H);
     with_beam_rows(a.beams, [&](auto kb) {
         constexpr int KB = decltype(kb)::value;
         auto packed = [&](auto pwc) {
diff --git a/generativeimage2text_amd/csrc/kernels_dgemm.hip b/generativeimage2text_amd/csrc/kernels_dgemm.hip
--- a/generativeimage2text_amd/csrc/kernels_dgemm.hip
+++ b/generativeimage2text_amd/csrc/kernels_dgemm.hip
@@ -1,114 +1,12 @@
 #include "gitmi_common.h"
 #include "launchers.h"
+#include "dgemm_shared.h"
 #include <type_traits>
 #include <utility>
 
 namespace gitmi {
 
-constexpr int STRIP_SLOTS = 16;
-
-struct RowStatLoads {
-    float2 v[STRIP_SLOTS];
-};
-__device__ __forceinline__ void stats_issue(RowStatLoads& L, const float2* __restrict__ stats, int strips, int M,
-                                            int row, int lg) {
-#pragma unroll
-    for (int u = 0; u < STRIP_SLOTS; ++u) {
-        const int sidx = lg + 4 * u;
-        L.v[u] = sidx < strips ? stats[(size_t)sidx * M + row] : float2{0.f, 0.f};
-    }
-}
-__device__ __forceinline__ void stats_issue_nb(RowStatLoads& L, const float2* __restrict__ stats, int strips, int M,
-                                               int row, int lg) {
-#pragma unroll
-    for (int u = 0; u < STRIP_SLOTS; ++u) {
-        const int sidx = lg + 4 * u;
-        const float2 v = stats[(size_t)min(sidx, strips - 1) * M + row];
-        L.v[u] = sidx < strips ? v : float2{0.f, 0.f};
-    }
-}
-__device__ __forceinline__ void stats_finish(const RowStatLoads& L, float inv_d, float eps, float& mean, float& rstd) {
-    float s = 0.f, q = 0.f;
-#pragma unroll
-    for (int u = 0; u < STRIP_SLOTS; ++u) { s += L.v[u].x; q += L.v[u].y; }
-    s += __shfl_xor(s, 16, 64); q += __shfl_xor(q, 16, 64);
-    s += __shfl_xor(s, 32, 64); q += __shfl_xor(q, 32, 64);
-    mean = s * inv_d;
-    const float var = fmaxf(q * inv_d - mean * mean, 0.f);
-    rstd = rsqrtf(var + eps);
-}
-
-
-struct KSlice { int kb, ke; };
-__device__ __forceinline__ KSlice k_slice(int ksteps, int nw, int wave) {
-    const int per = (ksteps + nw - 1) / nw;
-    const int kb = wave * per;
-    return KSlice{kb, min(kb + per, ksteps)};
-}
-
-__device__ __forceinline__ float4 load_cols4(const float* p, int n, int N) {
-    float4 r;
-    r.x = p[n < N ? n : N - 1];
-    r.y = p[n + 1 < N ? n + 1 : N - 1];
-    r.z = p[n + 2 < N ? n + 2 : N - 1];
-    r.w = p[n + 3 < N ? n + 3 : N - 1];
-    return r;
-}
-
-constexpr int DW_KS = 6;
-struct WSlice { bf16x8_t f[DW_KS]; };
-__device__ __forceinline__ WSlice load_w_slice(const bf16_t* W, int strip, KSlice ks, int ksteps, int lane) {
-    WSlice w;
-    const bf16_t* wp = W + frag_tile(strip, 0, ksteps, lane);
-#pragma unroll
-    for (int u = 0; u < DW_KS; ++u)
-        w.f[u] = ks.kb + u < ks.ke ? __builtin_nontemporal_load(reinterpret_cast<const bf16x8_t*>(wp + (size_t)(ks.kb + u) * 512))
-                                   : bf16x8_t{0, 0, 0, 0, 0, 0, 0, 0};
-    return w;
-}
-__device__ __forceinline__ void load_x_slice(bf16x8_t (&xf)[DW_KS][4], const bf16_t* X, int rt0, KSlice ks, int ksteps, int lane) {
-#pragma unroll
-    for (int u = 0; u < DW_KS; ++u)
-#pragma unroll
-        for (int i = 0; i < 4; ++i)
-            xf[u][i] = ks.kb + u < ks.ke ? *reinterpret_cast<const bf16x8_t*>(X + frag_tile(rt0 + i, ks.kb + u, ksteps, lane))
-                                         : bf16x8_t{0, 0, 0, 0, 0, 0, 0, 0};
-}
-__device__ __forceinline__ void mfma_slice(f32x4_t (&acc)[4], const WSlice& w, const bf16x8_t (&xf)[DW_KS][4], KSlice ks) {
-#pragma unroll
-    for (int u = 0; u < DW_KS; ++u) {
-        if (ks.kb + u < ks.ke) {
-#pragma unroll
-            for (int i = 0; i < 4; ++i) acc[i] = mfma16(w.f[u], xf[u][i], acc[i]);
-        }
-    }
-}
-
-template <int NW, int MT>
-__device__ __forceinline__ f32x4_t sum_waves(f32x4_t (*red)[MT][64], int tile, int lane) {
-    f32x4_t tot = {0.f, 0.f, 0.f, 0.f};
-#pragma unroll
-    for (int w = 0; w < NW; ++w) {
-        const f32x4_t t = red[w][tile][lane];
-        tot[0] += t[0]; tot[1] += t[1]; tot[2] += t[2]; tot[3] += t[3];
-    }
-    return tot;
-}
-
-#define DGEMM_CONSUMER_FINISH(v, tot, bias4, cs4, have_stats, mean, rstd, act)              \
-    float v[4] = {(tot)[0], (tot)[1], (tot)[2], (tot)[3]};                                  \
-    {                                                                                       \
-        const float biasv[4] = {(bias4).x, (bias4).y, (bias4).z, (bias4).w};                \
-        if (have_stats) {                                                                   \
-            const float cs[4] = {(cs4).x, (cs4).y, (cs4).z, (cs4).w};                       \
-            _Pragma("unroll") for (int r = 0; r < 4; ++r) v[r] = (rstd) * (v[r] - (mean) * cs[r]) + biasv[r]; \
-        } else {                                                                            \
-            _Pragma("unroll") for (int r = 0; r < 4; ++r) v[r] += biasv[r];                 \
-        }                                                                                   \
-        if ((act) != GITMI_ACT_NONE) {                                                      \
-            _Pragma("unroll") for (int r = 0; r < 4; ++r) v[r] = apply_act(v[r], (act));    \
-        }                                                                                   \
-    }
+
 __device__ __forceinline__ void consumer_store(const DGemmArgs& g, const float (&v)[4], int fm_raw, int fm, int fn) {
     if (fm_raw >= g.M || fn >= g.N) return;
     if (g.c_frag) {
diff --git a/generativeimage2text_amd/csrc/launchers.h b/generativeimage2text_amd/csrc/launchers.h
--- a/generativeimage2text_amd/csrc/launchers.h
+++ b/generativeimage2text_amd/csrc/launchers.h
@@ -140,11 +140,21 @@
     int waves_per_pair;
     int n_pairs;
     const int* ntok;
+    const unsigned short* x; const unsigned short* w; const float* bias; const float* colsum;
+    const float2* stats_in; int strips_in; float inv_d, eps_in;
+    int M;
 };
 hipError_t launch_kv_repack(const void* qkv, void* kh, void* vh, int B, int N, int H, int d, hipStream_t s);
 hipError_t launch_attn_decode(const AttnDecodeArgs& a, int B, int H, hipStream_t s);
 hipError_t launch_kv_repack_frag(const void* qkv, void* kf, void* vt, int B, int N, int N_pad, int H, int d, hipStream_t s);
 hipError_t launch_attn_decode_mfma(const AttnDecodeArgs& a, int B, int H, hipStream_t s);
+int attn_decode_pairs_per_wg(const AttnDecodeArgs& a, int B, int H);
+bool attn_decode_qkv_form(const AttnDecodeArgs& a, int B, int H);
+inline void attn_decode_set_qkv(AttnDecodeArgs& a, const DGemmArgs& g) {
+    a.x = g.A; a.w = g.W; a.bias = g.bias; a.colsum = g.colsum;
+    a.stats_in = g.stats_in; a.strips_in = g.strips_in; a.inv_d = g.inv_d; a.eps_in = g.eps_in; a.M = g.M;
+}
+hipError_t launch_attn_decode_qkv(const AttnDecodeArgs& a, int B, int H, hipStream_t s);
 
 constexpr int SS_NHMAX = 8;
 struct SearchState {
diff --git a/generativeimage2text_amd/engine.py b/generativeimage2text_amd/engine.py
--- a/generativeimage2text_amd/engine.py
+++ b/generativeimage2text_amd/engine.py
@@ -38,7 +38,7 @@
     "gitmi_debug_vocab_topm_rules", "gitmi_debug_search_begin_prefixed", "gitmi_debug_search_advance_lists", "gitmi_debug_read_hidden",
     "gitmi_debug_im2col", "gitmi_debug_pos_resize", "gitmi_debug_vit_assemble", "gitmi_debug_ragged_front", "gitmi_debug_zero_pad_rows",
     "gitmi_debug_layernorm_map", "gitmi_debug_score_attn_map", "gitmi_debug_attn_decode_form", "gitmi_debug_dgemm_form",
-    "gitmi_debug_gemm_form", "gitmi_debug_context_embed",
+    "gitmi_debug_gemm_form", "gitmi_debug_context_embed", "gitmi_debug_attn_decode_qkv",
 ]
 
 
@@ -152,6 +152,8 @@
         lib.gitmi_debug_attn_decode_ragged.argtypes = [vp, vp, vp, vp, vp, vp, vp, vp, i32, i32, i32, i32, i32, i32, i32, vp]
         lib.gitmi_debug_attn_decode_form.argtypes = [vp, vp, vp, vp, vp, vp, vp, vp, vp, i32, i32, i32, i32, i32, i32, i32, i32, i32,
                                                      i32, i32, i32, vp]
+        lib.gitmi_debug_attn_decode_qkv.argtypes = [vp, i32, vp, vp, vp, vp, i32, C.c_float, vp, vp, vp, vp, vp, vp, vp, vp, i32, i32, i32,
+                                                    i32, i32, i32, i32, i32, i32, i32, i32, i32, vp]
         lib.gitmi_debug_vocab_topm_rules.argtypes = [vp, vp, vp, vp, vp, i32, C.c_float, i32, i32, i32, i32, i32, vp, i32, i32, vp, i32,
                                                      i32, C.c_float, vp, vp, vp, vp, i32, vp]
         lib.gitmi_debug_search_begin_prefixed.argtypes = [vp, C.POINTER(GitmiSearch), i32, vp, i32, vp, i32, vp]
@@ -1112,6 +1114,28 @@
     return out
 
 
+def op_attn_decode_qkv(x, w, bias, img_k, img_v, txt_k, txt_v, kv_src, B, H, N_img, T_max, pos, beams=1, *, colsum=None, stats=None,
+                       eps: float = 1e-12, out=None, img_of=None, ntok=None, out_frag=False, pairs_per_wg=8, waves_per_pair=1,
+                       stream_wgs=0):
+    lib = _exp_library(x.dtype, w.dtype, img_k.dtype, img_v.dtype, txt_k.dtype, txt_v.dtype)
+    d = H * 64
+    n_images = img_k.shape[0] if img_k.dim() == 4 else img_k.numel() // (H * ((N_img + 31) // 32 * 32) * 64)
+    if img_k.dim() == 4:
+        img_k, img_v = kv_repack(img_k, img_v)
+    if img_of is not None:
+        img_of = torch.as_tensor(img_of, dtype=torch.int32).to(x.device)
+    if ntok is not None:
+        ntok = torch.as_tensor(ntok, dtype=torch.int32).to(x.device)
+    if out is None:
+        out = torch.empty((B * beams + 15) // 16 * 16 if out_frag else B * beams, d, device=x.device, dtype=x.dtype)
+    _ck(_experiment_only(lib, "gitmi_debug_attn_decode_qkv")(
+        x.data_ptr(), int(x.shape[0]), w.data_ptr(), _ptr(bias), _ptr(colsum), _ptr(stats), 0 if stats is None else int(stats.shape[0]),
+        eps, img_k.data_ptr(), img_v.data_ptr(), txt_k.data_ptr(), txt_v.data_ptr(), kv_src.data_ptr(), out.data_ptr(), _ptr(ntok),
+        _ptr(img_of), n_images, B, H, N_img, T_max, pos, beams, _torch_dtype_code(x), int(bool(out_frag)), int(pairs_per_wg),
+        int(waves_per_pair), int(stream_wgs), _stream()), lib)
+    return out
+
+
 def op_score_attn(qkv: torch.Tensor, img_kv: torch.Tensor, image_of: torch.Tensor, Q: int, H: int, N_img: int,
                   Lp: int) -> torch.Tensor:
     lib = load_library()
diff --git a/include/gitmi_experiment.h b/include/gitmi_experiment.h
--- a/include/gitmi_experiment.h
+++ b/include/gitmi_experiment.h
@@ -38,6 +38,11 @@
                                   const int* kv_src, void* out, const int* ntok, const int* img_of, int n_images, int B, int H,
                                   int N_img, int T_max, int pos, int beams, int dtype, int out_frag, int pairs_per_wg,
                                   int waves_per_pair, int stream_wgs, void* stream);
+int  gitmi_debug_attn_decode_qkv(const void* x, int x_rows, const void* w, const float* bias, const float* colsum, const float* stats,
+                                 int strips, float eps, const void* img_k, const void* img_v, void* txt_k, void* txt_v,
+                                 const int* kv_src, void* out, const int* ntok, const int* img_of, int n_images, int B, int H,
+                                 int N_img, int T_max, int pos, int beams, int dtype, int out_frag, int pairs_per_wg,
+                                 int waves_per_pair, int stream_wgs, void* stream);
 
 int  gitmi_debug_vocab_topm_rules(const void* A, const void* W, const float* bias, const float* colsum, const float* stats,
                                   int strips, float eps, int M, int V, int K, int cols_per_wg, int mtop, const int* ids, int ld_ids,
```

Result: faster. 11550 captions/s (median of 6 runs) (+1.5%).
